# fcogidi/X3D-tf

Measured on NVIDIA B200. Metric: X3D-M clips/sec, higher is better.
Workload: dtype bf16

## Files before the change

### include/x3d_b200.h

```cpp
#ifndef X3D_B200_H_
#define X3D_B200_H_

#include <stddef.h>
#include <stdint.h>

#ifdef __cplusplus
extern "C" {
#endif

#define X3D_B200_VERSION 100

enum x3d_dtype { X3D_F32 = 0, X3D_BF16 = 1 };

enum x3d_status {
  X3D_OK = 0,
  X3D_ERR_INVALID_ARG = -1,
  X3D_ERR_UNSUPPORTED = -2,
  X3D_ERR_LAUNCH = -3,
  X3D_ERR_NO_DEVICE = -4
};

int x3d_version(void);
const char* x3d_last_error(void);

uint32_t x3d_crc32c(const void* data, size_t len, uint32_t crc);

int x3d_stem_fwd(const void* in, int in_dtype, const float* ws, const float* wt,
                 const float* bias, void* out, int out_dtype,
                 int N, int T, int H, int W, int C, int kt, void* stream);

int x3d_stem_tc_fwd(const void* in, int in_dtype, const void* wc, const float* bias, void* out,
                    int N, int T, int H, int W, int C, int kt, void* stream);

typedef struct x3d_pw_args {
  const void* A; const float* Wt; const float* bias; const void* R; const float* se; void* D;
  int64_t M; int32_t K, Nc, lda, ldw, ldr, ldd;
  int64_t rows_per_clip;
  int32_t a_dtype, d_dtype, swish, relu;
  int32_t gather, T, Ho, Wo, Hi, Wi, stride;
} x3d_pw_args;
int x3d_pw_fwd(const x3d_pw_args* args, void* stream);

int x3d_tf32_split(const float* W, float* out, int rows, int cols, int ld, int transpose, void* stream);
int x3d_pw_tf32_fwd(const float* A, const float* Bsplit, const float* bias, float* D, int64_t M, int K,
                    int Nc, int lda, int ldd, int relu, double* stats, void* stream);

int x3d_dw_partial_blocks(int T, int H, int W, int C, int stride, int dtype);
int x3d_dw3x3x3_fwd(const void* in, const float* w, const float* bias, void* out,
                    float* se_partial, int N, int T, int H, int W, int C, int stride,
                    int pad_h, int pad_w, int dtype, void* stream);
int x3d_dw3x3x3_act_fwd(const void* in, const float* w, const float* bias, void* out,
                        float* se_partial, int N, int T, int H, int W, int C, int stride,
                        int pad_h, int pad_w, int dtype, int act, void* stream);

int x3d_dw_planar_partial_blocks(int T, int H, int W, int C, int stride);
int x3d_dw_planar_lane_permille(int T, int H, int W, int C, int stride);
int x3d_dw3x3x3_planar_fwd(const void* in, const float* taps, void* out, float* se_partial, int N, int T,
                           int H, int W, int C, int stride, int pad_h, int pad_w, int act, void* stream);

int x3d_se_mlp_fwd(const float* partial, int nblk, float inv_count, const float* w1,
                   const float* b1, const float* w2, const float* b2, float* scale,
                   int N, int C, int Cw, void* stream);

int x3d_avgpool_fwd(const void* in, float* out, int N, int64_t P, int C, int dtype, void* stream);

int x3d_softmax_viewmean_fwd(const float* logits, float* probs, int N, int ncls, int num_preds,
                             void* stream);

int x3d_gather_rows_fwd(const void* in, void* out, int NT, int Hi, int Wi, int stride, int C,
                        int dtype, void* stream);

int x3d_head_fc_fwd(const float* A, const float* Wt, const float* bias, float* D, int M, int K,
                    int Nc, int lda, int ldw, int ldd, int relu, void* stream);

typedef struct x3d_pw_tc_args {
  const void* A; const void* Wp; const float* bias; const void* R; const float* se; void* D;
  int64_t M; int32_t K, Nc, lda, ldr, ldd, Kpad, Npad;
  int64_t rows_per_clip;
  int32_t swish, relu;
  const void* A2; int64_t a2_nt; int32_t K2, a2_stride, a2_hi, a2_wi;
  float* colmean; int32_t store_d, reserved;
} x3d_pw_tc_args;
int x3d_pw_tc_fwd(const x3d_pw_tc_args* args, void* stream);
int x3d_pw_tc_sampler_supported(int Hi, int Wi, int stride);

int x3d_expand_dw_partial_blocks(int T, int H, int W, int Cin, int C, int stride);
int x3d_expand_dw_fwd(const void* x, const void* wa, const float* bias_a, const float* wb,
                      const float* bias_b, void* out, float* se_partial, int N, int T, int H,
                      int W, int Cin, int C, int Kpad, int Npad, int stride, int pad_h, int pad_w,
                      void* stream);

int x3d_expand_dw2_partial_blocks(int T, int H, int W, int Cin, int C, int stride);
int x3d_expand_dw2_fwd(const void* x, const void* wa, const float* bias_a, const float* wb,
                       const float* bias_b, void* out, float* se_partial, int N, int T, int H,
                       int W, int Cin, int C, int Kpad, int Npad, int stride, int pad_h, int pad_w,
                       int act, void* stream);

int x3d_normalize_u8(const uint8_t* in, void* out, int64_t pixels, const float* mean,
                     const float* std, float norm_value, int dtype, void* stream);
int x3d_eval_views_u8(const uint8_t* video, uint8_t* out, int F, int H, int W, int T, int views,
                      int crops, int S, void* stream);
int x3d_stem_tc_u8_fwd(const uint8_t* in, const float* mean, const float* std, float norm_value,
                       const void* wc, const float* bias, void* out, int N, int T, int H, int W,
                       int C, int kt, void* stream);
int x3d_eval_metrics(const float* probs, const int32_t* labels, double* acc, int V, int ncls,
                     int k, void* stream);


int x3d_colreduce(const float* a, const float* x, const float* mean, const float* rstd,
                  const float* relu_out, int64_t M, int C, int64_t seg_rows, double* out, int mode,
                  void* stream);
int x3d_bn_finalize(const double* sums, int64_t M, int C, float eps, float momentum, float* mean,
                    float* var, float* rstd, float* mov_mean, float* mov_var, void* stream);
int x3d_bn_apply_fwd(const float* x, const float* mean, const float* rstd, const float* gamma,
                     const float* beta, float* y, int64_t M, int C, int relu, void* stream);
int x3d_bn_bwd_apply(const float* dy, const float* x, const float* relu_out, const float* mean,
                     const float* rstd, const float* gamma, const double* sums, float* dx, int64_t M,
                     int C, void* stream);
int x3d_d2f(const double* in, float* out, int64_t n, float scale, void* stream);
int x3d_pw_wgrad(const float* A, const float* dD, double* dW, int64_t M, int K, int N, int lda,
                 int ldd, int gather, int Ho, int Wo, int Hi, int Wi, int stride, void* stream);
int x3d_dw_dgrad(const float* dy, const float* w, float* dx, int N, int T, int H, int W, int C,
                 int stride, int pad_h, int pad_w, void* stream);
int x3d_dw_wgrad(const float* x, const float* dy, double* dwt, int N, int T, int H, int W, int C,
                 int stride, int pad_h, int pad_w, void* stream);
int x3d_stem_convs_fwd(const float* in, const float* ws, float* out, int N, int T, int H, int W,
                       int C, void* stream);
int x3d_stem_convs_wgrad(const float* in, const float* ds, double* dws, int N, int T, int H, int W,
                         int C, void* stream);
int x3d_tconv_fwd(const float* in, const float* wt, float* out, int N, int T, int64_t P, int C,
                  int kt, int flip, void* stream);
int x3d_tconv_wgrad(const float* s, const float* dy, double* dwt, int N, int T, int64_t P, int C,
                    int kt, void* stream);
int x3d_scale_swish_fwd(const float* y, const float* s, float* out, int64_t M, int C,
                        int64_t rows_per_clip, void* stream);
int x3d_scale_swish_bwd(const float* dout, const float* y, const float* s, float* dy, double* ds,
                        int64_t M, int C, int64_t rows_per_clip, void* stream);
int x3d_ew(const float* a, const float* b, float* out, int64_t n, int op, void* stream);
int x3d_pool_bwd(const float* dm, float* dy, int64_t M, int C, int64_t rows_per_clip, float scale,
                 int accumulate, void* stream);
int x3d_strided_add(const float* src, float* dst, int NT, int Ho, int Wo, int Hi, int Wi,
                    int stride, int C, void* stream);
int x3d_dropout_mask(float* mask, int64_t n, float rate, uint64_t seed, void* stream);
int x3d_softmax_xent(const float* logits, const int32_t* labels, float* loss, float* dlogits, int N,
                     int ncls, float gscale, void* stream);
int x3d_sgd_nesterov_step(float* w, const float* grad, float* v, const float* wd, int64_t n,
                          float lr, float momentum, void* stream);
int x3d_adam_step(float* w, const float* grad, float* m, float* v, const float* wd, int64_t n,
                  float lr_t, float beta1, float beta2, float eps, void* stream);

#ifdef __cplusplus
}
#endif
#endif
```

### x3d_tf_b200/_lib.py

```python
from __future__ import annotations

import ctypes as C
import os
import threading

LIB_PATH = os.path.join(os.path.dirname(os.path.abspath(__file__)), "lib", "libx3d_b200.so")

X3D_F32, X3D_BF16 = 0, 1


class X3DLibError(RuntimeError):
    pass


class PwArgs(C.Structure):
    _fields_ = [("A", C.c_void_p), ("Wt", C.c_void_p), ("bias", C.c_void_p), ("R", C.c_void_p),
                ("se", C.c_void_p), ("D", C.c_void_p),
                ("M", C.c_int64), ("K", C.c_int32), ("Nc", C.c_int32), ("lda", C.c_int32),
                ("ldw", C.c_int32), ("ldr", C.c_int32), ("ldd", C.c_int32),
                ("rows_per_clip", C.c_int64),
                ("a_dtype", C.c_int32), ("d_dtype", C.c_int32), ("swish", C.c_int32),
                ("relu", C.c_int32),
                ("gather", C.c_int32), ("T", C.c_int32), ("Ho", C.c_int32), ("Wo", C.c_int32),
                ("Hi", C.c_int32), ("Wi", C.c_int32), ("stride", C.c_int32)]


class PwTcArgs(C.Structure):
    _fields_ = [("A", C.c_void_p), ("Wp", C.c_void_p), ("bias", C.c_void_p), ("R", C.c_void_p),
                ("se", C.c_void_p), ("D", C.c_void_p),
                ("M", C.c_int64), ("K", C.c_int32), ("Nc", C.c_int32), ("lda", C.c_int32),
                ("ldr", C.c_int32), ("ldd", C.c_int32), ("Kpad", C.c_int32), ("Npad", C.c_int32),
                ("rows_per_clip", C.c_int64), ("swish", C.c_int32), ("relu", C.c_int32),
                ("A2", C.c_void_p), ("a2_nt", C.c_int64), ("K2", C.c_int32), ("a2_stride", C.c_int32),
                ("a2_hi", C.c_int32), ("a2_wi", C.c_int32),
                ("colmean", C.c_void_p), ("store_d", C.c_int32), ("reserved", C.c_int32)]


SIGNATURES = {
    "x3d_version": (C.c_int, []),
    "x3d_last_error": (C.c_char_p, []),
    "x3d_crc32c": (C.c_uint32, [C.c_void_p, C.c_size_t, C.c_uint32]),
    "x3d_stem_fwd": (C.c_int, [C.c_void_p, C.c_int, C.c_void_p, C.c_void_p, C.c_void_p,
                               C.c_void_p, C.c_int, C.c_int, C.c_int, C.c_int, C.c_int, C.c_int,
                               C.c_int, C.c_void_p]),
    "x3d_stem_tc_fwd": (C.c_int, [C.c_void_p, C.c_int, C.c_void_p, C.c_void_p, C.c_void_p, C.c_int,
                                  C.c_int, C.c_int, C.c_int, C.c_int, C.c_int, C.c_void_p]),
    "x3d_pw_fwd": (C.c_int, [C.POINTER(PwArgs), C.c_void_p]),
    "x3d_tf32_split": (C.c_int, [C.c_void_p, C.c_void_p, C.c_int, C.c_int, C.c_int, C.c_int, C.c_void_p]),
    "x3d_pw_tf32_fwd": (C.c_int, [C.c_void_p] * 4 + [C.c_int64] + [C.c_int] * 5 + [C.c_void_p, C.c_void_p]),
    "x3d_dw_partial_blocks": (C.c_int, [C.c_int, C.c_int, C.c_int, C.c_int, C.c_int, C.c_int]),
    "x3d_dw3x3x3_fwd": (C.c_int, [C.c_void_p, C.c_void_p, C.c_void_p, C.c_void_p, C.c_void_p,
                                  C.c_int, C.c_int, C.c_int, C.c_int, C.c_int, C.c_int, C.c_int,
                                  C.c_int, C.c_int, C.c_void_p]),
    "x3d_dw3x3x3_act_fwd": (C.c_int, [C.c_void_p, C.c_void_p, C.c_void_p, C.c_void_p, C.c_void_p,
                                      C.c_int, C.c_int, C.c_int, C.c_int, C.c_int, C.c_int, C.c_int,
                                      C.c_int, C.c_int, C.c_int, C.c_void_p]),
    "x3d_dw_planar_partial_blocks": (C.c_int, [C.c_int] * 5),
    "x3d_dw_planar_lane_permille": (C.c_int, [C.c_int] * 5),
    "x3d_dw3x3x3_planar_fwd": (C.c_int, [C.c_void_p] * 4 + [C.c_int] * 9 + [C.c_void_p]),
    "x3d_se_mlp_fwd": (C.c_int, [C.c_void_p, C.c_int, C.c_float, C.c_void_p, C.c_void_p,
                                 C.c_void_p, C.c_void_p, C.c_void_p, C.c_int, C.c_int, C.c_int,
                                 C.c_void_p]),
    "x3d_avgpool_fwd": (C.c_int, [C.c_void_p, C.c_void_p, C.c_int, C.c_int64, C.c_int, C.c_int,
                                  C.c_void_p]),
    "x3d_softmax_viewmean_fwd": (C.c_int, [C.c_void_p, C.c_void_p, C.c_int, C.c_int, C.c_int,
                                           C.c_void_p]),
    "x3d_pw_tc_fwd": (C.c_int, [C.POINTER(PwTcArgs), C.c_void_p]),
    "x3d_pw_tc_sampler_supported": (C.c_int, [C.c_int] * 3),
    "x3d_gather_rows_fwd": (C.c_int, [C.c_void_p, C.c_void_p, C.c_int, C.c_int, C.c_int, C.c_int,
                                      C.c_int, C.c_int, C.c_void_p]),
    "x3d_expand_dw_partial_blocks": (C.c_int, [C.c_int] * 6),
    "x3d_expand_dw_fwd": (C.c_int, [C.c_void_p] * 7 + [C.c_int] * 11 + [C.c_void_p]),
    "x3d_expand_dw2_partial_blocks": (C.c_int, [C.c_int] * 6),
    "x3d_expand_dw2_fwd": (C.c_int, [C.c_void_p] * 7 + [C.c_int] * 12 + [C.c_void_p]),
    "x3d_colreduce": (C.c_int, [C.c_void_p] * 5 + [C.c_int64, C.c_int, C.c_int64, C.c_void_p, C.c_int, C.c_void_p]),
    "x3d_bn_finalize": (C.c_int, [C.c_void_p, C.c_int64, C.c_int, C.c_float, C.c_float] + [C.c_void_p] * 6),
    "x3d_bn_apply_fwd": (C.c_int, [C.c_void_p] * 6 + [C.c_int64, C.c_int, C.c_int, C.c_void_p]),
    "x3d_bn_bwd_apply": (C.c_int, [C.c_void_p] * 8 + [C.c_int64, C.c_int, C.c_void_p]),
    "x3d_d2f": (C.c_int, [C.c_void_p, C.c_void_p, C.c_int64, C.c_float, C.c_void_p]),
    "x3d_pw_wgrad": (C.c_int, [C.c_void_p] * 3 + [C.c_int64] + [C.c_int] * 10 + [C.c_void_p]),
    "x3d_dw_dgrad": (C.c_int, [C.c_void_p] * 3 + [C.c_int] * 8 + [C.c_void_p]),
    "x3d_dw_wgrad": (C.c_int, [C.c_void_p] * 3 + [C.c_int] * 8 + [C.c_void_p]),
    "x3d_stem_convs_fwd": (C.c_int, [C.c_void_p] * 3 + [C.c_int] * 5 + [C.c_void_p]),
    "x3d_stem_convs_wgrad": (C.c_int, [C.c_void_p] * 3 + [C.c_int] * 5 + [C.c_void_p]),
    "x3d_tconv_fwd": (C.c_int, [C.c_void_p] * 3 + [C.c_int, C.c_int, C.c_int64, C.c_int, C.c_int, C.c_int, C.c_void_p]),
    "x3d_tconv_wgrad": (C.c_int, [C.c_void_p] * 3 + [C.c_int, C.c_int, C.c_int64, C.c_int, C.c_int, C.c_void_p]),
    "x3d_scale_swish_fwd": (C.c_int, [C.c_void_p] * 3 + [C.c_int64, C.c_int, C.c_int64, C.c_void_p]),
    "x3d_scale_swish_bwd": (C.c_int, [C.c_void_p] * 5 + [C.c_int64, C.c_int, C.c_int64, C.c_void_p]),
    "x3d_ew": (C.c_int, [C.c_void_p] * 3 + [C.c_int64, C.c_int, C.c_void_p]),
    "x3d_pool_bwd": (C.c_int, [C.c_void_p] * 2 + [C.c_int64, C.c_int, C.c_int64, C.c_float, C.c_int, C.c_void_p]),
    "x3d_strided_add": (C.c_int, [C.c_void_p] * 2 + [C.c_int] * 7 + [C.c_void_p]),
    "x3d_dropout_mask": (C.c_int, [C.c_void_p, C.c_int64, C.c_float, C.c_uint64, C.c_void_p]),
    "x3d_softmax_xent": (C.c_int, [C.c_void_p] * 4 + [C.c_int, C.c_int, C.c_float, C.c_void_p]),
    "x3d_adam_step": (C.c_int, [C.c_void_p] * 5 + [C.c_int64, C.c_float, C.c_float, C.c_float, C.c_float, C.c_void_p]),
    "x3d_sgd_nesterov_step": (C.c_int, [C.c_void_p] * 4 + [C.c_int64, C.c_float, C.c_float, C.c_void_p]),
    "x3d_normalize_u8": (C.c_int, [C.c_void_p, C.c_void_p, C.c_int64, C.POINTER(C.c_float),
                                   C.POINTER(C.c_float), C.c_float, C.c_int, C.c_void_p]),
    "x3d_eval_views_u8": (C.c_int, [C.c_void_p, C.c_void_p] + [C.c_int] * 7 + [C.c_void_p]),
    "x3d_stem_tc_u8_fwd": (C.c_int, [C.c_void_p, C.POINTER(C.c_float), C.POINTER(C.c_float), C.c_float,
                                     C.c_void_p, C.c_void_p, C.c_void_p] + [C.c_int] * 6 + [C.c_void_p]),
    "x3d_eval_metrics": (C.c_int, [C.c_void_p, C.c_void_p, C.c_void_p, C.c_int, C.c_int, C.c_int,
                                   C.c_void_p]),
    "x3d_head_fc_fwd": (C.c_int, [C.c_void_p, C.c_void_p, C.c_void_p, C.c_void_p, C.c_int, C.c_int,
                                  C.c_int, C.c_int, C.c_int, C.c_int, C.c_int, C.c_void_p]),
}

_lock = threading.Lock()
_lib = None


def lib() -> C.CDLL:
    global _lib
    if _lib is None:
        with _lock:
            if _lib is None:
                if not os.path.exists(LIB_PATH):
                    raise X3DLibError(
                        f"{LIB_PATH} is missing: build it with `python -m x3d_tf_b200.build` "
                        "(nvcc, sm_100a).  There is no CPU or PyTorch fallback.")
                h = C.CDLL(LIB_PATH)
                for name, (res, args) in SIGNATURES.items():
                    fn = getattr(h, name)
                    fn.restype, fn.argtypes = res, args
                if h.x3d_version() != 100:
                    raise X3DLibError(f"ABI version mismatch: library reports {h.x3d_version()}")
                _lib = h
                try:
                    from . import tf_bundle
                    tf_bundle.set_native_crc32c(
                        lambda data, crc=0: h.x3d_crc32c(C.c_char_p(data), len(data), crc))
                except Exception:
                    pass
    return _lib


calls = 0


def check(status: int, what: str = "") -> None:
    global calls
    calls += 1
    if status != 0:
        msg = lib().x3d_last_error().decode("utf-8", "replace")
        raise X3DLibError(f"{what or 'x3d call'} failed with status {status}: {msg}")
```

### x3d_tf_b200/csrc/x3d_pw_tc.cu

```cuda
#include <stdlib.h>

#include "tma_common.cuh"

namespace x3d {
namespace tc {

constexpr int kBlockM = 128, kBlockK = 64, kStageBytes = kBlockM * kBlockK * 2;
using namespace ptx;

#ifdef X3D_PW_TRACE
__device__ long long g_pw_trace[8 * 256];
#define X3D_TRACE(slot)                                                                  \
  do {                                                                                   \
    if (trace_on && trace_n < 256) g_pw_trace[trace_n * 8 + (slot)] = clock64();         \
  } while (0)
#else
#define X3D_TRACE(slot) do {} while (0)
#endif

__device__ __forceinline__ void tcgen05_before_sync() {
  asm volatile("tcgen05.fence::before_thread_sync;" ::: "memory");
}
__device__ __forceinline__ void tcgen05_after_sync() {
  asm volatile("tcgen05.fence::after_thread_sync;" ::: "memory");
}
__device__ __forceinline__ void umma_bf16(uint32_t tmem_d, uint64_t desc_a, uint64_t desc_b,
                                          uint32_t idesc, uint32_t accumulate) {
  asm volatile(
      "{\n\t.reg .pred p;\n\t"
      "setp.ne.b32 p, %4, 0;\n\t"
      "tcgen05.mma.cta_group::1.kind::f16 [%0], %1, %2, %3, p;\n\t}" ::"r"(tmem_d),
      "l"(desc_a), "l"(desc_b), "r"(idesc), "r"(accumulate)
      : "memory");
}
__device__ __forceinline__ void umma_commit(uint64_t* bar) {
  asm volatile("tcgen05.commit.cta_group::1.mbarrier::arrive::one.shared::cluster.b64 [%0];" ::"r"(
                   smem_u32(bar))
               : "memory");
}
__device__ __forceinline__ void tmem_ld16(uint32_t taddr, uint32_t (&v)[16]) {
  asm volatile(
      "tcgen05.ld.sync.aligned.32x32b.x16.b32 "
      "{%0, %1, %2, %3, %4, %5, %6, %7, %8, %9, %10, %11, %12, %13, %14, %15}, [%16];"
      : "=r"(v[0]), "=r"(v[1]), "=r"(v[2]), "=r"(v[3]), "=r"(v[4]), "=r"(v[5]), "=r"(v[6]),
        "=r"(v[7]), "=r"(v[8]), "=r"(v[9]), "=r"(v[10]), "=r"(v[11]), "=r"(v[12]), "=r"(v[13]),
        "=r"(v[14]), "=r"(v[15])
      : "r"(taddr));
}
__device__ __forceinline__ void tmem_ld_wait() {
  asm volatile("tcgen05.wait::ld.sync.aligned;" ::: "memory");
}

__device__ __forceinline__ uint64_t make_desc_sw128(uint32_t smem_addr) {
  uint64_t d = 0;
  d |= static_cast<uint64_t>((smem_addr & 0x3FFFF) >> 4);
  d |= static_cast<uint64_t>(0) << 16;
  d |= static_cast<uint64_t>(1024 >> 4) << 32;
  d |= static_cast<uint64_t>(1) << 46;
  d |= static_cast<uint64_t>(2) << 61;
  return d;
}
__device__ __forceinline__ uint32_t make_idesc_bf16(int n) {
  return (1u << 4) | (1u << 7) | (1u << 10) | (static_cast<uint32_t>(n >> 3) << 17) |
         (static_cast<uint32_t>(kBlockM >> 4) << 24);
}

struct Params {
  const float* bias; const bf16* R; const float* se; bf16* D;
  long M; long rows_per_clip;
  int Kc;
  int Nc;
  int ldr, ldd;
  int NT;
  int KC;
  int k16_last;
  int KC1;
  int k16_last1;
  int a2_ppf;
  int a2_wo;
  float* colmean;
  int ldc;
  int store_d;
  int stages;
  int tmem_cols;
  int relu, swish;
  int contiguous;
};

constexpr int kEpiWarps = 8, kProWarps = 8, kOutBufs = 4;
constexpr int kProGroups = 2;
constexpr int kProRows = 8 * kProWarps / kProGroups / 2;
constexpr int kThreadsPlain = 64 + 32 * kEpiWarps, kThreadsPro = kThreadsPlain + 32 * kProWarps;

template <bool kPro>
__global__ void __launch_bounds__(kPro ? kThreadsPro : kThreadsPlain, 1)
pw_tc_kernel(const __grid_constant__ CUtensorMap tmA, const __grid_constant__ CUtensorMap tmW,
             const __grid_constant__ CUtensorMap tmD, const __grid_constant__ CUtensorMap tmA2,
             const Params p) {
  extern __shared__ __align__(1024) uint8_t smem_raw[];
  uint8_t* smem = reinterpret_cast<uint8_t*>((reinterpret_cast<uintptr_t>(smem_raw) + 1023) &
                                             ~static_cast<uintptr_t>(1023));
  const int warp = threadIdx.x >> 5, lane = threadIdx.x & 31;
  const int n0 = blockIdx.y * p.NT;
  const int w_chunk_bytes = p.NT * 128;

  uint8_t* sW = smem;
  uint8_t* sA = sW + p.KC * w_chunk_bytes;
  uint8_t* sD = sA + p.stages * kStageBytes;
  float* sBias = reinterpret_cast<float*>(sD + kOutBufs * kStageBytes);
  uint64_t* bars = reinterpret_cast<uint64_t*>(sBias + 256);
  uint64_t* full = bars;
  uint64_t* empty = full + p.stages;
  uint64_t* xform = empty + p.stages;
  uint64_t* w_full = xform + p.stages;
  uint64_t* t_full = w_full + 1;
  uint64_t* t_empty = t_full + 2;
  uint32_t* tmem_slot = reinterpret_cast<uint32_t*>(t_empty + 2);

  for (int i = threadIdx.x; i < p.NT; i += blockDim.x) {
    const int col = n0 + i;
    sBias[i] = (p.bias != nullptr && col < p.Nc) ? p.bias[col] : 0.f;
  }
  if (warp == 0 && elect_one()) {
    prefetch_tmap(&tmA);
    prefetch_tmap(&tmW);
    prefetch_tmap(&tmD);
    if (p.KC > p.KC1) prefetch_tmap(&tmA2);
    for (int s = 0; s < p.stages; ++s) {
      mbar_init(&full[s], 1);
      mbar_init(&empty[s], 1);
      mbar_init(&xform[s], 32 * kProWarps / kProGroups);
    }
    mbar_init(w_full, 1);
    for (int i = 0; i < 2; ++i) {
      mbar_init(&t_full[i], 1);
      mbar_init(&t_empty[i], 16 * kEpiWarps);
    }
    fence_barrier_init();
  }
  if (warp == 1) {
    asm volatile("tcgen05.alloc.cta_group::1.sync.aligned.shared::cta.b32 [%0], %1;" ::"r"(
                     smem_u32(tmem_slot)),
                 "r"(static_cast<uint32_t>(p.tmem_cols))
                 : "memory");
    asm volatile("tcgen05.relinquish_alloc_permit.cta_group::1.sync.aligned;" ::: "memory");
  }
  tcgen05_before_sync();
  __syncthreads();
  tcgen05_after_sync();
  const uint32_t tmem_base = *tmem_slot;

  const long num_tiles = (p.M + kBlockM - 1) / kBlockM;
  long tile_lo = blockIdx.x, tile_hi = num_tiles, t_stride = gridDim.x;
  if (p.contiguous) {
    const long t_per = num_tiles / gridDim.x, t_rem = num_tiles % gridDim.x;
    tile_lo = blockIdx.x * t_per + (blockIdx.x < t_rem ? blockIdx.x : t_rem);
    tile_hi = tile_lo + t_per + (blockIdx.x < t_rem ? 1 : 0);
    t_stride = 1;
  }

  if (warp == 0) {
    if (elect_one()) {
      mbar_expect_tx(w_full, static_cast<uint32_t>(p.KC * w_chunk_bytes));
      for (int kc = 0; kc < p.KC; ++kc)
        tma_load_2d(sW + kc * w_chunk_bytes, &tmW, kc * kBlockK, n0, w_full);
      pdl_wait();
      pdl_trigger();
      int s = 0;
      uint32_t ph = 0;
      for (long tile = tile_lo; tile < tile_hi; tile += t_stride) {
        const int row0 = static_cast<int>(tile * kBlockM);
        int nt0 = 0, ho0 = 0;
        if (p.a2_ppf) {
          nt0 = row0 / p.a2_ppf;
          ho0 = (row0 - nt0 * p.a2_ppf) / p.a2_wo;
        }
        for (int kc = 0; kc < p.KC; ++kc) {
          mbar_wait(&empty[s], ph ^ 1);
          mbar_expect_tx(&full[s], kStageBytes);
          if (kc < p.KC1) tma_load_2d(sA + s * kStageBytes, &tmA, kc * kBlockK, row0, &full[s]);
          else if (p.a2_ppf) tma_load_4d(smem_u32(sA + s * kStageBytes), &tmA2, (kc - p.KC1) * kBlockK, 0, ho0, nt0, &full[s]);
          else tma_load_2d(sA + s * kStageBytes, &tmA2, (kc - p.KC1) * kBlockK, row0, &full[s]);
          if (++s == p.stages) { s = 0; ph ^= 1; }
        }
      }
    }
  } else if (warp == 1) {
    pdl_trigger();
    const uint32_t idesc = make_idesc_bf16(p.NT);
    mbar_wait(w_full, 0);
    int s = 0;
    uint32_t ph = 0;
    long it = 0;
    for (long tile = tile_lo; tile < tile_hi; tile += t_stride, ++it) {
      const int as = static_cast<int>(it & 1);
      const uint32_t aph = static_cast<uint32_t>((it >> 1) & 1);
      mbar_wait(&t_empty[as], aph ^ 1);
      tcgen05_after_sync();
      const uint32_t d_tmem = tmem_base + static_cast<uint32_t>(as * p.NT);
      for (int kc = 0; kc < p.KC; ++kc) {
        mbar_wait(kPro ? &xform[s] : &full[s], ph);
        tcgen05_after_sync();
        if (elect_one()) {
          const uint32_t a_addr = smem_u32(sA + s * kStageBytes);
          const uint32_t b_addr = smem_u32(sW + kc * w_chunk_bytes);
          const int nk = (kc == p.KC - 1) ? p.k16_last : (kc == p.KC1 - 1 ? p.k16_last1 : 4);
          for (int k = 0; k < nk; ++k)
            umma_bf16(d_tmem, make_desc_sw128(a_addr + k * 32), make_desc_sw128(b_addr + k * 32),
                      idesc, (kc | k) != 0 ? 1u : 0u);
          umma_commit(&empty[s]);
          if (kc == p.KC - 1) umma_commit(&t_full[as]);
        }
        __syncwarp();
        if (++s == p.stages) { s = 0; ph ^= 1; }
      }
    }
  } else if (warp < 2 + kEpiWarps) {
    pdl_wait();
    pdl_trigger();
    const int q = warp & 3;
    const int grp = (warp - 2) >> 2;
    const bool leader = q == 2 && lane == 0;
    const __nv_bfloat162 zero2 = __floats2bfloat162_rn(0.f, 0.f);
    const int r_loc = q * 32 + lane;
    const uint32_t sw_row = static_cast<uint32_t>(r_loc) * 128, sw_x = static_cast<uint32_t>(r_loc & 7);
    const int n_sub = (p.NT + 63) >> 6;
    const uint32_t stage0 = smem_u32(sD + grp * 2 * kStageBytes);
    const uint32_t bias_s = smem_u32(sBias);
    const uint32_t taddr = tmem_base + (static_cast<uint32_t>(q * 32) << 16) +
                           static_cast<uint32_t>(grp * p.NT);
    uint32_t sub_ctr = 0, aph = 0;
#ifdef X3D_PW_TRACE
    const bool trace_on = blockIdx.x == 7 && blockIdx.y == 0 && grp == 0 && leader;
    int trace_n = 0;
#endif
    for (long tile = tile_lo + grp * t_stride; tile < tile_hi; tile += 2 * t_stride, aph ^= 1) {
      X3D_TRACE(0);
      const long row = tile * kBlockM + r_loc;
      const bool row_ok = row < p.M;
      const bf16* rrow = (p.R && row_ok) ? p.R + row * p.ldr + n0 : nullptr;
      uint4 rr[8];
#pragma unroll
      for (int c = 0; c < 8; ++c)
        rr[c] = (rrow && c * 8 < p.NT && n0 + c * 8 < p.Nc) ? __ldg(reinterpret_cast<const uint4*>(rrow + c * 8))
                                                           : make_uint4(0, 0, 0, 0);
      if (p.R) {
        const long nrow = row + 2L * t_stride * kBlockM;
        if (nrow < p.M && tile + 2 * t_stride < tile_hi) {
          const char* np_ = reinterpret_cast<const char*>(p.R + nrow * p.ldr + n0);
          for (int off = 0; off < p.NT * 2; off += 128)
            asm volatile("prefetch.global.L2 [%0];" ::"l"(np_ + off));
        }
      }
      mbar_wait(&t_full[grp], aph);
      X3D_TRACE(1);
      tcgen05_after_sync();
      for (int sb = 0; sb < n_sub; ++sb, ++sub_ctr) {
        if (n0 + sb * 64 >= p.Nc) break;
        const uint32_t buf = stage0 + (sub_ctr & 1) * kStageBytes + sw_row;
        if (sb > 0) {
#pragma unroll
          for (int c = 0; c < 8; ++c) {
            const int cc = sb * 64 + c * 8;
            rr[c] = (rrow && cc < p.NT && n0 + cc < p.Nc) ? __ldg(reinterpret_cast<const uint4*>(rrow + cc))
                                                         : make_uint4(0, 0, 0, 0);
          }
        }
#pragma unroll
        for (int g = 0; g < 4; ++g) {
          const int c0 = sb * 64 + g * 16;
          if (c0 >= p.NT || n0 + c0 >= p.Nc) continue;
          uint32_t v[16];
          tmem_ld16(taddr + c0, v);
          tmem_ld_wait();
#ifdef X3D_PW_TRACE
          if (g == 0 && sb == 0 && trace_on && trace_n < 256) g_pw_trace[trace_n * 8 + 7] = clock64();
#endif
#pragma unroll
          for (int h = 0; h < 2; ++h) {
            const int cc = c0 + h * 8;
            float4 b0, b1;
            asm volatile("ld.shared.v4.f32 {%0, %1, %2, %3}, [%4];" : "=f"(b0.x), "=f"(b0.y), "=f"(b0.z), "=f"(b0.w) : "r"(bias_s + cc * 4));
            asm volatile("ld.shared.v4.f32 {%0, %1, %2, %3}, [%4];" : "=f"(b1.x), "=f"(b1.y), "=f"(b1.z), "=f"(b1.w) : "r"(bias_s + cc * 4 + 16));
            float2 y[4];
            y[0] = __fadd2_rn(make_float2(__uint_as_float(v[h * 8 + 0]), __uint_as_float(v[h * 8 + 1])), make_float2(b0.x, b0.y));
            y[1] = __fadd2_rn(make_float2(__uint_as_float(v[h * 8 + 2]), __uint_as_float(v[h * 8 + 3])), make_float2(b0.z, b0.w));
            y[2] = __fadd2_rn(make_float2(__uint_as_float(v[h * 8 + 4]), __uint_as_float(v[h * 8 + 5])), make_float2(b1.x, b1.y));
            y[3] = __fadd2_rn(make_float2(__uint_as_float(v[h * 8 + 6]), __uint_as_float(v[h * 8 + 7])), make_float2(b1.z, b1.w));
            if (p.R) {
              const uint4 ru = rr[g * 2 + h];
              const uint32_t rw[4] = {ru.x, ru.y, ru.z, ru.w};
#pragma unroll
              for (int j = 0; j < 4; ++j)
                y[j] = __fadd2_rn(y[j], make_float2(__uint_as_float(rw[j] << 16),
                                                    __uint_as_float(rw[j] & 0xffff0000u)));
            }
            uint32_t o[4];
#pragma unroll
            for (int j = 0; j < 4; ++j) {
              __nv_bfloat162 t = __float22bfloat162_rn(y[j]);
              if (p.relu) t = __hmax2(t, zero2);
              o[j] = *reinterpret_cast<uint32_t*>(&t);
            }
            const uint32_t chunk = static_cast<uint32_t>(g * 2 + h);
            asm volatile("st.shared.v4.b32 [%0], {%1, %2, %3, %4};" ::"r"(buf + ((chunk ^ sw_x) << 4)),
                         "r"(o[0]), "r"(o[1]), "r"(o[2]), "r"(o[3]) : "memory");
          }
        }
        X3D_TRACE(2);
        if (sb == n_sub - 1 || n0 + (sb + 1) * 64 >= p.Nc) {
          tcgen05_before_sync();
          mbar_arrive(&t_empty[grp]);
        }
        fence_proxy_async();
        X3D_TRACE(3);
        if (leader) tma_store_wait_read<0>();
        X3D_TRACE(4);
        if (grp == 0) asm volatile("bar.sync 1, 128;" ::: "memory");
        else asm volatile("bar.sync 2, 128;" ::: "memory");
        X3D_TRACE(5);
        if (leader && p.store_d) {
          tma_store_2d(&tmD, stage0 + (sub_ctr & 1) * kStageBytes, n0 + sb * 64,
                       static_cast<int>(tile * kBlockM));
          tma_store_commit();
        }
        if (p.colmean != nullptr) {
          const int ccol = r_loc & 63, half = r_loc >> 6;
          const int col_g = n0 + sb * 64 + ccol;
          const long row_base = tile * kBlockM + half * 64;
          int nrows = p.M - row_base < 64 ? static_cast<int>(p.M - row_base) : 64;
          if (ccol < p.NT - sb * 64 && col_g < p.Nc && nrows > 0) {
            const uint32_t sbuf = stage0 + (sub_ctr & 1) * kStageBytes;
            float sum = 0.f;
            for (int r = 0; r < nrows; ++r) {
              const int row = half * 64 + r;
              unsigned short h;
              asm volatile("ld.shared.u16 %0, [%1];" : "=h"(h)
                           : "r"(sbuf + row * 128 + ((((ccol >> 3) ^ (row & 7)) << 4) | ((ccol & 7) << 1))));
              sum += __uint_as_float(static_cast<uint32_t>(h) << 16);
            }
            p.colmean[(tile * 2 + half) * p.ldc + col_g] = sum * (1.f / 64.f);
          }
        }
        X3D_TRACE(6);
#ifdef X3D_PW_TRACE
        if (trace_on) ++trace_n;
#endif
      }
    }
    if (leader) tma_store_wait_read<0>();
  } else if (kPro) {
    pdl_wait();
    pdl_trigger();
    const int tt = threadIdx.x - kThreadsPlain;
    constexpr int kGT = 32 * kProWarps / kProGroups;
    const int grp = tt / kGT;
    const int pchunk = tt & 7;
    const int rbase = (tt % kGT) >> 3;
    const int kin = (pchunk ^ (rbase & 7)) << 3;
    const uint32_t rpc = static_cast<uint32_t>(p.rows_per_clip > 0 ? p.rows_per_clip : 0x7fffffff);
    const uint32_t step = static_cast<uint32_t>(t_stride) * kBlockM;
    struct Pos { long tile; int kc; uint32_t clip, rem; };
    auto advance = [&](Pos& q) {
      if (++q.kc == p.KC) {
        q.kc = 0;
        q.tile += t_stride;
        q.rem += step;
        while (q.rem >= rpc) { q.rem -= rpc; ++q.clip; }
      }
    };
    auto se_request = [&](const Pos& q, float4& s0, float4& s1) {
      s0 = make_float4(1.f, 1.f, 1.f, 1.f);
      s1 = s0;
      const int k = q.kc * kBlockK + kin;
      if (p.se != nullptr && q.tile < tile_hi && k < p.Kc && q.kc < p.KC1 && q.rem + kBlockM <= rpc) {
        const float4* sp = reinterpret_cast<const float4*>(p.se + static_cast<long>(q.clip) * p.Kc + k);
        s0 = __ldg(sp);
        s1 = __ldg(sp + 1);
      }
    };
    Pos cur;
    cur.tile = tile_lo; cur.kc = 0;
    cur.clip = static_cast<uint32_t>(tile_lo * static_cast<long>(kBlockM) / rpc);
    cur.rem = static_cast<uint32_t>(tile_lo * static_cast<long>(kBlockM) - static_cast<long>(cur.clip) * rpc);
    int s = 0;
    uint32_t ph = 0;
    for (int g = 0; g < grp; ++g) {
      advance(cur);
      if (++s == p.stages) { s = 0; ph ^= 1; }
    }
    float4 nx0, nx1;
    se_request(cur, nx0, nx1);
    while (cur.tile < tile_hi) {
      const uint32_t clip0 = cur.clip, rem0 = cur.rem;
      const bool one_clip = rem0 + kBlockM <= rpc;
      const int k = cur.kc * kBlockK + kin;
      const bool k_ok = k < p.Kc && cur.kc < p.KC1;
      float2 sc[4];
      sc[0] = make_float2(nx0.x, nx0.y); sc[1] = make_float2(nx0.z, nx0.w);
      sc[2] = make_float2(nx1.x, nx1.y); sc[3] = make_float2(nx1.z, nx1.w);
#pragma unroll
      for (int g = 0; g < kProGroups; ++g) advance(cur);
      se_request(cur, nx0, nx1);
      mbar_wait(&full[s], ph);
      if (k_ok) {
        const uint32_t addr0 = smem_u32(sA + s * kStageBytes) + rbase * 128 + pchunk * 16;
        float2 hs[4];
#pragma unroll
        for (int j = 0; j < 4; ++j) hs[j] = __fmul2_rn(sc[j], make_float2(0.5f, 0.5f));
#pragma unroll
        for (int half = 0; half < kBlockM / (kGT / 8) / 4; ++half) {
          uint32_t w[4][4];
#pragma unroll
          for (int i = 0; i < 4; ++i)
            asm volatile("ld.shared.v4.b32 {%0, %1, %2, %3}, [%4];"
                         : "=r"(w[i][0]), "=r"(w[i][1]), "=r"(w[i][2]), "=r"(w[i][3])
                         : "r"(addr0 + (half * 4 + i) * (kGT / 8 * 128)));
#pragma unroll
          for (int i = 0; i < 4; ++i) {
            if (p.se && !one_clip) {
              uint32_t x = rem0 + rbase + (kGT / 8) * (half * 4 + i), clip = clip0;
              while (x >= rpc) { x -= rpc; ++clip; }
              if (static_cast<long>(clip) * rpc + x < p.M) {
                const float4* sp = reinterpret_cast<const float4*>(p.se + static_cast<long>(clip) * p.Kc + k);
                const float4 s0 = __ldg(sp), s1 = __ldg(sp + 1);
                sc[0] = make_float2(s0.x, s0.y); sc[1] = make_float2(s0.z, s0.w);
                sc[2] = make_float2(s1.x, s1.y); sc[3] = make_float2(s1.z, s1.w);
#pragma unroll
                for (int j = 0; j < 4; ++j) hs[j] = __fmul2_rn(sc[j], make_float2(0.5f, 0.5f));
              }
            }
            if (p.swish) {
#pragma unroll
              for (int j = 0; j < 4; ++j) {
                const float2 h = __fmul2_rn(make_float2(__uint_as_float(w[i][j] << 16), __uint_as_float(w[i][j] & 0xffff0000u)), hs[j]);
                float2 t;
                asm("tanh.approx.f32 %0, %1;" : "=f"(t.x) : "f"(h.x));
                asm("tanh.approx.f32 %0, %1;" : "=f"(t.y) : "f"(h.y));
                __nv_bfloat162 t2 = __float22bfloat162_rn(__ffma2_rn(h, t, h));
                w[i][j] = *reinterpret_cast<uint32_t*>(&t2);
              }
            } else {
#pragma unroll
              for (int j = 0; j < 4; ++j) {
                const float2 scj = make_float2(2.f * hs[j].x, 2.f * hs[j].y);
                __nv_bfloat162 t2 = __float22bfloat162_rn(__fmul2_rn(
                    make_float2(__uint_as_float(w[i][j] << 16), __uint_as_float(w[i][j] & 0xffff0000u)), scj));
                w[i][j] = *reinterpret_cast<uint32_t*>(&t2);
              }
            }
            asm volatile("st.shared.v4.b32 [%0], {%1, %2, %3, %4};" ::"r"(addr0 + (half * 4 + i) * (kGT / 8 * 128)), "r"(w[i][0]), "r"(w[i][1]), "r"(w[i][2]), "r"(w[i][3]) : "memory");
          }
        }
      }
      fence_proxy_async();
      mbar_arrive(&xform[s]);
      s += kProGroups;
      while (s >= p.stages) { s -= p.stages; ph ^= 1; }
    }
  }

  tcgen05_before_sync();
  __syncthreads();
  if (warp == 1) {
    asm volatile("tcgen05.dealloc.cta_group::1.sync.aligned.b32 %0, %1;" ::"r"(tmem_base),
                 "r"(static_cast<uint32_t>(p.tmem_cols))
                 : "memory");
  }
}

static bool make_map_2d(CUtensorMap* m, const void* base, uint64_t inner, uint64_t outer,
                        uint64_t row_stride_bytes, uint32_t box_inner, uint32_t box_outer) {
  EncodeTiledFn enc = tensor_map_encoder();
  if (!enc) return false;
  cuuint64_t dims[2] = {inner, outer};
  cuuint64_t strides[1] = {row_stride_bytes};
  cuuint32_t box[2] = {box_inner, box_outer};
  cuuint32_t estr[2] = {1, 1};
  return enc(m, CU_TENSOR_MAP_DATA_TYPE_BFLOAT16, 2, const_cast<void*>(base), dims, strides, box,
             estr, CU_TENSOR_MAP_INTERLEAVE_NONE, CU_TENSOR_MAP_SWIZZLE_128B,
             CU_TENSOR_MAP_L2_PROMOTION_L2_256B, CU_TENSOR_MAP_FLOAT_OOB_FILL_NONE) == CUDA_SUCCESS;
}

static bool make_map_sampler(CUtensorMap* m, const void* base, int C, int Hi, int Wi, long NT, int s,
                             int bw, int bh, int bf) {
  EncodeTiledFn enc = tensor_map_encoder();
  if (!enc) return false;
  const int Ho = (Hi - 1) / s + 1, Wo = (Wi - 1) / s + 1;
  cuuint64_t dims[4] = {(cuuint64_t)C, (cuuint64_t)Wo, (cuuint64_t)Ho, (cuuint64_t)NT};
  cuuint64_t strides[3] = {(cuuint64_t)s * C * 2, (cuuint64_t)s * Wi * C * 2, (cuuint64_t)Hi * Wi * C * 2};
  cuuint32_t box[4] = {64, (cuuint32_t)bw, (cuuint32_t)bh, (cuuint32_t)bf};
  cuuint32_t estr[4] = {1, 1, 1, 1};
  return enc(m, CU_TENSOR_MAP_DATA_TYPE_BFLOAT16, 4, const_cast<void*>(base), dims, strides, box,
             estr, CU_TENSOR_MAP_INTERLEAVE_NONE, CU_TENSOR_MAP_SWIZZLE_128B,
             CU_TENSOR_MAP_L2_PROMOTION_L2_256B, CU_TENSOR_MAP_FLOAT_OOB_FILL_NONE) == CUDA_SUCCESS;
}

static bool sampler_box(int Ho, int Wo, int* bh, int* bf) {
  if (Wo <= 0 || Wo > kBlockM || kBlockM % Wo) return false;
  const int rh = kBlockM / Wo;
  if (rh <= Ho) { if (Ho % rh) return false; *bh = rh; *bf = 1; return true; }
  if (rh % Ho) return false;
  *bh = Ho; *bf = rh / Ho;
  return true;
}

}
}

using namespace x3d;

extern "C" int x3d_pw_tc_sampler_supported(int Hi, int Wi, int stride) {
  if (Hi <= 0 || Wi <= 0 || stride < 1) return 0;
  int bh, bf;
  return tc::sampler_box((Hi - 1) / stride + 1, (Wi - 1) / stride + 1, &bh, &bf) ? 1 : 0;
}

extern "C" int x3d_pw_tc_fwd(const x3d_pw_tc_args* a, void* stream) {
  X3D_REQUIRE(a && a->A && a->Wp && a->D, X3D_ERR_INVALID_ARG, "x3d_pw_tc_fwd: null pointer");
  X3D_REQUIRE(a->M > 0 && a->M < (1L << 31), X3D_ERR_INVALID_ARG, "x3d_pw_tc_fwd: M out of range");
  X3D_REQUIRE(a->K > 0 && a->K % 8 == 0 && a->lda % 8 == 0 && a->lda >= a->K, X3D_ERR_INVALID_ARG,
              "x3d_pw_tc_fwd: K=%d / lda=%d must be multiples of 8", a->K, a->lda);
  X3D_REQUIRE(a->Nc > 0 && a->Nc % 8 == 0 && a->ldd % 8 == 0 && (!a->R || a->ldr % 8 == 0),
              X3D_ERR_INVALID_ARG, "x3d_pw_tc_fwd: Nc/ldd/ldr must be multiples of 8");
  X3D_REQUIRE(a->Kpad % 64 == 0 && a->Kpad >= a->K && a->Npad % 16 == 0 && a->Npad >= a->Nc,
              X3D_ERR_INVALID_ARG, "x3d_pw_tc_fwd: bad packed weight extents Kpad=%d Npad=%d", a->Kpad, a->Npad);
  X3D_REQUIRE(!a->se || a->rows_per_clip > 0, X3D_ERR_INVALID_ARG, "x3d_pw_tc_fwd: rows_per_clip missing");
  X3D_REQUIRE(!a->colmean || (reinterpret_cast<uintptr_t>(a->colmean) & 3) == 0, X3D_ERR_INVALID_ARG, "x3d_pw_tc_fwd: colmean alignment");
  X3D_REQUIRE((reinterpret_cast<uintptr_t>(a->A) & 15) == 0 && (reinterpret_cast<uintptr_t>(a->Wp) & 15) == 0 &&
              (reinterpret_cast<uintptr_t>(a->D) & 15) == 0, X3D_ERR_INVALID_ARG, "x3d_pw_tc_fwd: pointers must be 16-byte aligned");
  X3D_REQUIRE(device_sm_count() > 0 && device_is_sm100(), X3D_ERR_NO_DEVICE, "x3d_pw_tc_fwd: needs an sm_100 device");
  const int k16_total = (a->K + 15) / 16;
  const int KC1 = (k16_total + 3) / 4;
  const int k16_last1 = k16_total - (KC1 - 1) * 4;
  int KC = KC1, k16_last = k16_last1, a2_bh = 0, a2_bf = 0, a2_ho = 0, a2_wo = 0;
  if (a->A2) {
    X3D_REQUIRE(!a->R, X3D_ERR_INVALID_ARG, "x3d_pw_tc_fwd: A2 (shortcut as extra K) and R (residual) exclude each other");
    X3D_REQUIRE(a->K2 > 0 && a->K2 % 8 == 0 && a->a2_stride >= 0, X3D_ERR_INVALID_ARG, "x3d_pw_tc_fwd: bad second source K2=%d stride=%d", a->K2, a->a2_stride);
    X3D_REQUIRE((reinterpret_cast<uintptr_t>(a->A2) & 15) == 0, X3D_ERR_INVALID_ARG, "x3d_pw_tc_fwd: A2 must be 16-byte aligned");
    if (a->a2_stride > 0) {
      X3D_REQUIRE(a->a2_hi > 0 && a->a2_wi > 0 && a->a2_nt > 0, X3D_ERR_INVALID_ARG, "x3d_pw_tc_fwd: bad second source %dx%d", a->a2_hi, a->a2_wi);
      a2_ho = (a->a2_hi - 1) / a->a2_stride + 1; a2_wo = (a->a2_wi - 1) / a->a2_stride + 1;
      X3D_REQUIRE(a->M == a->a2_nt * a2_ho * a2_wo, X3D_ERR_INVALID_ARG, "x3d_pw_tc_fwd: M=%ld is not nt*Ho*Wo = %ld*%d*%d",
                  (long)a->M, (long)a->a2_nt, a2_ho, a2_wo);
      X3D_REQUIRE(tc::sampler_box(a2_ho, a2_wo, &a2_bh, &a2_bf), X3D_ERR_UNSUPPORTED,
                  "x3d_pw_tc_fwd: 128-pixel tiles do not align with %dx%d frames (x3d_pw_tc_sampler_supported)", a2_ho, a2_wo);
    }
    const int k16_2 = (a->K2 + 15) / 16, KC2 = (k16_2 + 3) / 4;
    KC = KC1 + KC2; k16_last = k16_2 - (KC2 - 1) * 4;
    X3D_REQUIRE(a->Kpad >= KC * 64, X3D_ERR_INVALID_ARG, "x3d_pw_tc_fwd: Kpad=%d < %d (both sources, 64-wide chunks)", a->Kpad, KC * 64);
  }
  const int budget = device_max_smem() - 1024  - 1024  - 512  -
                     tc::kOutBufs * tc::kStageBytes ;
  int n_tiles = (a->Npad + 255) / 256;
  int NT = 0, stages = 0;
  for (;; ++n_tiles) {
    const int per = (a->Npad + n_tiles - 1) / n_tiles;
    NT = n_tiles == 1 ? (per + 15) / 16 * 16 : (per + 63) / 64 * 64;
    const int wbytes = KC * NT * 128;
    stages = (budget - wbytes) / tc::kStageBytes;
    if (stages >= 3 || NT <= 64) break;
  }
  X3D_REQUIRE(stages >= 2 && stages >= tc::kProGroups, X3D_ERR_UNSUPPORTED, "x3d_pw_tc_fwd: K=%d too large for shared memory", a->K);
  if (stages > 8) stages = 8;
  n_tiles = (a->Nc + NT - 1) / NT;
  int tmem_cols = 32;
  while (tmem_cols < 2 * NT) tmem_cols *= 2;
  X3D_REQUIRE(tmem_cols <= 512, X3D_ERR_UNSUPPORTED, "x3d_pw_tc_fwd: NT=%d needs too much TMEM", NT);

  CUtensorMap tmA, tmW;
  X3D_REQUIRE(tensor_map_encoder() != nullptr, X3D_ERR_NO_DEVICE, "x3d_pw_tc_fwd: cuTensorMapEncodeTiled unavailable");
  X3D_REQUIRE(tc::make_map_2d(&tmA, a->A, (uint64_t)a->K, (uint64_t)a->M, (uint64_t)a->lda * 2, 64, 128),
              X3D_ERR_LAUNCH, "x3d_pw_tc_fwd: tensor map for A failed (K=%d M=%ld lda=%d)", a->K, (long)a->M, a->lda);
  X3D_REQUIRE(tc::make_map_2d(&tmW, a->Wp, (uint64_t)a->Kpad, (uint64_t)a->Npad, (uint64_t)a->Kpad * 2, 64, (uint32_t)NT),
              X3D_ERR_LAUNCH, "x3d_pw_tc_fwd: tensor map for W failed (Kpad=%d Npad=%d NT=%d)", a->Kpad, a->Npad, NT);

  CUtensorMap tmD;
  X3D_REQUIRE(tc::make_map_2d(&tmD, a->D, (uint64_t)a->Nc, (uint64_t)a->M, (uint64_t)a->ldd * 2, 64, 128),
              X3D_ERR_LAUNCH, "x3d_pw_tc_fwd: tensor map for D failed (Nc=%d M=%ld ldd=%d)", a->Nc, (long)a->M, a->ldd);
  CUtensorMap tmA2 = tmA;
  if (a->A2 && a->a2_stride > 0)
    X3D_REQUIRE(tc::make_map_sampler(&tmA2, a->A2, a->K2, a->a2_hi, a->a2_wi, (long)a->a2_nt, a->a2_stride, a2_wo, a2_bh, a2_bf),
                X3D_ERR_LAUNCH, "x3d_pw_tc_fwd: tensor map for A2 failed (K2=%d %dx%d stride %d)", a->K2, a->a2_hi, a->a2_wi, a->a2_stride);
  else if (a->A2)
    X3D_REQUIRE(tc::make_map_2d(&tmA2, a->A2, (uint64_t)a->K2, (uint64_t)a->M, (uint64_t)a->K2 * 2, 64, 128),
                X3D_ERR_LAUNCH, "x3d_pw_tc_fwd: tensor map for dense A2 failed (K2=%d M=%ld)", a->K2, (long)a->M);
  tc::Params p;
  p.bias = a->bias; p.R = static_cast<const bf16*>(a->R); p.se = a->se; p.D = static_cast<bf16*>(a->D);
  p.M = a->M; p.rows_per_clip = a->rows_per_clip; p.Kc = a->K; p.Nc = a->Nc; p.ldr = a->ldr; p.ldd = a->ldd;
  p.colmean = a->colmean; p.ldc = a->Nc; p.store_d = a->colmean == nullptr || a->store_d;
  p.KC1 = KC1; p.k16_last1 = k16_last1; p.a2_ppf = (a->A2 && a->a2_stride > 0) ? a2_ho * a2_wo : 0; p.a2_wo = a2_wo;
  p.NT = NT; p.KC = KC; p.k16_last = k16_last; p.stages = stages; p.tmem_cols = tmem_cols;
  p.relu = a->relu; p.swish = a->swish;
  p.contiguous = a->se != nullptr ? 1 : 0;

  const size_t smem = 1024 + (size_t)KC * NT * 128 + (size_t)(stages + tc::kOutBufs) * tc::kStageBytes + 1024 + 512;
  const long num_tiles = (a->M + tc::kBlockM - 1) / tc::kBlockM;
  int gx = device_sm_count() / n_tiles;
  if (gx < 1) gx = 1;
  if (gx > num_tiles) gx = (int)num_tiles;
  dim3 grid(gx, n_tiles);
  cudaStream_t st = static_cast<cudaStream_t>(stream);
  const bool pro = (a->se != nullptr) || a->swish;
  cudaError_t e;
  static SmemOptIn optin_pro, optin_plain;
  if (pro) {
    e = ensure_dynamic_smem(tc::pw_tc_kernel<true>, optin_pro, smem, false);
    X3D_REQUIRE(e == cudaSuccess, X3D_ERR_LAUNCH, "x3d_pw_tc_fwd: smem attribute: %s", cudaGetErrorString(e));
    e = launch_pdl(tc::pw_tc_kernel<true>, grid, dim3(tc::kThreadsPro), smem, st, tmA, tmW, tmD, tmA2, p);
    X3D_REQUIRE(e == cudaSuccess, X3D_ERR_LAUNCH, "x3d_pw_tc_fwd: launch: %s", cudaGetErrorString(e));
  } else {
    e = ensure_dynamic_smem(tc::pw_tc_kernel<false>, optin_plain, smem, false);
    X3D_REQUIRE(e == cudaSuccess, X3D_ERR_LAUNCH, "x3d_pw_tc_fwd: smem attribute: %s", cudaGetErrorString(e));
    e = launch_pdl(tc::pw_tc_kernel<false>, grid, dim3(tc::kThreadsPlain), smem, st, tmA, tmW, tmD, tmA2, p);
    X3D_REQUIRE(e == cudaSuccess, X3D_ERR_LAUNCH, "x3d_pw_tc_fwd: launch: %s", cudaGetErrorString(e));
  }
  return check_launch("x3d_pw_tc_fwd");
}

#ifdef X3D_PW_TRACE
extern "C" int x3d_pw_trace_dump(long long* host_out) {
  return cudaMemcpyFromSymbol(host_out, x3d::tc::g_pw_trace, sizeof(long long) * 8 * 256) == cudaSuccess ? 0 : -3;
}
#endif
```

### x3d_tf_b200/model.py

```python
from __future__ import annotations

import os

import math
from collections import OrderedDict
from typing import Dict, Iterable, List, Optional, Tuple

import numpy as np
import torch

from . import arch as A
from . import ops
from . import tf_bundle

_BN_LEAVES = ("gamma", "beta", "moving_mean", "moving_variance")


def _pad8(c: int) -> int:
    return (c + 7) // 8 * 8


def _glorot(rng, shape, fan_in, fan_out):
    lim = math.sqrt(6.0 / (fan_in + fan_out))
    return rng.uniform(-lim, lim, size=shape).astype(np.float32)


class _LoadStatus:

    def __init__(self, missing, unused):
        self.missing, self.unused = list(missing), list(unused)

    def expect_partial(self):
        return self

    def assert_consumed(self):
        if self.missing or self.unused:
            raise AssertionError(f"unresolved: missing={self.missing[:3]} unused={self.unused[:3]}")
        return self

    def assert_existing_objects_matched(self):
        if self.missing:
            raise AssertionError(f"variables without a checkpoint value: {self.missing[:3]}")
        return self


class Layer:

    _init_seed = 0

    def __init__(self, name: Optional[str] = None):
        self.name = name or type(self).__name__.lower()
        self._vars: "OrderedDict[str, np.ndarray]" = OrderedDict()
        self._children: "OrderedDict[str, Layer]" = OrderedDict()
        self._dev: Dict[tuple, dict] = {}

    def _rng(self):
        Layer._init_seed += 1
        return np.random.default_rng(Layer._init_seed)

    def _add_conv(self, key: str, shape: Tuple[int, ...], groups: int = 1):
        rf = int(np.prod(shape[:-2]))
        fan_in, fan_out = rf * shape[-2], rf * shape[-1]
        self._vars[key] = _glorot(self._rng(), shape, fan_in, fan_out)

    def _add_bn(self, key: str, c: int):
        self._vars[f"{key}/gamma"] = np.ones(c, np.float32)
        self._vars[f"{key}/beta"] = np.zeros(c, np.float32)
        self._vars[f"{key}/moving_mean"] = np.zeros(c, np.float32)
        self._vars[f"{key}/moving_variance"] = np.ones(c, np.float32)

    def _child(self, key: str, layer: "Layer") -> "Layer":
        self._children[key] = layer
        return layer

    def named_variables(self, prefix: str = "") -> "OrderedDict[str, np.ndarray]":
        out: "OrderedDict[str, np.ndarray]" = OrderedDict()
        for k, v in self._vars.items():
            out[prefix + k] = v
        for ck, ch in self._children.items():
            out.update(ch.named_variables(f"{prefix}{ck}/"))
        return out

    def set_weights_dict(self, weights: Dict[str, np.ndarray], prefix: str = "",
                         strict: bool = True) -> List[str]:
        missing = []
        for k in list(self._vars):
            full = prefix + k
            if full in weights:
                w = np.asarray(weights[full], dtype=np.float32)
                if w.shape != self._vars[k].shape:
                    raise ValueError(f"{full}: shape {w.shape} != expected {self._vars[k].shape}")
                self._vars[k] = np.ascontiguousarray(w)
            else:
                missing.append(full)
        for ck, ch in self._children.items():
            missing += ch.set_weights_dict(weights, f"{prefix}{ck}/", strict=False)
        self._invalidate()
        if strict and missing:
            raise KeyError(f"no value for {len(missing)} variables, e.g. {missing[:3]}")
        return missing

    def count_params(self) -> int:
        return sum(int(v.size) for v in self.named_variables().values())

    def _invalidate(self):
        self._dev.clear()
        for ch in self._children.values():
            ch._invalidate()

    def __call__(self, x, training: bool = False):
        return self.call(x, training=training)

    def call(self, x, training: bool = False):
        raise NotImplementedError

    @staticmethod
    def _no_training(training: bool):
        if training:
            raise NotImplementedError(
                "training=True on a stand-alone block: the training kernels (batch-statistics BatchNorm, "
                "dropout, backward) run on the whole model's flat parameter arena -- use "
                "X3D.call(x, training=True) / X3D.fit(...) (training.X3DTrainer), see INTEGRATION.md")

    def _fold_bn(self, key: str, eps: float) -> Tuple[np.ndarray, np.ndarray]:
        g = self._vars[f"{key}/gamma"].astype(np.float64)
        b = self._vars[f"{key}/beta"].astype(np.float64)
        m = self._vars[f"{key}/moving_mean"].astype(np.float64)
        v = self._vars[f"{key}/moving_variance"].astype(np.float64)
        s = g / np.sqrt(v + eps)
        return s, b - m * s


def _dev_f32(a: np.ndarray, device) -> torch.Tensor:
    return torch.from_numpy(np.ascontiguousarray(a, dtype=np.float32)).to(device)


def _pad_to(a: np.ndarray, axis: int, size: int) -> np.ndarray:
    if a.shape[axis] == size:
        return a
    pad = [(0, 0)] * a.ndim
    pad[axis] = (0, size - a.shape[axis])
    return np.pad(a, pad)


def _as_device_clip(x, device) -> torch.Tensor:
    if isinstance(x, np.ndarray):
        x = torch.from_numpy(np.ascontiguousarray(x))
    if not isinstance(x, torch.Tensor):
        raise TypeError("input must be a torch.Tensor or numpy array in NDHWC layout")
    if x.dim() != 5:
        raise ValueError(f"expected a 5-D NDHWC tensor, got shape {tuple(x.shape)}")
    if x.dtype == torch.float16:
        x = x.to(torch.bfloat16)
    elif x.dtype == torch.float64:
        x = x.to(torch.float32)
    if x.dtype not in (torch.float32, torch.bfloat16, torch.uint8):
        raise TypeError(f"unsupported input dtype {x.dtype}")
    if not x.is_cuda:
        if device is None:
            if not torch.cuda.is_available():
                raise RuntimeError("no CUDA device: the X3D path has no CPU implementation")
            device = torch.device("cuda", torch.cuda.current_device())
        x = x.to(device, non_blocking=True)
    return x.contiguous()


def _pad_channels(x: torch.Tensor, cs: int) -> torch.Tensor:
    c = x.shape[-1]
    if c == cs:
        return x
    out = torch.zeros(x.shape[:-1] + (cs,), dtype=x.dtype, device=x.device)
    out[..., :c] = x
    return out


class PointwiseConv:

    def __init__(self, kernel: np.ndarray, scale, shift, device, bias=None):
        k2 = kernel.reshape(kernel.shape[-2], kernel.shape[-1]).astype(np.float64)
        K, N = k2.shape
        self.K, self.N, self.Ks, self.Ns = K, N, _pad8(K), _pad8(N)
        if scale is not None:
            k2 = k2 * scale[None, :]
        b = np.zeros(N, np.float64) if shift is None else np.asarray(shift, np.float64)
        if bias is not None:
            b = b + np.asarray(bias, np.float64)
        wt = _pad_to(_pad_to(k2, 0, self.Ks), 1, self.Ns)
        self.wt = _dev_f32(wt, device)
        self.bias = _dev_f32(_pad_to(b, 0, self.Ns), device)
        npad, kpad = (self.Ns + 15) // 16 * 16, (self.Ks + 63) // 64 * 64
        wp = _pad_to(_pad_to(k2.T, 0, npad), 1, kpad)
        self.wp = torch.from_numpy(np.ascontiguousarray(wp, dtype=np.float32)).to(device).to(
            torch.bfloat16).contiguous()
        self._k2t = _pad_to(_pad_to(k2.T, 0, self.Ns), 1, self.Ks)
        self._paired: Dict[int, Tuple[torch.Tensor, torch.Tensor]] = {}
        self._stacked: Dict[int, tuple] = {}

    def _pair_factor(self, M: int, rows_per_clip: int = 0) -> int:
        for P in (4, 2):
            if P > Options.pair_pixels or M % P or (rows_per_clip and rows_per_clip % P):
                continue
            if P * self.Ks > Options.pair_max_k or P * self.Ns > Options.pair_max_n:
                continue
            if not Options.pair_aligned and self.Ks % 16 == 0 and self.Ns % 16 == 0:
                continue
            return P
        return 1

    def _paired_weights(self, P: int, device) -> Tuple[torch.Tensor, torch.Tensor]:
        if P not in self._paired:
            w = np.zeros((P * self.Ns, P * self.Ks), np.float64)
            for i in range(P):
                w[i * self.Ns:(i + 1) * self.Ns, i * self.Ks:(i + 1) * self.Ks] = self._k2t
            npad, kpad = (P * self.Ns + 15) // 16 * 16, (P * self.Ks + 63) // 64 * 64
            w = _pad_to(_pad_to(w, 0, npad), 1, kpad)
            wp = torch.from_numpy(np.ascontiguousarray(w, dtype=np.float32)).to(device).to(
                torch.bfloat16).contiguous()
            self._paired[P] = (wp, self.bias.repeat(P).contiguous())
        return self._paired[P]

    def _stacked_weights(self, other: "PointwiseConv", device) -> Tuple[torch.Tensor, torch.Tensor]:
        key = id(other)
        if key not in self._stacked:
            if other.Ns != self.Ns:
                raise ValueError("stacked pointwise convs need the same output width")
            k1, k2 = (self.Ks + 63) // 64 * 64, (other.Ks + 63) // 64 * 64
            w = np.zeros(((self.Ns + 15) // 16 * 16, k1 + k2), np.float64)
            w[:self.Ns, :self.Ks] = self._k2t
            w[:self.Ns, k1:k1 + other.Ks] = other._k2t
            wp = torch.from_numpy(np.ascontiguousarray(w, dtype=np.float32)).to(device).to(
                torch.bfloat16).contiguous()
            self._stacked[key] = (wp, (self.bias + other.bias).contiguous(), other)
        return self._stacked[key][:2]

    def run_with_shortcut(self, a: torch.Tensor, M: int, shortcut: "PointwiseConv", x: torch.Tensor,
                          stride: int, *, se=None, rows_per_clip=0, swish=False, relu=False) -> torch.Tensor:
        wp, bias = self._stacked_weights(shortcut, a.device)
        return ops.pw_tc_fwd(a, wp, bias, M=M, K=self.Ks, Nc=self.Ns, se=se, rows_per_clip=rows_per_clip,
                             swish=swish, relu=relu, a2=x, a2_stride=stride)

    def run(self, a: torch.Tensor, M: int, *, use_tc: bool, out_dtype=None, residual=None,
            se=None, rows_per_clip=0, swish=False, relu=False, gather=None, pair_rows=0) -> torch.Tensor:
        if use_tc and a.dtype == torch.bfloat16 and gather is None and \
                (out_dtype is None or out_dtype == torch.bfloat16):
            P = self._pair_factor(M, pair_rows or rows_per_clip) if se is None else 1
            if P > 1 and a.is_contiguous() and (residual is None or residual.is_contiguous()):
                wp, bias = self._paired_weights(P, a.device)
                return ops.pw_tc_fwd(a, wp, bias, M=M // P, K=P * self.Ks, Nc=P * self.Ns, residual=residual,
                                     swish=swish, relu=relu).view(M, self.Ns)
            return ops.pw_tc_fwd(a, self.wp, self.bias, M=M, K=self.Ks, Nc=self.Ns,
                                 residual=residual, se=se, rows_per_clip=rows_per_clip,
                                 swish=swish, relu=relu)
        return ops.pw_fwd(a, self.wt, self.bias, M=M, K=self.Ks, Nc=self.Ns, out_dtype=out_dtype,
                          residual=residual, se=se, rows_per_clip=rows_per_clip, swish=swish,
                          relu=relu, gather=gather)


class Options:
    pointwise = "tc"
    stem = "tc"
    fuse_expand = os.environ.get("X3D_FUSE_EXPAND", "off")
    stem_u8 = os.environ.get("X3D_STEM_U8", "normalize")
    swish_in_dw = os.environ.get("X3D_SWISH_IN_DW", "1") == "1"
    fold_shortcut = os.environ.get("X3D_FOLD_SHORTCUT", "1") == "1"
    pool_in_conv5 = os.environ.get("X3D_POOL_IN_CONV5", "1") == "1"
    channelwise = os.environ.get("X3D_CHANNELWISE", "auto")
    pair_pixels = int(os.environ.get("X3D_PAIR_PIXELS", "2"))
    pair_max_k = int(os.environ.get("X3D_PAIR_MAX_K", "256"))
    pair_max_n = int(os.environ.get("X3D_PAIR_MAX_N", "256"))
    pair_aligned = os.environ.get("X3D_PAIR_ALIGNED", "0") == "1"


def _use_tc() -> bool:
    return Options.pointwise == "tc"


class X3D_Stem(Layer):

    def __init__(self, bn_cfg, regularizer=None, out_channels: int = 24,
                 temp_filter_size: int = 5, in_channels: int = 3):
        super().__init__(name="conv_1")
        self.bn_momentum, self.bn_eps = bn_cfg.MOMENTUM, bn_cfg.EPS
        self.out_channels, self.temp_filter_size = out_channels, temp_filter_size
        self._add_conv("conv_s/kernel", (1, 3, 3, in_channels, out_channels))
        self._add_conv("conv_t/kernel", (temp_filter_size, 1, 1, 1, out_channels),
                       groups=out_channels)
        self._add_bn("bn", out_channels)
        self.input_norm: Optional[Tuple[tuple, tuple]] = None

    def _prep(self, device):
        key = (str(device),)
        if key not in self._dev:
            C, cs = self.out_channels, _pad8(self.out_channels)
            s, t = self._fold_bn("bn", self.bn_eps)
            ws = self._vars["conv_s/kernel"].reshape(27, C).astype(np.float64)
            wt = self._vars["conv_t/kernel"].reshape(self.temp_filter_size, C).astype(np.float64) * s
            d = {"ws": _dev_f32(_pad_to(ws, 1, cs), device),
                 "wt": _dev_f32(_pad_to(wt, 1, cs), device),
                 "bias": _dev_f32(_pad_to(t, 0, cs), device)}
            if cs <= 32 and self.temp_filter_size == 5:
                wc = np.zeros((self.temp_filter_size, 4, 32, 8), np.float64)
                full = ws[None, :, :] * wt[:, None, :]
                for k in range(27):
                    wc[:, k // 8, :C, k % 8] = full[:, k, :]
                d["wc"] = torch.from_numpy(wc.astype(np.float32)).to(device).to(
                    torch.bfloat16).contiguous()
            self._dev[key] = d
        return self._dev[key]

    def _forward(self, x: torch.Tensor, out_dtype) -> torch.Tensor:
        d = self._prep(x.device)
        ops.Profiler.tag = "stem"
        tc = out_dtype == torch.bfloat16 and "wc" in d and Options.stem == "tc"
        if x.dtype == torch.uint8:
            if self.input_norm is None:
                raise ValueError("uint8 clips need input_norm = (mean, std) (cfg.DATA.MEAN / cfg.DATA.STD)")
            mean, std = self.input_norm
            if tc and Options.stem_u8 == "fused":
                return ops.stem_tc_u8_fwd(x, mean, std, d["wc"], d["bias"])
            x = ops.normalize_u8(x, mean, std, out_dtype)
        if tc:
            return ops.stem_tc_fwd(x, d["wc"], d["bias"])
        return ops.stem_fwd(x, d["ws"], d["wt"], d["bias"], out_dtype)

    def call(self, input, training: bool = False):
        self._no_training(training)
        x = _as_device_clip(input, None)
        out_dtype = torch.float32 if x.dtype == torch.uint8 else x.dtype
        return self._forward(x, out_dtype)[..., :self.out_channels]


class AdaptiveAvgPool3D(Layer):

    def __init__(self, spatial_out_shape=(1, 1, 1), data_format="channels_last", **kwargs):
        super().__init__(name=kwargs.get("name"))
        assert len(spatial_out_shape) == 3, "Please specify 3D shape"
        assert data_format in ("channels_last", "channels_first")
        self.data_format, self.out_shape = data_format, tuple(spatial_out_shape)

    def call(self, input, training: bool = False):
        x = _as_device_clip(input, None)
        if self.data_format == "channels_first":
            x = x.permute(0, 2, 3, 4, 1).contiguous()
        m = ops.avgpool_fwd(x)
        n, c = m.shape
        o = self.out_shape
        if self.data_format == "channels_last":
            return m.reshape(-1, o[0], o[1], o[2], c)
        return m.reshape(-1, c, o[0], o[1], o[2])


class Bottleneck(Layer):

    def __init__(self, channels: tuple, bn_cfg, regularizer=None, stride: int = 1,
                 block_index: int = 0, se_ratio: float = 0.0625, temp_kernel_size: int = 3,
                 in_channels: Optional[int] = None):
        super().__init__()
        if temp_kernel_size != 3:
            raise NotImplementedError("only the 3x3x3 channelwise kernel is built")
        self.block_index, self._bn_cfg = block_index, bn_cfg
        self.inner, self.out_channels, self.stride = channels[0], channels[1], stride
        self.in_channels = in_channels
        self.has_se = A.se_enabled(block_index)
        self.se_width = A.round_width(self.inner, se_ratio) if self.has_se else 0
        if in_channels is not None:
            self._build(in_channels)

    def _build(self, cin: int):
        self.in_channels = cin
        inner, cout = self.inner, self.out_channels
        v = OrderedDict()
        old, self._vars = self._vars, v
        self._add_conv("a/kernel", (1, 1, 1, cin, inner))
        self._add_bn("bn_a", inner)
        self._add_conv("b/kernel", (3, 3, 3, 1, inner), groups=inner)
        self._add_bn("bn_b", inner)
        if self.has_se:
            self._add_conv("se_fc1/kernel", (1, 1, 1, inner, self.se_width))
            self._vars["se_fc1/bias"] = np.zeros(self.se_width, np.float32)
            self._add_conv("se_fc2/kernel", (1, 1, 1, self.se_width, inner))
            self._vars["se_fc2/bias"] = np.zeros(inner, np.float32)
        self._add_conv("c/kernel", (1, 1, 1, inner, cout))
        self._add_bn("bn_c", cout)
        self._vars.update(old)

    def _prep(self, device):
        key = (str(device),)
        if key not in self._dev:
            eps = self._bn_cfg.EPS
            ci = _pad8(self.inner)
            sa, ta = self._fold_bn("bn_a", eps)
            sb, tb = self._fold_bn("bn_b", eps)
            sc, tc = self._fold_bn("bn_c", eps)
            d = {"a": PointwiseConv(self._vars["a/kernel"], sa, ta, device),
                 "c": PointwiseConv(self._vars["c/kernel"], sc, tc, device)}
            wb = self._vars["b/kernel"].reshape(27, self.inner).astype(np.float64) * sb
            d["wb"] = _dev_f32(_pad_to(wb, 1, ci), device)
            d["bb"] = _dev_f32(_pad_to(tb, 0, ci), device)
            d["wbp"] = ops.dw_planar_taps(d["wb"], d["bb"])
            if self.has_se:
                w1 = self._vars["se_fc1/kernel"].reshape(self.inner, self.se_width)
                w2 = self._vars["se_fc2/kernel"].reshape(self.se_width, self.inner)
                d["w1"] = _dev_f32(_pad_to(w1, 0, ci), device)
                d["b1"] = _dev_f32(self._vars["se_fc1/bias"], device)
                d["w2"] = _dev_f32(_pad_to(w2, 1, ci), device)
                d["b2"] = _dev_f32(_pad_to(self._vars["se_fc2/bias"], 0, ci), device)
            self._dev[key] = d
        return self._dev[key]

    def _forward(self, x: torch.Tensor, residual: Optional[torch.Tensor] = None,
                 relu: bool = False, shortcut: Optional[PointwiseConv] = None,
                 shortcut_rows: Optional[torch.Tensor] = None) -> torch.Tensor:
        if self.in_channels is None:
            raise RuntimeError("Bottleneck used before its input width is known")
        d = self._prep(x.device)
        N, T, H, W, _ = x.shape
        ci = _pad8(self.inner)
        tc = _use_tc()
        _, ph, _ = A.same_pad(H, 3, self.stride)
        _, pw, _ = A.same_pad(W, 3, self.stride)
        mode = Options.fuse_expand
        fuse2 = tc and x.dtype == torch.bfloat16 and (mode == "all" or (mode == "auto" and ci <= 72)) and \
            ops.expand_dw2_supported(T, H, W, x.shape[-1], ci, self.stride) > 0
        if fuse2:
            ops.Profiler.tag = "ab"
            swish_in_b = Options.swish_in_dw and not self.has_se
            b, partial = ops.expand_dw2_fwd(x, d["a"].wp, d["a"].bias, d["wb"], d["bb"],
                                            self.stride, ph, pw, self.has_se, swish=swish_in_b)
        elif tc and mode == "v1" and x.dtype == torch.bfloat16 and \
                ops.expand_dw_supported(T, H, W, x.shape[-1], ci, self.stride) > 0:
            ops.Profiler.tag = "ab"
            b, partial = ops.expand_dw_fwd(x, d["a"].wp, d["a"].bias, d["wb"], d["bb"],
                                           self.stride, ph, pw, self.has_se)
            swish_in_b = False
        else:
            ops.Profiler.tag = "a"
            a = d["a"].run(x, N * T * H * W, use_tc=tc, relu=True, pair_rows=T * H * W).view(N, T, H, W, ci)
            ops.Profiler.tag = "b"
            swish_in_b = Options.swish_in_dw and not self.has_se
            cw = Options.channelwise
            planar = a.dtype == torch.bfloat16 and cw != "tma" and \
                ops.dw_planar_supported(T, H, W, ci, self.stride) > 0 and \
                (cw == "planar" or (self.stride == 1 and
                                    ops.dw_planar_lane_use(T, H, W, ci, self.stride) >= 0.85))
            if planar:
                b, partial = ops.dw_planar_fwd(a, d["wbp"], self.stride, ph, pw, self.has_se, swish=swish_in_b)
            else:
                b, partial = ops.dw_fwd(a, d["wb"], d["bb"], self.stride, ph, pw, self.has_se, swish=swish_in_b)
            del a
        _, _, Ho, Wo, _ = b.shape
        se = None
        if self.has_se:
            ops.Profiler.tag = "se"
            se = ops.se_mlp_fwd(partial, T * Ho * Wo, d["w1"], d["b1"], d["w2"], d["b2"])
        ops.Profiler.tag = "c"
        if shortcut is not None:
            out = d["c"].run_with_shortcut(b, N * T * Ho * Wo, shortcut, x if shortcut_rows is None else shortcut_rows,
                                           self.stride, se=se,
                                           rows_per_clip=T * Ho * Wo, swish=not swish_in_b, relu=relu)
        else:
            out = d["c"].run(b, N * T * Ho * Wo, use_tc=tc, se=se, rows_per_clip=T * Ho * Wo,
                             swish=not swish_in_b, residual=residual, relu=relu)
        return out.view(N, T, Ho, Wo, _pad8(self.out_channels))

    def call(self, input, training: bool = False):
        self._no_training(training)
        x = _as_device_clip(input, None)
        if self.in_channels is None:
            self._build(x.shape[-1])
        if x.shape[-1] != self.in_channels:
            raise ValueError(f"expected {self.in_channels} input channels, got {x.shape[-1]}")
        y = self._forward(_pad_channels(x, _pad8(self.in_channels)))
        return y[..., :self.out_channels]


class ResBlock(Layer):

    _block_index = 0

    def __init__(self, channels: tuple, bn_cfg, regularizer=None, stride: int = 1,
                 se_ratio: float = 0.0625, temp_kernel_size: int = 3):
        super().__init__(name="ResBlock_%u" % ResBlock._block_index)
        ResBlock._block_index += 1
        self.in_channels, self.inner_channels, self.out_channels = channels
        self._bn_cfg, self.stride = bn_cfg, stride
        self.has_shortcut = self.in_channels != self.out_channels or stride != 1
        if self.has_shortcut:
            self._add_conv("residual/kernel", (1, 1, 1, self.in_channels, self.out_channels))
            self._add_bn("bn_r", self.out_channels)
        self.bottleneck = self._child("bottleneck", Bottleneck(
            channels=channels[1:], stride=stride, bn_cfg=bn_cfg, regularizer=regularizer,
            block_index=ResBlock._block_index, se_ratio=se_ratio,
            temp_kernel_size=temp_kernel_size, in_channels=self.in_channels))

    def _prep(self, device):
        key = (str(device),)
        if key not in self._dev:
            d = {}
            if self.has_shortcut:
                s, t = self._fold_bn("bn_r", self._bn_cfg.EPS)
                d["r"] = PointwiseConv(self._vars["residual/kernel"], s, t, device)
            self._dev[key] = d
        return self._dev[key]

    def _forward(self, x: torch.Tensor) -> torch.Tensor:
        d = self._prep(x.device)
        N, T, H, W, _ = x.shape
        if self.has_shortcut:
            s = self.stride
            Ho, Wo = (H - 1) // s + 1, (W - 1) // s + 1
            ops.Profiler.tag = "shortcut"
            if _use_tc() and x.dtype == torch.bfloat16 and Options.fold_shortcut:
                rows = None if ops.pw_tc_sampler_supported(H, W, s) else \
                    (x.view(-1, x.shape[-1]) if s == 1 else ops.gather_rows_fwd(x, s))
                return self.bottleneck._forward(x, relu=True, shortcut=d["r"], shortcut_rows=rows)
            if _use_tc() and x.dtype == torch.bfloat16:
                rows = x.view(-1, x.shape[-1]) if s == 1 else ops.gather_rows_fwd(x, s)
                res = d["r"].run(rows, N * T * Ho * Wo, use_tc=True, pair_rows=T * Ho * Wo)
            else:
                res = d["r"].run(x, N * T * Ho * Wo, use_tc=False, gather=(T, Ho, Wo, H, W, s))
        else:
            res = x
        return self.bottleneck._forward(x, residual=res, relu=True)

    def call(self, input, training: bool = False):
        self._no_training(training)
        x = _as_device_clip(input, None)
        if x.shape[-1] != self.in_channels:
            raise ValueError(f"expected {self.in_channels} input channels, got {x.shape[-1]}")
        y = self._forward(_pad_channels(x, _pad8(self.in_channels)))
        return y[..., :self.out_channels]


class ResStage(Layer):

    _stage_index = 2

    def __init__(self, in_channels: int, inner_channels: int, out_channels: int, depth: int,
                 bn_cfg, regularizer=None, se_ratio: float = 0.0625, temp_kernel_size: int = 3):
        super().__init__(name="res_stage_%u" % ResStage._stage_index)
        ResStage._stage_index += 1
        self._bn_cfg, self._inner_channels = bn_cfg, inner_channels
        self.in_channels, self.out_channels = in_channels, out_channels
        self.blocks: List[ResBlock] = []
        for i in range(depth):
            blk = ResBlock(bn_cfg=bn_cfg, se_ratio=se_ratio, regularizer=regularizer,
                           temp_kernel_size=temp_kernel_size, stride=2 if i == 0 else 1,
                           channels=(in_channels if i == 0 else out_channels, inner_channels,
                                     out_channels))
            self.blocks.append(self._child(f"stage/layer_with_weights-{i}", blk))

    def _forward(self, x):
        for b in self.blocks:
            x = b._forward(x)
        return x

    def call(self, input, training: bool = False):
        self._no_training(training)
        x = _as_device_clip(input, None)
        y = self._forward(_pad_channels(x, _pad8(self.in_channels)))
        return y[..., :self.out_channels]


def finalize_metrics(acc: torch.Tensor, group=None, k: int = 5, return_dict: bool = True):
    import torch.distributed as dist
    if dist.is_available() and dist.is_initialized():
        backend = dist.get_backend(group)
        buf = acc if (backend == "nccl") == acc.is_cuda else (acc.cuda() if backend == "nccl" else acc.cpu())
        dist.all_reduce(buf, op=dist.ReduceOp.SUM, group=group)
        acc = buf
    a = [float(v) for v in acc.detach().cpu().tolist()]
    count = max(a[3], 1.0)
    res = {"loss": a[0] / count, "acc": a[1] / count, f"top_{k}_acc": a[2] / count, "videos": int(a[3])}
    return res if return_dict else [res["loss"], res["acc"], res[f"top_{k}_acc"]]


def keras_default_weights(cfg, seed: int = 0) -> "OrderedDict[str, np.ndarray]":
    saved = (ResBlock._block_index, ResStage._stage_index, Layer._init_seed)
    reset_block_counters()
    Layer._init_seed = int(seed) * 100003
    try:
        return X3D(cfg).named_variables()
    finally:
        ResBlock._block_index, ResStage._stage_index, Layer._init_seed = saved


def reset_block_counters() -> None:
    ResBlock._block_index = 0
    ResStage._stage_index = 2


class _Conv5(Layer):

    def __init__(self, cin: int, cout: int, bn_cfg):
        super().__init__(name="conv_5")
        self.cin, self.cout, self._bn_cfg = cin, cout, bn_cfg
        self._add_conv("layer_with_weights-0/kernel", (1, 1, 1, cin, cout))
        self._add_bn("layer_with_weights-1", cout)

    def _prep(self, device):
        key = (str(device),)
        if key not in self._dev:
            s, t = self._fold_bn("layer_with_weights-1", self._bn_cfg.EPS)
            self._dev[key] = PointwiseConv(self._vars["layer_with_weights-0/kernel"], s, t, device)
        return self._dev[key]

    def _forward(self, x):
        N, T, H, W, _ = x.shape
        ops.Profiler.tag = "conv5"
        y = self._prep(x.device).run(x, N * T * H * W, use_tc=_use_tc(), relu=True)
        return y.view(N, T, H, W, _pad8(self.cout))

    def _forward_pooled(self, x) -> Optional[torch.Tensor]:
        N, T, H, W, _ = x.shape
        P = T * H * W
        if not (_use_tc() and x.dtype == torch.bfloat16 and Options.pool_in_conv5 and P % 64 == 0):
            return None
        ops.Profiler.tag = "conv5"
        pc = self._prep(x.device)
        means = ops.pw_tc_fwd(x, pc.wp, pc.bias, M=N * P, K=pc.Ks, Nc=pc.Ns, relu=True, colmean=True, store=False)
        ops.Profiler.tag = "head_pool"
        return ops.avgpool_fwd(means[:N * P // 64].view(N, P // 64, pc.Ns))


class _Dense(Layer):
    def __init__(self, name, key_shape, bias: bool):
        super().__init__(name=name)
        if len(key_shape) == 5:
            self._add_conv("kernel", key_shape)
        else:
            self._vars["kernel"] = _glorot(self._rng(), key_shape, key_shape[0], key_shape[1])
        if bias:
            self._vars["bias"] = np.zeros(key_shape[-1], np.float32)

    def _prep(self, device):
        key = (str(device),)
        if key not in self._dev:
            self._dev[key] = PointwiseConv(self._vars["kernel"], None, None, device,
                                           bias=self._vars.get("bias"))
        return self._dev[key]


class X3D(Layer):

    def __init__(self, cfg, dtype: Optional[str] = None, device=None, use_cuda_graph: bool = True):
        super().__init__(name="X3D")
        self.cfg = cfg
        self.num_classes = cfg.NETWORK.NUM_CLASSES
        self._bn_cfg = cfg.NETWORK.BN
        self._num_preds = cfg.TEST.NUM_TEMPORAL_VIEWS * cfg.TEST.NUM_SPATIAL_CROPS
        self._arch = A.build_arch(cfg, first_block_index=ResBlock._block_index + 1)
        self._conv1_dim = self._arch.stem_channels
        self._dtype = {None: None, "float32": torch.float32, "bfloat16": torch.bfloat16,
                       "bf16": torch.bfloat16, "fp32": torch.float32}[dtype]
        self._device = torch.device(device) if device is not None else None
        self._use_graph = use_cuda_graph
        self._graphs: Dict[tuple, tuple] = {}
        self.last_logits: Optional[torch.Tensor] = None

        self.conv1 = self._child("conv1", X3D_Stem(
            regularizer=None, bn_cfg=cfg.NETWORK.BN, out_channels=self._conv1_dim,
            temp_filter_size=cfg.NETWORK.C1_TEMP_FILTER,
            in_channels=cfg.DATA.NUM_INPUT_CHANNELS))
        if cfg.DATA.NUM_INPUT_CHANNELS == 3:
            self.conv1.input_norm = (tuple(cfg.DATA.MEAN), tuple(cfg.DATA.STD))
        self.stages: List[ResStage] = []
        for s, (depth, cin, inner, cout) in enumerate(self._arch.stage_dims):
            st = ResStage(in_channels=cin, inner_channels=inner, out_channels=cout, depth=depth,
                          bn_cfg=self._bn_cfg, regularizer=None)
            self.stages.append(self._child(f"stages/{s}", st))
        last_out = self._arch.stage_dims[-1][3]
        c5 = self.stages[-1]._inner_channels
        self.conv5 = self._child("conv5", _Conv5(last_out, c5, self._bn_cfg))
        self.pool5 = AdaptiveAvgPool3D(name="pool_5")
        self.fc1 = self._child("fc1", _Dense("fc_1", (1, 1, 1, c5, 2048), bias=False))
        self.dropout_rate = cfg.NETWORK.DROPOUT_RATE
        self.fc2 = self._child("fc2", _Dense("fc_2", (2048, self.num_classes), bias=True))

    def load_weights(self, filepath: str, verify: bool = True) -> _LoadStatus:
        names = set(self.named_variables())
        got = tf_bundle.load_model_variables(filepath, verify=verify)
        missing = self.set_weights_dict(got, strict=False)
        return _LoadStatus(missing, sorted(set(got) - names))

    def save_weights(self, filepath: str) -> None:
        tf_bundle.write_bundle(filepath, dict(self.named_variables()))

    def _forward(self, x: torch.Tensor, training: bool) -> Tuple[torch.Tensor, torch.Tensor]:
        act_dtype = self._dtype or (torch.float32 if x.dtype == torch.uint8 else x.dtype)
        out = self.conv1._forward(x, act_dtype)
        for st in self.stages:
            out = st._forward(out)
        pooled = self.conv5._forward_pooled(out)
        if pooled is None:
            out = self.conv5._forward(out)
            ops.Profiler.tag = "head_pool"
            pooled = ops.avgpool_fwd(out)
        N = pooled.shape[0]
        ops.Profiler.tag = "head_fc"
        f1 = self.fc1._prep(x.device)
        h = ops.head_fc_fwd(pooled, f1.wt, None, K=f1.Ks, Nc=f1.Ns, relu=True)
        f2 = self.fc2._prep(x.device)
        logits_p = ops.head_fc_fwd(h, f2.wt, f2.bias, K=f2.Ks, Nc=f2.Ns)
        logits = logits_p if f2.Ns == self.num_classes else \
            logits_p[:, :self.num_classes].contiguous()
        ops.Profiler.tag = "head_softmax"
        probs = ops.softmax_viewmean_fwd(logits, 1 if training else self._num_preds)
        return probs, logits

    def _check_input(self, shape):
        if len(shape) != 5 or shape[-1] != self.cfg.DATA.NUM_INPUT_CHANNELS:
            raise ValueError(f"expected NDHWC clips with {self.cfg.DATA.NUM_INPUT_CHANNELS} channels, "
                             f"got shape {tuple(shape)}")
        if shape[0] % self._num_preds != 0:
            raise ValueError(f"batch {shape[0]} must be a multiple of "
                             f"NUM_TEMPORAL_VIEWS*NUM_SPATIAL_CROPS = {self._num_preds}")

    def _graph(self, shape, dtype, device, slot: int = 0, training: bool = False):
        key = (tuple(shape), dtype, str(device), Options.pointwise, Options.stem, Options.stem_u8, Options.swish_in_dw,
               Options.fuse_expand, Options.channelwise, Options.fold_shortcut, Options.pool_in_conv5, slot)
        if key not in self._graphs:
            static_in = torch.zeros(tuple(shape), dtype=dtype, device=device)
            self._forward(static_in, training)
            torch.cuda.current_stream().synchronize()
            g = torch.cuda.CUDAGraph()
            pool = None
            if slot:
                pool = self._graph(shape, dtype, device, 0, training)[0].pool()
            with torch.cuda.graph(g, pool=pool):
                s_probs, s_logits = self._forward(static_in, training)
            self._graphs[key] = (g, static_in, s_probs, s_logits)
        return self._graphs[key]

    def __call__(self, x, training: bool = False, copy: bool = True):
        return self.call(x, training=training, copy=copy)

    def _trainer(self):
        if getattr(self, "_tr", None) is None:
            import torch.distributed as dist
            from .training import X3DTrainer
            world = dist.get_world_size() if dist.is_available() and dist.is_initialized() else 1
            rank = dist.get_rank() if world > 1 else 0
            dev = self._device or torch.device("cuda", torch.cuda.current_device())
            self._tr = X3DTrainer(self.cfg, device=dev, world=world, rank=rank).load(dict(self.named_variables()))
        return self._tr

    def _sync_from_trainer(self):
        if getattr(self, "_tr", None) is not None:
            self.set_weights_dict(self._tr.weights(), strict=False)

    def set_weights_dict(self, weights, prefix: str = "", strict: bool = True):
        self._graphs.clear()
        missing = super().set_weights_dict(weights, prefix, strict)
        if getattr(self, "_tr", None) is not None and not getattr(self, "_syncing", False):
            self._tr = None
        return missing

    def fit(self, dataset, epochs: int = 1, initial_epoch: int = 0, steps_per_epoch: Optional[int] = None,
            lr_schedule=None, verbose: int = 0, **_):
        from . import ops
        from .training import lr_schedule as default_schedule
        tr = self._trainer()
        sched = lr_schedule or (lambda e: default_schedule(self.cfg, e))
        dev = tr.device
        mean, std = tuple(self.cfg.DATA.MEAN), tuple(self.cfg.DATA.STD)
        hist = {"loss": [], "lr": []}
        for epoch in range(initial_epoch, epochs):
            lr = float(sched(epoch))
            tot, n = torch.zeros((), dtype=torch.float64, device=dev), 0
            for i, (clips, labels) in enumerate(dataset):
                if steps_per_epoch is not None and i >= steps_per_epoch:
                    break
                x = _as_device_clip(clips, dev)
                if x.dtype == torch.uint8:
                    x = ops.normalize_u8(x, mean, std, torch.float32)
                lab = torch.as_tensor(np.asarray(labels.cpu() if isinstance(labels, torch.Tensor) else labels)
                                      .reshape(-1), dtype=torch.int32).to(dev)
                loss = tr.step(x.float(), lab, lr)
                tot += loss.double().mean()
                n += 1
            hist["loss"].append(float(tot / max(n, 1)))
            hist["lr"].append(lr)
            if verbose:
                print(f"Epoch {epoch + 1}/{epochs} - loss: {hist['loss'][-1]:.4f} - lr: {lr:.5f}")
        self._syncing = True
        try:
            self._sync_from_trainer()
        finally:
            self._syncing = False
        return hist

    def call(self, input, training: bool = False, copy: bool = True):
        if training:
            x = _as_device_clip(input, self._device)
            if x.dtype == torch.uint8:
                x = ops.normalize_u8(x, tuple(self.cfg.DATA.MEAN), tuple(self.cfg.DATA.STD), torch.float32)
            tr = self._trainer()
            logits = tr.forward_training(x.float())
            tr.iteration += 1
            self.last_logits = logits
            self._syncing = True
            try:
                self._sync_from_trainer()
            finally:
                self._syncing = False
            return ops.softmax_viewmean_fwd(logits.contiguous(), 1)
        x = _as_device_clip(input, self._device)
        self._check_input(x.shape)
        if not self._use_graph:
            probs, self.last_logits = self._forward(x, training)
            return probs
        g, static_in, s_probs, s_logits = self._graph(x.shape, x.dtype, x.device, 0, training)
        if x.data_ptr() != static_in.data_ptr():
            static_in.copy_(x, non_blocking=True)
        g.replay()
        if not copy:
            self.last_logits = s_logits
            return s_probs
        self.last_logits = s_logits.clone()
        return s_probs.clone()

    def static_input(self, shape, dtype=torch.bfloat16):
        for key, (_, static_in, _, _) in self._graphs.items():
            if tuple(key[0]) == tuple(shape) and key[1] == dtype and key[-1] == 0:
                return static_in
        return None

    def predict(self, batches, training: bool = False, on_device=None):
        self._no_training(training)
        if not torch.cuda.is_available():
            raise RuntimeError("no CUDA device: the X3D path has no CPU implementation")
        device = self._device or torch.device("cuda", torch.cuda.current_device())
        main = torch.cuda.current_stream(device)
        if getattr(self, "_copy_stream", None) is None:
            self._copy_stream = torch.cuda.Stream(device)
        cs = self._copy_stream
        slots: Dict[tuple, dict] = {}

        def stage(hb, slot):
            if isinstance(hb, np.ndarray):
                hb = torch.from_numpy(np.ascontiguousarray(hb))
            if hb.dtype in (torch.float16, torch.float64):
                hb = hb.to(torch.float32)
            self._check_input(hb.shape)
            g, static_in, s_probs, s_logits = self._graph(hb.shape, hb.dtype, device, slot, training)
            st = slots.setdefault((tuple(hb.shape), hb.dtype, slot), {
                "host_out": torch.empty(tuple(s_probs.shape), dtype=torch.float32).pin_memory(),
                "done": torch.cuda.Event(), "copied": torch.cuda.Event()})
            st.update(g=g, s_probs=s_probs, s_logits=s_logits)
            cs.wait_event(st["done"])
            cs.wait_stream(main) if not st.get("used") else None
            st["used"] = True
            with torch.cuda.stream(cs):
                static_in.copy_(hb, non_blocking=True)
                st["copied"].record(cs)
            return st

        it = iter(batches)
        first = next(it, None)
        if first is None:
            return
        nxt, pending, i = stage(first, 0), None, 0
        while nxt is not None:
            cur = nxt
            hb = next(it, None)
            nxt = stage(hb, (i + 1) & 1) if hb is not None else None
            main.wait_event(cur["copied"])
            cur["g"].replay()
            if on_device is not None:
                on_device(cur["s_probs"], i)
            cur["host_out"].copy_(cur["s_probs"], non_blocking=True)
            cur["done"].record(main)
            self.last_logits = cur["s_logits"]
            if pending is not None:
                pending["done"].synchronize()
                yield pending["host_out"].clone()
            pending, i = cur, i + 1
        pending["done"].synchronize()
        yield pending["host_out"].clone()

    def compile(self, optimizer=None, loss=None, metrics=None, top_k: int = 5, **_):
        self._top_k = int(top_k)
        return self

    def evaluate(self, dataset, group=None, return_dict: bool = True, verbose: int = 0):
        device = self._device or torch.device("cuda", torch.cuda.current_device())
        acc = torch.zeros(4, dtype=torch.float64, device=device)
        labels_dev: List[torch.Tensor] = []
        k = getattr(self, "_top_k", 5)

        def clips_only():
            for clips, labels in dataset:
                lab = torch.as_tensor(np.asarray(labels).reshape(-1), dtype=torch.int32)
                if lab.numel() * self._num_preds != clips.shape[0]:
                    raise ValueError(f"{clips.shape[0]} clips need {clips.shape[0] // self._num_preds} "
                                     f"labels, got {lab.numel()}")
                labels_dev.append(lab.to(device))
                yield clips

        def on_device(probs, i):
            ops.eval_metrics(probs, labels_dev[i], acc, k)
            labels_dev[i] = None

        n = 0
        for _ in self.predict(clips_only(), on_device=on_device):
            n += 1
            if verbose:
                print(f"\r{n} batches", end="", flush=True)
        return finalize_metrics(acc, group, k, return_dict)

    def summary(self, input_shape) -> str:
        T, H, W, _ = input_shape
        plan = A.plan_shapes(self._arch, T, H, W)
        rows = [("input_1 (InputLayer)", f"[(None, {T}, {H}, {W}, {input_shape[3]})]", 0),
                ("conv_1 (X3D_Stem)", f"(None, {T}, {plan.stem.H}, {plan.stem.W}, {self._conv1_dim})",
                 self.conv1.count_params())]
        for s, st in enumerate(self.stages):
            lv = plan.stages[s]
            rows.append((f"res_stage_{s + 2} (ResStage)",
                         f"(None, {T}, {lv.H}, {lv.W}, {st.out_channels})", st.count_params()))
        lv = plan.stages[-1]
        rows += [("conv_5 (Sequential)", f"(None, {T}, {lv.H}, {lv.W}, {self.conv5.cout})",
                  self.conv5.count_params()),
                 ("pool_5 (AdaptiveAvgPool3D)", f"(None, 1, 1, 1, {self.conv5.cout})", 0),
                 ("fc_1 (Conv3D)", "(None, 1, 1, 1, 2048)", self.fc1.count_params()),
                 ("dropout (Dropout)", "(None, 1, 1, 1, 2048)", 0),
                 ("fc_2 (Dense)", f"(None, 1, 1, 1, {self.num_classes})", self.fc2.count_params())]
        total = self.count_params()
        nontrain = sum(int(v.size) for k, v in self.named_variables().items()
                       if not A.is_trainable(k))
        lines = ['Model: "X3D"', "_" * 65, f"{'Layer (type)':<29}{'Output Shape':<26}Param #",
                 "=" * 65]
        for name, shape, n in rows:
            lines += [f"{name:<29}{shape:<26}{n}", "_" * 65]
        lines[-1] = "=" * 65
        lines += [f"Total params: {total:,}", f"Trainable params: {total - nontrain:,}",
                  f"Non-trainable params: {nontrain:,}", "_" * 65]
        text = "\n".join(lines)
        print(text)
        return text
```

### x3d_tf_b200/ops.py

```python
from __future__ import annotations

from typing import Optional, Tuple

import torch

from . import _lib
from ._lib import X3D_BF16, X3D_F32, PwArgs, PwTcArgs, check, lib


class Profiler:
    enabled = False
    tag = ""
    records: list = []
    launches = 0

    @classmethod
    def start(cls):
        cls.enabled, cls.records, cls.launches = True, [], 0

    @classmethod
    def stop(cls):
        cls.enabled = False
        torch.cuda.synchronize()
        out = [(tag, name, e0.elapsed_time(e1)) for tag, name, e0, e1 in cls.records]
        cls.records = []
        return out


def _launch(name: str, fn) -> None:
    Profiler.launches += 1
    if Profiler.enabled:
        e0 = torch.cuda.Event(enable_timing=True)
        e1 = torch.cuda.Event(enable_timing=True)
        e0.record()
        status = fn()
        e1.record()
        Profiler.records.append((Profiler.tag, name, e0, e1))
    else:
        status = fn()
    check(status, name)


def _dt(t: torch.Tensor) -> int:
    if t.dtype == torch.float32:
        return X3D_F32
    if t.dtype == torch.bfloat16:
        return X3D_BF16
    raise TypeError(f"unsupported activation dtype {t.dtype} (float32 or bfloat16)")


def _torch_dt(code: int):
    return torch.float32 if code == X3D_F32 else torch.bfloat16


def _stream() -> int:
    return torch.cuda.current_stream().cuda_stream


def _req(t: torch.Tensor, name: str) -> torch.Tensor:
    if not t.is_cuda:
        raise ValueError(f"{name} must be a CUDA tensor (there is no CPU path)")
    if not t.is_contiguous():
        raise ValueError(f"{name} must be contiguous")
    return t


def _ptr(t: Optional[torch.Tensor]) -> Optional[int]:
    return None if t is None else t.data_ptr()


def stem_fwd(x: torch.Tensor, ws: torch.Tensor, wt: torch.Tensor, bias: torch.Tensor,
             out_dtype: torch.dtype) -> torch.Tensor:
    _req(x, "x")
    N, T, H, W, ci = x.shape
    if ci != 3:
        raise ValueError("stem input must have 3 channels")
    C = bias.numel()
    Ho, Wo = (H - 1) // 2 + 1, (W - 1) // 2 + 1
    out = torch.empty((N, T, Ho, Wo, C), dtype=out_dtype, device=x.device)
    _launch("x3d_stem_fwd", lambda: lib().x3d_stem_fwd(x.data_ptr(), _dt(x), ws.data_ptr(), wt.data_ptr(), bias.data_ptr(),
                             out.data_ptr(), _dt(out), N, T, H, W, C, wt.shape[0], _stream()))
    return out


def stem_tc_fwd(x: torch.Tensor, wc: torch.Tensor, bias: torch.Tensor) -> torch.Tensor:
    _req(x, "x")
    N, T, H, W, ci = x.shape
    if ci != 3:
        raise ValueError("stem input must have 3 channels")
    C = bias.numel()
    Ho, Wo = (H - 1) // 2 + 1, (W - 1) // 2 + 1
    out = torch.empty((N, T, Ho, Wo, C), dtype=torch.bfloat16, device=x.device)
    _launch("x3d_stem_tc_fwd", lambda: lib().x3d_stem_tc_fwd(
        x.data_ptr(), _dt(x), wc.data_ptr(), bias.data_ptr(), out.data_ptr(), N, T, H, W, C,
        wc.shape[0], _stream()))
    return out


def _f3(vals) -> "_lib.C.Array":
    v = [float(x) for x in vals]
    if len(v) != 3:
        raise ValueError("mean / std must have 3 entries (RGB)")
    return (_lib.C.c_float * 3)(*v)


def normalize_u8(x: torch.Tensor, mean, std, out_dtype: torch.dtype, norm_value: float = 255.0) -> torch.Tensor:
    _req(x, "x")
    if x.dtype != torch.uint8 or x.shape[-1] != 3:
        raise TypeError("normalize_u8 needs uint8 clips with 3 channels")
    out = torch.empty(x.shape, dtype=out_dtype, device=x.device)
    _launch("x3d_normalize_u8", lambda: lib().x3d_normalize_u8(
        x.data_ptr(), out.data_ptr(), x.numel() // 3, _f3(mean), _f3(std), float(norm_value), _dt(out), _stream()))
    return out


def eval_views_u8(video: torch.Tensor, T: int, views: int, crops: int, size: int) -> torch.Tensor:
    _req(video, "video")
    if video.dtype != torch.uint8 or video.dim() != 4 or video.shape[-1] != 3:
        raise TypeError("eval_views_u8 needs a [F,H,W,3] uint8 video")
    F, H, W, _ = video.shape
    out = torch.empty((crops * views, T, size, size, 3), dtype=torch.uint8, device=video.device)
    _launch("x3d_eval_views_u8", lambda: lib().x3d_eval_views_u8(video.data_ptr(), out.data_ptr(), F, H, W, T, views,
                                                               crops, size, _stream()))
    return out


def stem_tc_u8_fwd(x: torch.Tensor, mean, std, wc: torch.Tensor, bias: torch.Tensor,
                   norm_value: float = 255.0) -> torch.Tensor:
    _req(x, "x")
    if x.dtype != torch.uint8 or x.shape[-1] != 3:
        raise TypeError("stem_tc_u8_fwd needs uint8 clips with 3 channels")
    N, T, H, W, _ = x.shape
    C = bias.numel()
    Ho, Wo = (H - 1) // 2 + 1, (W - 1) // 2 + 1
    out = torch.empty((N, T, Ho, Wo, C), dtype=torch.bfloat16, device=x.device)
    _launch("x3d_stem_tc_u8_fwd", lambda: lib().x3d_stem_tc_u8_fwd(
        x.data_ptr(), _f3(mean), _f3(std), float(norm_value), wc.data_ptr(), bias.data_ptr(), out.data_ptr(),
        N, T, H, W, C, wc.shape[0], _stream()))
    return out


def eval_metrics(probs: torch.Tensor, labels: torch.Tensor, acc: torch.Tensor, k: int = 5) -> None:
    _req(probs, "probs"); _req(labels, "labels"); _req(acc, "acc")
    if probs.dtype != torch.float32 or labels.dtype != torch.int32 or acc.dtype != torch.float64:
        raise TypeError("eval_metrics: probs fp32, labels int32, acc fp64")
    V, ncls = probs.shape
    if labels.numel() != V or acc.numel() < 4:
        raise ValueError(f"eval_metrics: {V} videos but {labels.numel()} labels / acc of {acc.numel()}")
    _launch("x3d_eval_metrics", lambda: lib().x3d_eval_metrics(
        probs.data_ptr(), labels.data_ptr(), acc.data_ptr(), V, ncls, int(k), _stream()))


def pw_fwd(a: torch.Tensor, wt: torch.Tensor, bias: Optional[torch.Tensor], *, M: int, K: int,
           Nc: int, out: Optional[torch.Tensor] = None, out_dtype: Optional[torch.dtype] = None,
           residual: Optional[torch.Tensor] = None, se: Optional[torch.Tensor] = None,
           rows_per_clip: int = 0, swish: bool = False, relu: bool = False,
           gather: Optional[Tuple[int, int, int, int, int, int]] = None) -> torch.Tensor:
    _req(a, "a")
    if out is None:
        out = torch.empty((M, Nc), dtype=out_dtype or a.dtype, device=a.device)
    args = PwArgs()
    args.A, args.Wt, args.bias = a.data_ptr(), wt.data_ptr(), _ptr(bias)
    args.R, args.se, args.D = _ptr(residual), _ptr(se), out.data_ptr()
    args.M, args.K, args.Nc = M, K, Nc
    args.lda, args.ldw, args.ldr, args.ldd = K, wt.shape[1], Nc, Nc
    args.rows_per_clip = rows_per_clip
    args.a_dtype, args.d_dtype = _dt(a), _dt(out)
    args.swish, args.relu = int(swish), int(relu)
    if gather is not None:
        args.gather = 1
        args.T, args.Ho, args.Wo, args.Hi, args.Wi, args.stride = gather
    _launch("x3d_pw_fwd", lambda: lib().x3d_pw_fwd(args, _stream()))
    return out


def pw_tc_fwd(a: torch.Tensor, wp: torch.Tensor, bias: Optional[torch.Tensor], *, M: int, K: int,
              Nc: int, out: Optional[torch.Tensor] = None, residual: Optional[torch.Tensor] = None,
              se: Optional[torch.Tensor] = None, rows_per_clip: int = 0, swish: bool = False,
              relu: bool = False, a2: Optional[torch.Tensor] = None, a2_stride: int = 1,
              colmean: bool = False, store: bool = True):
    _req(a, "a")
    if a.dtype != torch.bfloat16:
        raise TypeError("pw_tc_fwd needs bf16 activations")
    if not store and not colmean:
        raise ValueError("pw_tc_fwd: store=False only together with colmean=True")
    if out is None:
        out = torch.empty((M if store else 128, Nc), dtype=torch.bfloat16, device=a.device)
    means = torch.empty((2 * -(-M // 128), Nc), dtype=torch.float32, device=a.device) if colmean else None
    args = PwTcArgs()
    args.A, args.Wp, args.bias = a.data_ptr(), wp.data_ptr(), _ptr(bias)
    args.R, args.se, args.D = _ptr(residual), _ptr(se), out.data_ptr()
    args.colmean, args.store_d = _ptr(means), int(store)
    args.M, args.K, args.Nc = M, K, Nc
    args.lda, args.ldr, args.ldd = K, Nc, Nc
    args.Npad, args.Kpad = wp.shape
    args.rows_per_clip = rows_per_clip
    args.swish, args.relu = int(swish), int(relu)
    if a2 is not None:
        _req(a2, "a2")
        if a2.dtype != torch.bfloat16 or a2.dim() not in (2, 5):
            raise TypeError("pw_tc_fwd: a2 must be a bf16 [N,T,H,W,C] tensor or a dense [M,C] matrix")
        if a2.dim() == 5:
            args.A2, args.a2_nt, args.K2 = a2.data_ptr(), a2.shape[0] * a2.shape[1], a2.shape[4]
            args.a2_stride, args.a2_hi, args.a2_wi = a2_stride, a2.shape[2], a2.shape[3]
        else:
            if a2.shape[0] != M:
                raise ValueError("pw_tc_fwd: dense a2 needs M rows")
            args.A2, args.K2, args.a2_stride = a2.data_ptr(), a2.shape[1], 0
    _launch("x3d_pw_tc_fwd", lambda: lib().x3d_pw_tc_fwd(args, _stream()))
    if colmean:
        return (out, means) if store else means
    return out


def pw_tc_sampler_supported(Hi: int, Wi: int, stride: int) -> bool:
    return bool(lib().x3d_pw_tc_sampler_supported(Hi, Wi, stride))


def gather_rows_fwd(x: torch.Tensor, stride: int) -> torch.Tensor:
    _req(x, "x")
    N, T, H, W, C = x.shape
    Ho, Wo = (H - 1) // stride + 1, (W - 1) // stride + 1
    out = torch.empty((N * T * Ho * Wo, C), dtype=x.dtype, device=x.device)
    _launch("x3d_gather_rows_fwd", lambda: lib().x3d_gather_rows_fwd(
        x.data_ptr(), out.data_ptr(), N * T, H, W, stride, C, _dt(x), _stream()))
    return out


def head_fc_fwd(a: torch.Tensor, wt: torch.Tensor, bias: Optional[torch.Tensor], *, K: int, Nc: int,
                relu: bool = False) -> torch.Tensor:
    _req(a, "a")
    if a.dtype != torch.float32:
        raise TypeError("head_fc_fwd needs float32 input")
    M = a.shape[0]
    out = torch.empty((M, Nc), dtype=torch.float32, device=a.device)
    _launch("x3d_head_fc_fwd", lambda: lib().x3d_head_fc_fwd(
        a.data_ptr(), wt.data_ptr(), _ptr(bias), out.data_ptr(), M, K, Nc, a.shape[1], wt.shape[1],
        Nc, int(relu), _stream()))
    return out


def dw_fwd(x: torch.Tensor, w: torch.Tensor, bias: torch.Tensor, stride: int, pad_h: int,
           pad_w: int, want_se: bool, swish: bool = False) -> Tuple[torch.Tensor, Optional[torch.Tensor]]:
    _req(x, "x")
    if swish and want_se:
        raise ValueError("swish can only be fused when no SE sums are requested")
    N, T, H, W, C = x.shape
    Ho, Wo = -(-H // stride), -(-W // stride)
    out = torch.empty((N, T, Ho, Wo, C), dtype=x.dtype, device=x.device)
    partial = None
    if want_se:
        nblk = lib().x3d_dw_partial_blocks(T, H, W, C, stride, _dt(x))
        if nblk <= 0:
            raise _lib.X3DLibError("x3d_dw_partial_blocks rejected the shape")
        partial = torch.empty((N, nblk, C), dtype=torch.float32, device=x.device)
    _launch("x3d_dw3x3x3_fwd", lambda: lib().x3d_dw3x3x3_act_fwd(x.data_ptr(), w.data_ptr(), bias.data_ptr(), out.data_ptr(),
                                _ptr(partial), N, T, H, W, C, stride, pad_h, pad_w, _dt(x), int(swish),
                                _stream()))
    return out, partial


def dw_planar_taps(w: torch.Tensor, bias: torch.Tensor) -> torch.Tensor:
    C = w.shape[1]
    t = torch.cat([w, bias.view(1, C)], 0)
    return t.view(28, C // 2, 2).permute(1, 0, 2).contiguous()


def dw_planar_supported(T: int, H: int, W: int, c: int, stride: int) -> int:
    if c % 8 or c // 2 > 288:
        return 0
    return int(lib().x3d_dw_planar_partial_blocks(T, H, W, c, stride))


def dw_planar_lane_use(T: int, H: int, W: int, c: int, stride: int) -> float:
    if c % 8 or c // 2 > 288:
        return 0.0
    return int(lib().x3d_dw_planar_lane_permille(T, H, W, c, stride)) / 1000.0


def dw_planar_fwd(x: torch.Tensor, taps: torch.Tensor, stride: int, pad_h: int, pad_w: int, want_se: bool,
                  swish: bool = False) -> Tuple[torch.Tensor, Optional[torch.Tensor]]:
    _req(x, "x")
    if x.dtype != torch.bfloat16:
        raise TypeError("dw_planar_fwd needs bf16 activations")
    if swish and want_se:
        raise ValueError("swish in the epilogue only without SE (the SE scale comes before the swish)")
    N, T, H, W, C = x.shape
    Ho, Wo = -(-H // stride), -(-W // stride)
    out = torch.empty((N, T, Ho, Wo, C), dtype=x.dtype, device=x.device)
    partial = None
    if want_se:
        nblk = dw_planar_supported(T, H, W, C, stride)
        if nblk <= 0:
            raise _lib.X3DLibError("x3d_dw_planar_partial_blocks rejected the shape")
        partial = torch.empty((N, nblk, C), dtype=torch.float32, device=x.device)
    _launch("x3d_dw3x3x3_planar_fwd", lambda: lib().x3d_dw3x3x3_planar_fwd(
        x.data_ptr(), taps.data_ptr(), out.data_ptr(), _ptr(partial), N, T, H, W, C, stride, pad_h, pad_w,
        1 if swish else 0, _stream()))
    return out, partial


def expand_dw_supported(T: int, H: int, W: int, cin: int, c: int, stride: int) -> int:
    return int(lib().x3d_expand_dw_partial_blocks(T, H, W, cin, c, stride))


def expand_dw_fwd(x: torch.Tensor, wa: torch.Tensor, bias_a: torch.Tensor, wb: torch.Tensor,
                  bias_b: torch.Tensor, stride: int, pad_h: int, pad_w: int,
                  want_se: bool) -> Tuple[torch.Tensor, Optional[torch.Tensor]]:
    _req(x, "x")
    if x.dtype != torch.bfloat16:
        raise TypeError("expand_dw_fwd needs bf16 activations")
    N, T, H, W, cin = x.shape
    C = wb.shape[1]
    Ho, Wo = -(-H // stride), -(-W // stride)
    out = torch.empty((N, T, Ho, Wo, C), dtype=x.dtype, device=x.device)
    partial = None
    if want_se:
        nblk = expand_dw_supported(T, H, W, cin, C, stride)
        if nblk <= 0:
            raise _lib.X3DLibError("x3d_expand_dw_partial_blocks rejected the shape")
        partial = torch.empty((N, nblk, C), dtype=torch.float32, device=x.device)
    npad, kpad = wa.shape
    _launch("x3d_expand_dw_fwd", lambda: lib().x3d_expand_dw_fwd(
        x.data_ptr(), wa.data_ptr(), bias_a.data_ptr(), wb.data_ptr(), bias_b.data_ptr(),
        out.data_ptr(), _ptr(partial), N, T, H, W, cin, C, kpad, npad, stride, pad_h, pad_w,
        _stream()))
    return out, partial


def pw_tf32(a: torch.Tensor, w: torch.Tensor, bias: Optional[torch.Tensor] = None, *, relu: bool = False,
            transpose_w: bool = True, M: Optional[int] = None, stats: Optional[torch.Tensor] = None) -> torch.Tensor:
    _req(a, "a")
    _req(w, "w")
    if a.dtype != torch.float32 or w.dtype != torch.float32:
        raise TypeError("pw_tf32 needs fp32 operands")
    K, N = w.shape
    red, nout = (K, N) if transpose_w else (N, K)
    M = a.shape[0] if M is None else M
    lda = a.shape[-1]
    if lda < red:
        raise ValueError(f"a has {lda} columns, the reduction needs {red}")
    bs = torch.empty((2, nout, red), dtype=torch.float32, device=a.device)
    _launch("x3d_tf32_split", lambda: lib().x3d_tf32_split(w.data_ptr(), bs.data_ptr(), nout, red, N,
                                                         1 if transpose_w else 0, _stream()))
    out = torch.empty((M, nout), dtype=torch.float32, device=a.device)
    _launch("x3d_pw_tf32_fwd", lambda: lib().x3d_pw_tf32_fwd(a.data_ptr(), bs.data_ptr(), _ptr(bias), out.data_ptr(),
                                                           M, red, nout, lda, nout, 1 if relu else 0, _ptr(stats),
                                                           _stream()))
    return out


def expand_dw2_supported(T: int, H: int, W: int, cin: int, c: int, stride: int) -> int:
    return int(lib().x3d_expand_dw2_partial_blocks(T, H, W, cin, c, stride))


def expand_dw2_fwd(x: torch.Tensor, wa: torch.Tensor, bias_a: torch.Tensor, wb: torch.Tensor,
                   bias_b: torch.Tensor, stride: int, pad_h: int, pad_w: int, want_se: bool,
                   swish: bool = False) -> Tuple[torch.Tensor, Optional[torch.Tensor]]:
    _req(x, "x")
    if x.dtype != torch.bfloat16:
        raise TypeError("expand_dw2_fwd needs bf16 activations")
    if swish and want_se:
        raise ValueError("swish in the epilogue only without SE (the SE scale comes before the swish)")
    N, T, H, W, cin = x.shape
    C = wb.shape[1]
    Ho, Wo = -(-H // stride), -(-W // stride)
    out = torch.empty((N, T, Ho, Wo, C), dtype=x.dtype, device=x.device)
    partial = None
    if want_se:
        nblk = expand_dw2_supported(T, H, W, cin, C, stride)
        if nblk <= 0:
            raise _lib.X3DLibError("x3d_expand_dw2_partial_blocks rejected the shape")
        partial = torch.empty((N, nblk, C), dtype=torch.float32, device=x.device)
    npad, kpad = wa.shape
    _launch("x3d_expand_dw2_fwd", lambda: lib().x3d_expand_dw2_fwd(
        x.data_ptr(), wa.data_ptr(), bias_a.data_ptr(), wb.data_ptr(), bias_b.data_ptr(),
        out.data_ptr(), _ptr(partial), N, T, H, W, cin, C, kpad, npad, stride, pad_h, pad_w,
        1 if swish else 0, _stream()))
    return out, partial


def se_mlp_fwd(partial: torch.Tensor, count: int, w1: torch.Tensor, b1: torch.Tensor,
               w2: torch.Tensor, b2: torch.Tensor) -> torch.Tensor:
    N, nblk, C = partial.shape
    scale = torch.empty((N, C), dtype=torch.float32, device=partial.device)
    _launch("x3d_se_mlp_fwd", lambda: lib().x3d_se_mlp_fwd(partial.data_ptr(), nblk, 1.0 / float(count), w1.data_ptr(),
                               b1.data_ptr(), w2.data_ptr(), b2.data_ptr(), scale.data_ptr(),
                               N, C, w1.shape[1], _stream()))
    return scale


def avgpool_fwd(x: torch.Tensor) -> torch.Tensor:
    _req(x, "x")
    N, C = x.shape[0], x.shape[-1]
    P = x.numel() // (N * C)
    out = torch.empty((N, C), dtype=torch.float32, device=x.device)
    _launch("x3d_avgpool_fwd", lambda: lib().x3d_avgpool_fwd(x.data_ptr(), out.data_ptr(), N, P, C, _dt(x), _stream()))
    return out


def softmax_viewmean_fwd(logits: torch.Tensor, num_preds: int) -> torch.Tensor:
    _req(logits, "logits")
    N, ncls = logits.shape
    if N % num_preds:
        raise ValueError(f"batch {N} is not a multiple of num_preds {num_preds}")
    probs = torch.empty((N // num_preds, ncls), dtype=torch.float32, device=logits.device)
    _launch("x3d_softmax_viewmean_fwd", lambda: lib().x3d_softmax_viewmean_fwd(logits.data_ptr(), probs.data_ptr(), N, ncls, num_preds,
                                         _stream()))
    return probs
```

Before: 8323.

## Chain block projection GEMM with next block's expand GEMM in one kernel

New measurement: 8440, median of 6. +1.4%, better.

```diff
diff --git a/include/x3d_b200.h b/include/x3d_b200.h
--- a/include/x3d_b200.h
+++ b/include/x3d_b200.h
@@ -84,6 +84,18 @@
 int x3d_pw_tc_fwd(const x3d_pw_tc_args* args, void* stream);
 int x3d_pw_tc_sampler_supported(int Hi, int Wi, int stride);
 
+typedef struct x3d_pw_tc_chain_args {
+  const void* A; const void* Wp; const float* bias; const void* R; const float* se; void* D;
+  int64_t M; int32_t K, Nc, lda, ldr, ldd, Kpad, Npad;
+  int64_t rows_per_clip;
+  int32_t swish, relu;
+  const void* A2; int64_t a2_nt; int32_t K2, a2_stride, a2_hi, a2_wi;
+  const void* Wp2; const float* bias2; void* D2;
+  int32_t Nc2, ldd2, Kpad2, Npad2, pair2, relu2;
+} x3d_pw_tc_chain_args;
+int x3d_pw_tc_chain_fwd(const x3d_pw_tc_chain_args* args, void* stream);
+int x3d_pw_tc_chain_supported(int K, int K2, int Nc, int Nc2, int pair2);
+
 int x3d_expand_dw_partial_blocks(int T, int H, int W, int Cin, int C, int stride);
 int x3d_expand_dw_fwd(const void* x, const void* wa, const float* bias_a, const float* wb,
                       const float* bias_b, void* out, float* se_partial, int N, int T, int H,
diff --git a/x3d_tf_b200/_lib.py b/x3d_tf_b200/_lib.py
--- a/x3d_tf_b200/_lib.py
+++ b/x3d_tf_b200/_lib.py
@@ -36,6 +36,19 @@
                 ("colmean", C.c_void_p), ("store_d", C.c_int32), ("reserved", C.c_int32)]
 
 
+class PwTcChainArgs(C.Structure):
+    _fields_ = [("A", C.c_void_p), ("Wp", C.c_void_p), ("bias", C.c_void_p), ("R", C.c_void_p),
+                ("se", C.c_void_p), ("D", C.c_void_p),
+                ("M", C.c_int64), ("K", C.c_int32), ("Nc", C.c_int32), ("lda", C.c_int32),
+                ("ldr", C.c_int32), ("ldd", C.c_int32), ("Kpad", C.c_int32), ("Npad", C.c_int32),
+                ("rows_per_clip", C.c_int64), ("swish", C.c_int32), ("relu", C.c_int32),
+                ("A2", C.c_void_p), ("a2_nt", C.c_int64), ("K2", C.c_int32), ("a2_stride", C.c_int32),
+                ("a2_hi", C.c_int32), ("a2_wi", C.c_int32),
+                ("Wp2", C.c_void_p), ("bias2", C.c_void_p), ("D2", C.c_void_p),
+                ("Nc2", C.c_int32), ("ldd2", C.c_int32), ("Kpad2", C.c_int32), ("Npad2", C.c_int32),
+                ("pair2", C.c_int32), ("relu2", C.c_int32)]
+
+
 SIGNATURES = {
     "x3d_version": (C.c_int, []),
     "x3d_last_error": (C.c_char_p, []),
@@ -67,6 +80,8 @@
                                            C.c_void_p]),
     "x3d_pw_tc_fwd": (C.c_int, [C.POINTER(PwTcArgs), C.c_void_p]),
     "x3d_pw_tc_sampler_supported": (C.c_int, [C.c_int] * 3),
+    "x3d_pw_tc_chain_fwd": (C.c_int, [C.POINTER(PwTcChainArgs), C.c_void_p]),
+    "x3d_pw_tc_chain_supported": (C.c_int, [C.c_int] * 5),
     "x3d_gather_rows_fwd": (C.c_int, [C.c_void_p, C.c_void_p, C.c_int, C.c_int, C.c_int, C.c_int,
                                       C.c_int, C.c_int, C.c_void_p]),
     "x3d_expand_dw_partial_blocks": (C.c_int, [C.c_int] * 6),
diff --git a/x3d_tf_b200/csrc/x3d_pw_tc.cu b/x3d_tf_b200/csrc/x3d_pw_tc.cu
--- a/x3d_tf_b200/csrc/x3d_pw_tc.cu
+++ b/x3d_tf_b200/csrc/x3d_pw_tc.cu
@@ -89,8 +89,203 @@
 
 constexpr int kEpiWarps = 8, kProWarps = 8, kOutBufs = 4;
 constexpr int kProGroups = 2;
-constexpr int kProRows = 8 * kProWarps / kProGroups / 2;
 constexpr int kThreadsPlain = 64 + 32 * kEpiWarps, kThreadsPro = kThreadsPlain + 32 * kProWarps;
+
+struct TileRange { long lo, hi, stride; };
+__device__ __forceinline__ TileRange cta_tiles(const Params& p) {
+  const long num_tiles = (p.M + kBlockM - 1) / kBlockM;
+  TileRange r{blockIdx.x, num_tiles, gridDim.x};
+  if (p.contiguous) {
+    const long t_per = num_tiles / gridDim.x, t_rem = num_tiles % gridDim.x;
+    r.lo = blockIdx.x * t_per + (blockIdx.x < t_rem ? blockIdx.x : t_rem);
+    r.hi = r.lo + t_per + (blockIdx.x < t_rem ? 1 : 0);
+    r.stride = 1;
+  }
+  return r;
+}
+
+__device__ __forceinline__ void produce_a(const Params& p, const TileRange& tr, const CUtensorMap* tmA,
+                                          const CUtensorMap* tmA2, uint8_t* sA, uint64_t* full, uint64_t* empty) {
+  int s = 0;
+  uint32_t ph = 0;
+  for (long tile = tr.lo; tile < tr.hi; tile += tr.stride) {
+    const int row0 = static_cast<int>(tile * kBlockM);
+    int nt0 = 0, ho0 = 0;
+    if (p.a2_ppf) {
+      nt0 = row0 / p.a2_ppf;
+      ho0 = (row0 - nt0 * p.a2_ppf) / p.a2_wo;
+    }
+    for (int kc = 0; kc < p.KC; ++kc) {
+      mbar_wait(&empty[s], ph ^ 1);
+      mbar_expect_tx(&full[s], kStageBytes);
+      if (kc < p.KC1) tma_load_2d(sA + s * kStageBytes, tmA, kc * kBlockK, row0, &full[s]);
+      else if (p.a2_ppf) tma_load_4d(smem_u32(sA + s * kStageBytes), tmA2, (kc - p.KC1) * kBlockK, 0, ho0, nt0, &full[s]);
+      else tma_load_2d(sA + s * kStageBytes, tmA2, (kc - p.KC1) * kBlockK, row0, &full[s]);
+      if (++s == p.stages) { s = 0; ph ^= 1; }
+    }
+  }
+}
+
+__device__ __forceinline__ void mma_tile(const Params& p, uint8_t* sA, uint8_t* sW, uint64_t* ready, uint64_t* empty,
+                                         uint64_t* acc_full, uint32_t d_tmem, uint32_t idesc, int& s, uint32_t& ph) {
+  for (int kc = 0; kc < p.KC; ++kc) {
+    mbar_wait(&ready[s], ph);
+    tcgen05_after_sync();
+    if (elect_one()) {
+      const uint32_t a_addr = smem_u32(sA + s * kStageBytes);
+      const uint32_t b_addr = smem_u32(sW + kc * p.NT * 128);
+      const int nk = (kc == p.KC - 1) ? p.k16_last : (kc == p.KC1 - 1 ? p.k16_last1 : 4);
+      for (int k = 0; k < nk; ++k)
+        umma_bf16(d_tmem, make_desc_sw128(a_addr + k * 32), make_desc_sw128(b_addr + k * 32),
+                  idesc, (kc | k) != 0 ? 1u : 0u);
+      umma_commit(&empty[s]);
+      if (kc == p.KC - 1) umma_commit(acc_full);
+    }
+    __syncwarp();
+    if (++s == p.stages) { s = 0; ph ^= 1; }
+  }
+}
+
+__device__ __forceinline__ uint4 epi_pack8(const uint32_t* v, uint32_t bias_addr, bool has_r, uint4 ru, bool relu) {
+  const __nv_bfloat162 zero2 = __floats2bfloat162_rn(0.f, 0.f);
+  float4 b0, b1;
+  asm volatile("ld.shared.v4.f32 {%0, %1, %2, %3}, [%4];" : "=f"(b0.x), "=f"(b0.y), "=f"(b0.z), "=f"(b0.w) : "r"(bias_addr));
+  asm volatile("ld.shared.v4.f32 {%0, %1, %2, %3}, [%4];" : "=f"(b1.x), "=f"(b1.y), "=f"(b1.z), "=f"(b1.w) : "r"(bias_addr + 16));
+  float2 y[4];
+  y[0] = __fadd2_rn(make_float2(__uint_as_float(v[0]), __uint_as_float(v[1])), make_float2(b0.x, b0.y));
+  y[1] = __fadd2_rn(make_float2(__uint_as_float(v[2]), __uint_as_float(v[3])), make_float2(b0.z, b0.w));
+  y[2] = __fadd2_rn(make_float2(__uint_as_float(v[4]), __uint_as_float(v[5])), make_float2(b1.x, b1.y));
+  y[3] = __fadd2_rn(make_float2(__uint_as_float(v[6]), __uint_as_float(v[7])), make_float2(b1.z, b1.w));
+  if (has_r) {
+    const uint32_t rw[4] = {ru.x, ru.y, ru.z, ru.w};
+#pragma unroll
+    for (int j = 0; j < 4; ++j)
+      y[j] = __fadd2_rn(y[j], make_float2(__uint_as_float(rw[j] << 16), __uint_as_float(rw[j] & 0xffff0000u)));
+  }
+  uint32_t o[4];
+#pragma unroll
+  for (int j = 0; j < 4; ++j) {
+    __nv_bfloat162 t = __float22bfloat162_rn(y[j]);
+    if (relu) t = __hmax2(t, zero2);
+    o[j] = *reinterpret_cast<uint32_t*>(&t);
+  }
+  return make_uint4(o[0], o[1], o[2], o[3]);
+}
+__device__ __forceinline__ void st_shared16(uint32_t addr, uint4 o) {
+  asm volatile("st.shared.v4.b32 [%0], {%1, %2, %3, %4};" ::"r"(addr), "r"(o.x), "r"(o.y), "r"(o.z), "r"(o.w) : "memory");
+}
+
+__device__ __forceinline__ void prologue_transform(const Params& p, const TileRange& tr, int tt, uint8_t* sA,
+                                                   uint64_t* full, uint64_t* xform) {
+  pdl_wait();
+  pdl_trigger();
+  const long tile_hi = tr.hi, t_stride = tr.stride;
+  constexpr int kGT = 32 * kProWarps / kProGroups;
+  const int grp = tt / kGT;
+  const int pchunk = tt & 7;
+  const int rbase = (tt % kGT) >> 3;
+  const int kin = (pchunk ^ (rbase & 7)) << 3;
+  const uint32_t rpc = static_cast<uint32_t>(p.rows_per_clip > 0 ? p.rows_per_clip : 0x7fffffff);
+  const uint32_t step = static_cast<uint32_t>(t_stride) * kBlockM;
+  struct Pos { long tile; int kc; uint32_t clip, rem; };
+  auto advance = [&](Pos& q) {
+    if (++q.kc == p.KC) {
+      q.kc = 0;
+      q.tile += t_stride;
+      q.rem += step;
+      while (q.rem >= rpc) { q.rem -= rpc; ++q.clip; }
+    }
+  };
+  auto se_request = [&](const Pos& q, float4& s0, float4& s1) {
+    s0 = make_float4(1.f, 1.f, 1.f, 1.f);
+    s1 = s0;
+    const int k = q.kc * kBlockK + kin;
+    if (p.se != nullptr && q.tile < tile_hi && k < p.Kc && q.kc < p.KC1 && q.rem + kBlockM <= rpc) {
+      const float4* sp = reinterpret_cast<const float4*>(p.se + static_cast<long>(q.clip) * p.Kc + k);
+      s0 = __ldg(sp);
+      s1 = __ldg(sp + 1);
+    }
+  };
+  Pos cur;
+  cur.tile = tr.lo; cur.kc = 0;
+  cur.clip = static_cast<uint32_t>(tr.lo * static_cast<long>(kBlockM) / rpc);
+  cur.rem = static_cast<uint32_t>(tr.lo * static_cast<long>(kBlockM) - static_cast<long>(cur.clip) * rpc);
+  int s = 0;
+  uint32_t ph = 0;
+  for (int g = 0; g < grp; ++g) {
+    advance(cur);
+    if (++s == p.stages) { s = 0; ph ^= 1; }
+  }
+  float4 nx0, nx1;
+  se_request(cur, nx0, nx1);
+  while (cur.tile < tile_hi) {
+    const uint32_t clip0 = cur.clip, rem0 = cur.rem;
+    const bool one_clip = rem0 + kBlockM <= rpc;
+    const int k = cur.kc * kBlockK + kin;
+    const bool k_ok = k < p.Kc && cur.kc < p.KC1;
+    float2 sc[4];
+    sc[0] = make_float2(nx0.x, nx0.y); sc[1] = make_float2(nx0.z, nx0.w);
+    sc[2] = make_float2(nx1.x, nx1.y); sc[3] = make_float2(nx1.z, nx1.w);
+#pragma unroll
+    for (int g = 0; g < kProGroups; ++g) advance(cur);
+    se_request(cur, nx0, nx1);
+    mbar_wait(&full[s], ph);
+    if (k_ok) {
+      const uint32_t addr0 = smem_u32(sA + s * kStageBytes) + rbase * 128 + pchunk * 16;
+      float2 hs[4];
+#pragma unroll
+      for (int j = 0; j < 4; ++j) hs[j] = __fmul2_rn(sc[j], make_float2(0.5f, 0.5f));
+#pragma unroll
+      for (int half = 0; half < kBlockM / (kGT / 8) / 4; ++half) {
+        uint32_t w[4][4];
+#pragma unroll
+        for (int i = 0; i < 4; ++i)
+          asm volatile("ld.shared.v4.b32 {%0, %1, %2, %3}, [%4];"
+                       : "=r"(w[i][0]), "=r"(w[i][1]), "=r"(w[i][2]), "=r"(w[i][3])
+                       : "r"(addr0 + (half * 4 + i) * (kGT / 8 * 128)));
+#pragma unroll
+        for (int i = 0; i < 4; ++i) {
+          if (p.se && !one_clip) {
+            uint32_t x = rem0 + rbase + (kGT / 8) * (half * 4 + i), clip = clip0;
+            while (x >= rpc) { x -= rpc; ++clip; }
+            if (static_cast<long>(clip) * rpc + x < p.M) {
+              const float4* sp = reinterpret_cast<const float4*>(p.se + static_cast<long>(clip) * p.Kc + k);
+              const float4 s0 = __ldg(sp), s1 = __ldg(sp + 1);
+              sc[0] = make_float2(s0.x, s0.y); sc[1] = make_float2(s0.z, s0.w);
+              sc[2] = make_float2(s1.x, s1.y); sc[3] = make_float2(s1.z, s1.w);
+#pragma unroll
+              for (int j = 0; j < 4; ++j) hs[j] = __fmul2_rn(sc[j], make_float2(0.5f, 0.5f));
+            }
+          }
+          if (p.swish) {
+#pragma unroll
+            for (int j = 0; j < 4; ++j) {
+              const float2 h = __fmul2_rn(make_float2(__uint_as_float(w[i][j] << 16), __uint_as_float(w[i][j] & 0xffff0000u)), hs[j]);
+              float2 t;
+              asm("tanh.approx.f32 %0, %1;" : "=f"(t.x) : "f"(h.x));
+              asm("tanh.approx.f32 %0, %1;" : "=f"(t.y) : "f"(h.y));
+              __nv_bfloat162 t2 = __float22bfloat162_rn(__ffma2_rn(h, t, h));
+              w[i][j] = *reinterpret_cast<uint32_t*>(&t2);
+            }
+          } else {
+#pragma unroll
+            for (int j = 0; j < 4; ++j) {
+              const float2 scj = make_float2(2.f * hs[j].x, 2.f * hs[j].y);
+              __nv_bfloat162 t2 = __float22bfloat162_rn(__fmul2_rn(
+                  make_float2(__uint_as_float(w[i][j] << 16), __uint_as_float(w[i][j] & 0xffff0000u)), scj));
+              w[i][j] = *reinterpret_cast<uint32_t*>(&t2);
+            }
+          }
+          asm volatile("st.shared.v4.b32 [%0], {%1, %2, %3, %4};" ::"r"(addr0 + (half * 4 + i) * (kGT / 8 * 128)), "r"(w[i][0]), "r"(w[i][1]), "r"(w[i][2]), "r"(w[i][3]) : "memory");
+        }
+      }
+    }
+    fence_proxy_async();
+    mbar_arrive(&xform[s]);
+    s += kProGroups;
+    while (s >= p.stages) { s -= p.stages; ph ^= 1; }
+  }
+}
 
 template <bool kPro>
 __global__ void __launch_bounds__(kPro ? kThreadsPro : kThreadsPlain, 1)
@@ -150,14 +345,8 @@
   tcgen05_after_sync();
   const uint32_t tmem_base = *tmem_slot;
 
-  const long num_tiles = (p.M + kBlockM - 1) / kBlockM;
-  long tile_lo = blockIdx.x, tile_hi = num_tiles, t_stride = gridDim.x;
-  if (p.contiguous) {
-    const long t_per = num_tiles / gridDim.x, t_rem = num_tiles % gridDim.x;
-    tile_lo = blockIdx.x * t_per + (blockIdx.x < t_rem ? blockIdx.x : t_rem);
-    tile_hi = tile_lo + t_per + (blockIdx.x < t_rem ? 1 : 0);
-    t_stride = 1;
-  }
+  const TileRange tr = cta_tiles(p);
+  const long tile_lo = tr.lo, tile_hi = tr.hi, t_stride = tr.stride;
 
   if (warp == 0) {
     if (elect_one()) {
@@ -166,24 +355,7 @@
         tma_load_2d(sW + kc * w_chunk_bytes, &tmW, kc * kBlockK, n0, w_full);
       pdl_wait();
       pdl_trigger();
-      int s = 0;
-      uint32_t ph = 0;
-      for (long tile = tile_lo; tile < tile_hi; tile += t_stride) {
-        const int row0 = static_cast<int>(tile * kBlockM);
-        int nt0 = 0, ho0 = 0;
-        if (p.a2_ppf) {
-          nt0 = row0 / p.a2_ppf;
-          ho0 = (row0 - nt0 * p.a2_ppf) / p.a2_wo;
-        }
-        for (int kc = 0; kc < p.KC; ++kc) {
-          mbar_wait(&empty[s], ph ^ 1);
-          mbar_expect_tx(&full[s], kStageBytes);
-          if (kc < p.KC1) tma_load_2d(sA + s * kStageBytes, &tmA, kc * kBlockK, row0, &full[s]);
-          else if (p.a2_ppf) tma_load_4d(smem_u32(sA + s * kStageBytes), &tmA2, (kc - p.KC1) * kBlockK, 0, ho0, nt0, &full[s]);
-          else tma_load_2d(sA + s * kStageBytes, &tmA2, (kc - p.KC1) * kBlockK, row0, &full[s]);
-          if (++s == p.stages) { s = 0; ph ^= 1; }
-        }
-      }
+      produce_a(p, tr, &tmA, &tmA2, sA, full, empty);
     }
   } else if (warp == 1) {
     pdl_trigger();
@@ -197,23 +369,8 @@
       const uint32_t aph = static_cast<uint32_t>((it >> 1) & 1);
       mbar_wait(&t_empty[as], aph ^ 1);
       tcgen05_after_sync();
-      const uint32_t d_tmem = tmem_base + static_cast<uint32_t>(as * p.NT);
-      for (int kc = 0; kc < p.KC; ++kc) {
-        mbar_wait(kPro ? &xform[s] : &full[s], ph);
-        tcgen05_after_sync();
-        if (elect_one()) {
-          const uint32_t a_addr = smem_u32(sA + s * kStageBytes);
-          const uint32_t b_addr = smem_u32(sW + kc * w_chunk_bytes);
-          const int nk = (kc == p.KC - 1) ? p.k16_last : (kc == p.KC1 - 1 ? p.k16_last1 : 4);
-          for (int k = 0; k < nk; ++k)
-            umma_bf16(d_tmem, make_desc_sw128(a_addr + k * 32), make_desc_sw128(b_addr + k * 32),
-                      idesc, (kc | k) != 0 ? 1u : 0u);
-          umma_commit(&empty[s]);
-          if (kc == p.KC - 1) umma_commit(&t_full[as]);
-        }
-        __syncwarp();
-        if (++s == p.stages) { s = 0; ph ^= 1; }
-      }
+      mma_tile(p, sA, sW, kPro ? xform : full, empty, &t_full[as], tmem_base + static_cast<uint32_t>(as * p.NT),
+               idesc, s, ph);
     }
   } else if (warp < 2 + kEpiWarps) {
     pdl_wait();
@@ -221,7 +378,6 @@
     const int q = warp & 3;
     const int grp = (warp - 2) >> 2;
     const bool leader = q == 2 && lane == 0;
-    const __nv_bfloat162 zero2 = __floats2bfloat162_rn(0.f, 0.f);
     const int r_loc = q * 32 + lane;
     const uint32_t sw_row = static_cast<uint32_t>(r_loc) * 128, sw_x = static_cast<uint32_t>(r_loc & 7);
     const int n_sub = (p.NT + 63) >> 6;
@@ -279,32 +435,9 @@
 #pragma unroll
           for (int h = 0; h < 2; ++h) {
             const int cc = c0 + h * 8;
-            float4 b0, b1;
-            asm volatile("ld.shared.v4.f32 {%0, %1, %2, %3}, [%4];" : "=f"(b0.x), "=f"(b0.y), "=f"(b0.z), "=f"(b0.w) : "r"(bias_s + cc * 4));
-            asm volatile("ld.shared.v4.f32 {%0, %1, %2, %3}, [%4];" : "=f"(b1.x), "=f"(b1.y), "=f"(b1.z), "=f"(b1.w) : "r"(bias_s + cc * 4 + 16));
-            float2 y[4];
-            y[0] = __fadd2_rn(make_float2(__uint_as_float(v[h * 8 + 0]), __uint_as_float(v[h * 8 + 1])), make_float2(b0.x, b0.y));
-            y[1] = __fadd2_rn(make_float2(__uint_as_float(v[h * 8 + 2]), __uint_as_float(v[h * 8 + 3])), make_float2(b0.z, b0.w));
-            y[2] = __fadd2_rn(make_float2(__uint_as_float(v[h * 8 + 4]), __uint_as_float(v[h * 8 + 5])), make_float2(b1.x, b1.y));
-            y[3] = __fadd2_rn(make_float2(__uint_as_float(v[h * 8 + 6]), __uint_as_float(v[h * 8 + 7])), make_float2(b1.z, b1.w));
-            if (p.R) {
-              const uint4 ru = rr[g * 2 + h];
-              const uint32_t rw[4] = {ru.x, ru.y, ru.z, ru.w};
-#pragma unroll
-              for (int j = 0; j < 4; ++j)
-                y[j] = __fadd2_rn(y[j], make_float2(__uint_as_float(rw[j] << 16),
-                                                    __uint_as_float(rw[j] & 0xffff0000u)));
-            }
-            uint32_t o[4];
-#pragma unroll
-            for (int j = 0; j < 4; ++j) {
-              __nv_bfloat162 t = __float22bfloat162_rn(y[j]);
-              if (p.relu) t = __hmax2(t, zero2);
-              o[j] = *reinterpret_cast<uint32_t*>(&t);
-            }
+            const uint4 o = epi_pack8(v + h * 8, bias_s + cc * 4, p.R != nullptr, rr[g * 2 + h], p.relu);
             const uint32_t chunk = static_cast<uint32_t>(g * 2 + h);
-            asm volatile("st.shared.v4.b32 [%0], {%1, %2, %3, %4};" ::"r"(buf + ((chunk ^ sw_x) << 4)),
-                         "r"(o[0]), "r"(o[1]), "r"(o[2]), "r"(o[3]) : "memory");
+            st_shared16(buf + ((chunk ^ sw_x) << 4), o);
           }
         }
         X3D_TRACE(2);
@@ -350,114 +483,289 @@
     }
     if (leader) tma_store_wait_read<0>();
   } else if (kPro) {
+    prologue_transform(p, tr, threadIdx.x - kThreadsPlain, sA, full, xform);
+  }
+
+  tcgen05_before_sync();
+  __syncthreads();
+  if (warp == 1) {
+    asm volatile("tcgen05.dealloc.cta_group::1.sync.aligned.b32 %0, %1;" ::"r"(tmem_base),
+                 "r"(static_cast<uint32_t>(p.tmem_cols))
+                 : "memory");
+  }
+}
+
+struct ChainParams {
+  Params c;
+  const float* bias2;
+  int Nc2, NT2;
+  int KCy, k16_y;
+  int pair;
+  int ny;
+  int nd2;
+  int relu2;
+};
+constexpr int kChainEpi2Warps = 4;
+constexpr int kChainThreadsPlain = 64 + 32 * (kEpiWarps + kChainEpi2Warps);
+constexpr int kChainThreadsPro = kChainThreadsPlain + 32 * kProWarps;
+
+template <bool kPro>
+__global__ void __launch_bounds__(kPro ? kChainThreadsPro : kChainThreadsPlain, 1)
+pw_tc_chain_kernel(const __grid_constant__ CUtensorMap tmA, const __grid_constant__ CUtensorMap tmW,
+                   const __grid_constant__ CUtensorMap tmD, const __grid_constant__ CUtensorMap tmA2,
+                   const __grid_constant__ CUtensorMap tmW2, const __grid_constant__ CUtensorMap tmZ,
+                   const ChainParams cp) {
+  extern __shared__ __align__(1024) uint8_t smem_raw[];
+  uint8_t* smem = reinterpret_cast<uint8_t*>((reinterpret_cast<uintptr_t>(smem_raw) + 1023) &
+                                             ~static_cast<uintptr_t>(1023));
+  const Params& p = cp.c;
+  const int warp = threadIdx.x >> 5, lane = threadIdx.x & 31;
+  const int y_slot_bytes = cp.KCy * kStageBytes;
+
+  uint8_t* sW = smem;
+  uint8_t* sW2 = sW + p.KC * p.NT * 128;
+  uint8_t* sA = sW2 + cp.KCy * cp.NT2 * 128;
+  uint8_t* sY = sA + p.stages * kStageBytes;
+  uint8_t* sS = sY + cp.ny * y_slot_bytes;
+  uint8_t* sO = sS + (cp.pair ? cp.ny * kStageBytes : 0);
+  float* sBias = reinterpret_cast<float*>(sO + 2 * kStageBytes);
+  float* sBias2 = sBias + 256;
+  uint64_t* bars = reinterpret_cast<uint64_t*>(sBias2 + 256);
+  uint64_t* full = bars;
+  uint64_t* empty = full + p.stages;
+  uint64_t* xform = empty + p.stages;
+  uint64_t* w_full = xform + p.stages;
+  uint64_t* t_full = w_full + 1;
+  uint64_t* t_empty = t_full + 2;
+  uint64_t* y_full = t_empty + 2;
+  uint64_t* y_free = y_full + 2;
+  uint64_t* z_full = y_free + 2;
+  uint64_t* z_empty = z_full + 2;
+  uint32_t* tmem_slot = reinterpret_cast<uint32_t*>(z_empty + 2);
+
+  for (int i = threadIdx.x; i < 256; i += blockDim.x) {
+    sBias[i] = (p.bias != nullptr && i < p.Nc) ? p.bias[i] : 0.f;
+    sBias2[i] = (cp.bias2 != nullptr && i < cp.Nc2) ? cp.bias2[i] : 0.f;
+  }
+  if (warp == 0 && elect_one()) {
+    prefetch_tmap(&tmA);
+    prefetch_tmap(&tmW);
+    prefetch_tmap(&tmD);
+    prefetch_tmap(&tmW2);
+    prefetch_tmap(&tmZ);
+    if (p.KC > p.KC1) prefetch_tmap(&tmA2);
+    for (int s = 0; s < p.stages; ++s) {
+      mbar_init(&full[s], 1);
+      mbar_init(&empty[s], 1);
+      mbar_init(&xform[s], 32 * kProWarps / kProGroups);
+    }
+    mbar_init(w_full, 1);
+    for (int i = 0; i < 2; ++i) {
+      mbar_init(&t_full[i], 1);
+      mbar_init(&t_empty[i], 16 * kEpiWarps);
+      mbar_init(&y_full[i], 16 * kEpiWarps);
+      mbar_init(&y_free[i], 2);
+      mbar_init(&z_full[i], 1);
+      mbar_init(&z_empty[i], 32 * kChainEpi2Warps);
+    }
+    fence_barrier_init();
+  }
+  if (warp == 1) {
+    asm volatile("tcgen05.alloc.cta_group::1.sync.aligned.shared::cta.b32 [%0], %1;" ::"r"(
+                     smem_u32(tmem_slot)),
+                 "r"(static_cast<uint32_t>(p.tmem_cols))
+                 : "memory");
+    asm volatile("tcgen05.relinquish_alloc_permit.cta_group::1.sync.aligned;" ::: "memory");
+  }
+  tcgen05_before_sync();
+  __syncthreads();
+  tcgen05_after_sync();
+  const uint32_t tmem_base = *tmem_slot;
+  const uint32_t z_col = static_cast<uint32_t>(2 * p.NT);
+
+  const TileRange tr = cta_tiles(p);
+  if (warp == 0) {
+    if (elect_one()) {
+      mbar_expect_tx(w_full, static_cast<uint32_t>((p.KC * p.NT + cp.KCy * cp.NT2) * 128));
+      for (int kc = 0; kc < p.KC; ++kc) tma_load_2d(sW + kc * p.NT * 128, &tmW, kc * kBlockK, 0, w_full);
+      for (int kc = 0; kc < cp.KCy; ++kc) tma_load_2d(sW2 + kc * cp.NT2 * 128, &tmW2, kc * kBlockK, 0, w_full);
+      pdl_wait();
+      pdl_trigger();
+      produce_a(p, tr, &tmA, &tmA2, sA, full, empty);
+    }
+  } else if (warp == 1) {
+    pdl_trigger();
+    const uint32_t idesc = make_idesc_bf16(p.NT), idesc2 = make_idesc_bf16(cp.NT2);
+    mbar_wait(w_full, 0);
+    auto expand_mma = [&](long j) {
+      const int ys = cp.ny == 2 ? static_cast<int>(j & 1) : 0;
+      const long yu = cp.ny == 2 ? (j >> 1) : j;
+      const int zs = cp.nd2 == 2 ? static_cast<int>(j & 1) : 0;
+      const long zu = cp.nd2 == 2 ? (j >> 1) : j;
+      mbar_wait(&y_full[ys], static_cast<uint32_t>(yu & 1));
+      mbar_wait(&z_empty[zs], static_cast<uint32_t>((zu & 1) ^ 1));
+      tcgen05_after_sync();
+      if (elect_one()) {
+        const uint32_t d = tmem_base + z_col + static_cast<uint32_t>(zs * cp.NT2);
+        for (int kc = 0; kc < cp.KCy; ++kc) {
+          const uint32_t a_addr = smem_u32(sY + ys * y_slot_bytes + kc * kStageBytes);
+          const uint32_t b_addr = smem_u32(sW2 + kc * cp.NT2 * 128);
+          const int nk = kc == cp.KCy - 1 ? cp.k16_y : 4;
+          for (int k = 0; k < nk; ++k)
+            umma_bf16(d, make_desc_sw128(a_addr + k * 32), make_desc_sw128(b_addr + k * 32), idesc2,
+                      (kc | k) != 0 ? 1u : 0u);
+        }
+        umma_commit(&z_full[zs]);
+        umma_commit(&y_free[ys]);
+      }
+      __syncwarp();
+    };
+    int s = 0;
+    uint32_t ph = 0;
+    long it = 0;
+    for (long tile = tr.lo; tile < tr.hi; tile += tr.stride, ++it) {
+      const int as = static_cast<int>(it & 1);
+      mbar_wait(&t_empty[as], static_cast<uint32_t>(((it >> 1) & 1) ^ 1));
+      tcgen05_after_sync();
+      mma_tile(p, sA, sW, kPro ? xform : full, empty, &t_full[as], tmem_base + static_cast<uint32_t>(as * p.NT),
+               idesc, s, ph);
+      if (it > 0) expand_mma(it - 1);
+    }
+    if (it > 0) expand_mma(it - 1);
+  } else if (warp < 2 + kEpiWarps) {
     pdl_wait();
     pdl_trigger();
-    const int tt = threadIdx.x - kThreadsPlain;
-    constexpr int kGT = 32 * kProWarps / kProGroups;
-    const int grp = tt / kGT;
-    const int pchunk = tt & 7;
-    const int rbase = (tt % kGT) >> 3;
-    const int kin = (pchunk ^ (rbase & 7)) << 3;
-    const uint32_t rpc = static_cast<uint32_t>(p.rows_per_clip > 0 ? p.rows_per_clip : 0x7fffffff);
-    const uint32_t step = static_cast<uint32_t>(t_stride) * kBlockM;
-    struct Pos { long tile; int kc; uint32_t clip, rem; };
-    auto advance = [&](Pos& q) {
-      if (++q.kc == p.KC) {
-        q.kc = 0;
-        q.tile += t_stride;
-        q.rem += step;
-        while (q.rem >= rpc) { q.rem -= rpc; ++q.clip; }
+    const int q = warp & 3;
+    const int grp = (warp - 2) >> 2;
+    const bool leader = q == 2 && lane == 0;
+    const int r_loc = q * 32 + lane;
+    const uint32_t sw_row = static_cast<uint32_t>(r_loc) * 128, sw_x = static_cast<uint32_t>(r_loc & 7);
+    const int n_sub = (p.NT + 63) >> 6;
+    const uint32_t bias_s = smem_u32(sBias);
+    const uint32_t taddr = tmem_base + (static_cast<uint32_t>(q * 32) << 16) + static_cast<uint32_t>(grp * p.NT);
+    const uint32_t pair_chunks = static_cast<uint32_t>(p.Nc >> 3);
+    const uint32_t pair_sh = (r_loc & 1) * pair_chunks, pair_zero = (1 - (r_loc & 1)) * pair_chunks;
+    const uint4 z4 = make_uint4(0, 0, 0, 0);
+    uint32_t aph = 0;
+    long it = grp;
+    for (long tile = tr.lo + grp * tr.stride; tile < tr.hi; tile += 2 * tr.stride, it += 2, aph ^= 1) {
+      const long row = tile * kBlockM + r_loc;
+      const bool row_ok = row < p.M;
+      const bf16* rrow = (p.R && row_ok) ? p.R + row * p.ldr : nullptr;
+      uint4 rr[8];
+#pragma unroll
+      for (int c = 0; c < 8; ++c)
+        rr[c] = (rrow && c * 8 < p.Nc) ? __ldg(reinterpret_cast<const uint4*>(rrow + c * 8)) : z4;
+      if (p.R) {
+        const long nrow = row + 2L * tr.stride * kBlockM;
+        if (nrow < p.M && tile + 2 * tr.stride < tr.hi) {
+          const char* np_ = reinterpret_cast<const char*>(p.R + nrow * p.ldr);
+          for (int off = 0; off < p.Nc * 2; off += 128)
+            asm volatile("prefetch.global.L2 [%0];" ::"l"(np_ + off));
+        }
       }
-    };
-    auto se_request = [&](const Pos& q, float4& s0, float4& s1) {
-      s0 = make_float4(1.f, 1.f, 1.f, 1.f);
-      s1 = s0;
-      const int k = q.kc * kBlockK + kin;
-      if (p.se != nullptr && q.tile < tile_hi && k < p.Kc && q.kc < p.KC1 && q.rem + kBlockM <= rpc) {
-        const float4* sp = reinterpret_cast<const float4*>(p.se + static_cast<long>(q.clip) * p.Kc + k);
-        s0 = __ldg(sp);
-        s1 = __ldg(sp + 1);
+      const int ys = cp.ny == 2 ? grp : 0;
+      const long yu = cp.ny == 2 ? (it >> 1) : it;
+      const uint32_t yslot = smem_u32(sY + ys * y_slot_bytes) + sw_row;
+      const uint32_t sslot = cp.pair ? smem_u32(sS + ys * kStageBytes) : smem_u32(sY + ys * y_slot_bytes);
+      mbar_wait(&t_full[grp], aph);
+      tcgen05_after_sync();
+      mbar_wait(&y_free[ys], static_cast<uint32_t>((yu & 1) ^ 1));
+      for (int sb = 0; sb < n_sub; ++sb) {
+        if (sb > 0) {
+#pragma unroll
+          for (int c = 0; c < 8; ++c) {
+            const int cc = sb * 64 + c * 8;
+            rr[c] = (rrow && cc < p.Nc) ? __ldg(reinterpret_cast<const uint4*>(rrow + cc)) : z4;
+          }
+        }
+#pragma unroll
+        for (int g = 0; g < 4; ++g) {
+          const int c0 = sb * 64 + g * 16;
+          if (c0 >= p.NT) continue;
+          uint32_t v[16];
+          tmem_ld16(taddr + c0, v);
+          tmem_ld_wait();
+#pragma unroll
+          for (int h = 0; h < 2; ++h) {
+            const int cc = c0 + h * 8;
+            const uint4 o = cc < p.Nc ? epi_pack8(v + h * 8, bias_s + cc * 4, p.R != nullptr, rr[g * 2 + h], p.relu) : z4;
+            const uint32_t chunk = static_cast<uint32_t>(g * 2 + h);
+            if (cp.pair) {
+              st_shared16(sslot + sw_row + ((chunk ^ sw_x) << 4), o);
+              st_shared16(yslot + (((chunk + pair_sh) ^ sw_x) << 4), o);
+              if (chunk < pair_chunks) st_shared16(yslot + (((chunk + pair_zero) ^ sw_x) << 4), z4);
+            } else {
+              st_shared16(yslot + sb * kStageBytes + ((chunk ^ sw_x) << 4), o);
+            }
+          }
+        }
       }
-    };
-    Pos cur;
-    cur.tile = tile_lo; cur.kc = 0;
-    cur.clip = static_cast<uint32_t>(tile_lo * static_cast<long>(kBlockM) / rpc);
-    cur.rem = static_cast<uint32_t>(tile_lo * static_cast<long>(kBlockM) - static_cast<long>(cur.clip) * rpc);
-    int s = 0;
-    uint32_t ph = 0;
-    for (int g = 0; g < grp; ++g) {
-      advance(cur);
-      if (++s == p.stages) { s = 0; ph ^= 1; }
-    }
-    float4 nx0, nx1;
-    se_request(cur, nx0, nx1);
-    while (cur.tile < tile_hi) {
-      const uint32_t clip0 = cur.clip, rem0 = cur.rem;
-      const bool one_clip = rem0 + kBlockM <= rpc;
-      const int k = cur.kc * kBlockK + kin;
-      const bool k_ok = k < p.Kc && cur.kc < p.KC1;
-      float2 sc[4];
-      sc[0] = make_float2(nx0.x, nx0.y); sc[1] = make_float2(nx0.z, nx0.w);
-      sc[2] = make_float2(nx1.x, nx1.y); sc[3] = make_float2(nx1.z, nx1.w);
-#pragma unroll
-      for (int g = 0; g < kProGroups; ++g) advance(cur);
-      se_request(cur, nx0, nx1);
-      mbar_wait(&full[s], ph);
-      if (k_ok) {
-        const uint32_t addr0 = smem_u32(sA + s * kStageBytes) + rbase * 128 + pchunk * 16;
-        float2 hs[4];
-#pragma unroll
-        for (int j = 0; j < 4; ++j) hs[j] = __fmul2_rn(sc[j], make_float2(0.5f, 0.5f));
-#pragma unroll
-        for (int half = 0; half < kBlockM / (kGT / 8) / 4; ++half) {
-          uint32_t w[4][4];
-#pragma unroll
-          for (int i = 0; i < 4; ++i)
-            asm volatile("ld.shared.v4.b32 {%0, %1, %2, %3}, [%4];"
-                         : "=r"(w[i][0]), "=r"(w[i][1]), "=r"(w[i][2]), "=r"(w[i][3])
-                         : "r"(addr0 + (half * 4 + i) * (kGT / 8 * 128)));
-#pragma unroll
-          for (int i = 0; i < 4; ++i) {
-            if (p.se && !one_clip) {
-              uint32_t x = rem0 + rbase + (kGT / 8) * (half * 4 + i), clip = clip0;
-              while (x >= rpc) { x -= rpc; ++clip; }
-              if (static_cast<long>(clip) * rpc + x < p.M) {
-                const float4* sp = reinterpret_cast<const float4*>(p.se + static_cast<long>(clip) * p.Kc + k);
-                const float4 s0 = __ldg(sp), s1 = __ldg(sp + 1);
-                sc[0] = make_float2(s0.x, s0.y); sc[1] = make_float2(s0.z, s0.w);
-                sc[2] = make_float2(s1.x, s1.y); sc[3] = make_float2(s1.z, s1.w);
-#pragma unroll
-                for (int j = 0; j < 4; ++j) hs[j] = __fmul2_rn(sc[j], make_float2(0.5f, 0.5f));
-              }
-            }
-            if (p.swish) {
-#pragma unroll
-              for (int j = 0; j < 4; ++j) {
-                const float2 h = __fmul2_rn(make_float2(__uint_as_float(w[i][j] << 16), __uint_as_float(w[i][j] & 0xffff0000u)), hs[j]);
-                float2 t;
-                asm("tanh.approx.f32 %0, %1;" : "=f"(t.x) : "f"(h.x));
-                asm("tanh.approx.f32 %0, %1;" : "=f"(t.y) : "f"(h.y));
-                __nv_bfloat162 t2 = __float22bfloat162_rn(__ffma2_rn(h, t, h));
-                w[i][j] = *reinterpret_cast<uint32_t*>(&t2);
-              }
-            } else {
-#pragma unroll
-              for (int j = 0; j < 4; ++j) {
-                const float2 scj = make_float2(2.f * hs[j].x, 2.f * hs[j].y);
-                __nv_bfloat162 t2 = __float22bfloat162_rn(__fmul2_rn(
-                    make_float2(__uint_as_float(w[i][j] << 16), __uint_as_float(w[i][j] & 0xffff0000u)), scj));
-                w[i][j] = *reinterpret_cast<uint32_t*>(&t2);
-              }
-            }
-            asm volatile("st.shared.v4.b32 [%0], {%1, %2, %3, %4};" ::"r"(addr0 + (half * 4 + i) * (kGT / 8 * 128)), "r"(w[i][0]), "r"(w[i][1]), "r"(w[i][2]), "r"(w[i][3]) : "memory");
+      tcgen05_before_sync();
+      mbar_arrive(&t_empty[grp]);
+      fence_proxy_async();
+      mbar_arrive(&y_full[ys]);
+      if (grp == 0) asm volatile("bar.sync 1, 128;" ::: "memory");
+      else asm volatile("bar.sync 2, 128;" ::: "memory");
+      if (leader) {
+        for (int sb = 0; sb < n_sub; ++sb)
+          tma_store_2d(&tmD, sslot + sb * kStageBytes, sb * 64, static_cast<int>(tile * kBlockM));
+        tma_store_commit();
+        tma_store_wait_read<0>();
+        mbar_arrive(&y_free[ys]);
+      }
+    }
+  } else if (warp < 2 + kEpiWarps + kChainEpi2Warps) {
+    pdl_wait();
+    pdl_trigger();
+    const int q = warp & 3;
+    const bool leader = warp == 2 + kEpiWarps && lane == 0;
+    const int r_loc = q * 32 + lane;
+    const uint32_t sw_row = static_cast<uint32_t>(r_loc) * 128, sw_x = static_cast<uint32_t>(r_loc & 7);
+    const int n_sub = (cp.NT2 + 63) >> 6;
+    const uint32_t bias_s = smem_u32(sBias2);
+    const uint32_t stage0 = smem_u32(sO);
+    const uint4 z4 = make_uint4(0, 0, 0, 0);
+    uint32_t sub_ctr = 0;
+    long j = 0;
+    for (long tile = tr.lo; tile < tr.hi; tile += tr.stride, ++j) {
+      const int zs = cp.nd2 == 2 ? static_cast<int>(j & 1) : 0;
+      const long zu = cp.nd2 == 2 ? (j >> 1) : j;
+      const uint32_t taddr = tmem_base + (static_cast<uint32_t>(q * 32) << 16) + z_col +
+                             static_cast<uint32_t>(zs * cp.NT2);
+      mbar_wait(&z_full[zs], static_cast<uint32_t>(zu & 1));
+      tcgen05_after_sync();
+      for (int sb = 0; sb < n_sub; ++sb, ++sub_ctr) {
+        const uint32_t buf = stage0 + (sub_ctr & 1) * kStageBytes + sw_row;
+#pragma unroll
+        for (int g = 0; g < 4; ++g) {
+          const int c0 = sb * 64 + g * 16;
+          if (c0 >= cp.NT2) continue;
+          uint32_t v[16];
+          tmem_ld16(taddr + c0, v);
+          tmem_ld_wait();
+#pragma unroll
+          for (int h = 0; h < 2; ++h) {
+            const uint4 o = epi_pack8(v + h * 8, bias_s + (c0 + h * 8) * 4, false, z4, cp.relu2);
+            st_shared16(buf + (((g * 2 + h) ^ sw_x) << 4), o);
           }
         }
+        if (sb == n_sub - 1) {
+          tcgen05_before_sync();
+          mbar_arrive(&z_empty[zs]);
+        }
+        fence_proxy_async();
+        if (leader) tma_store_wait_read<0>();
+        asm volatile("bar.sync 3, 128;" ::: "memory");
+        if (leader) {
+          tma_store_2d(&tmZ, stage0 + (sub_ctr & 1) * kStageBytes, sb * 64, static_cast<int>(tile * kBlockM));
+          tma_store_commit();
+        }
       }
-      fence_proxy_async();
-      mbar_arrive(&xform[s]);
-      s += kProGroups;
-      while (s >= p.stages) { s -= p.stages; ph ^= 1; }
-    }
+    }
+    if (leader) tma_store_wait_read<0>();
+  } else if (kPro) {
+    prologue_transform(p, tr, threadIdx.x - kChainThreadsPlain, sA, full, xform);
   }
 
   tcgen05_before_sync();
@@ -505,10 +813,139 @@
   return true;
 }
 
+struct ChainPlan {
+  int NT, KC, KC1, k16_last, k16_last1, NT2, KCy, k16_y, stages, ny, nd2, tmem_cols;
+  size_t smem;
+};
+constexpr int kSmemSm100 = 227 * 1024;
+static bool chain_plan(int K, int K2, int Nc, int Nc2, int pair, ChainPlan* pl) {
+  if (K <= 0 || Nc <= 0 || Nc2 <= 0 || K2 < 0 || K % 8 || K2 % 8 || Nc % 8 || Nc2 % 8) return false;
+  pl->NT = (Nc + 15) / 16 * 16;
+  pl->NT2 = (Nc2 + 15) / 16 * 16;
+  if (pl->NT > 256 || pl->NT2 > 256 || (pair && 2 * Nc > kBlockK)) return false;
+  const int k16 = (K + 15) / 16;
+  pl->KC1 = pl->KC = (k16 + 3) / 4;
+  pl->k16_last1 = pl->k16_last = k16 - (pl->KC1 - 1) * 4;
+  if (K2 > 0) {
+    const int k16_2 = (K2 + 15) / 16, KC2 = (k16_2 + 3) / 4;
+    pl->KC += KC2;
+    pl->k16_last = k16_2 - (KC2 - 1) * 4;
+  }
+  const int k16y = ((pair ? 2 * Nc : Nc) + 15) / 16;
+  pl->KCy = (k16y + 3) / 4;
+  pl->k16_y = k16y - (pl->KCy - 1) * 4;
+  if (2 * pl->NT + pl->NT2 > 512) return false;
+  pl->nd2 = 2 * pl->NT + 2 * pl->NT2 <= 512 ? 2 : 1;
+  pl->tmem_cols = 32;
+  while (pl->tmem_cols < 2 * pl->NT + pl->nd2 * pl->NT2) pl->tmem_cols *= 2;
+  const size_t fixed = 1024  + 2048  + 512  + (size_t)pl->KC * pl->NT * 128 +
+                       (size_t)pl->KCy * pl->NT2 * 128 + 2 * kStageBytes ;
+  const size_t slot = (size_t)pl->KCy * kStageBytes + (pair ? kStageBytes : 0);
+  for (pl->ny = 2; pl->ny >= 1; --pl->ny) {
+    const size_t used = fixed + pl->ny * slot;
+    pl->stages = used < (size_t)kSmemSm100 ? static_cast<int>((kSmemSm100 - used) / kStageBytes) : 0;
+    if (pl->stages >= (pl->ny == 2 ? 3 : 2)) break;
+  }
+  if (pl->ny < 1) return false;
+  if (pl->stages > 8) pl->stages = 8;
+  pl->smem = fixed + pl->ny * slot + (size_t)pl->stages * kStageBytes;
+  return true;
+}
+
 }
 }
 
 using namespace x3d;
+
+extern "C" int x3d_pw_tc_chain_supported(int K, int K2, int Nc, int Nc2, int pair2) {
+  tc::ChainPlan pl;
+  return tc::chain_plan(K, K2, Nc, Nc2, pair2, &pl) ? 1 : 0;
+}
+
+extern "C" int x3d_pw_tc_chain_fwd(const x3d_pw_tc_chain_args* a, void* stream) {
+  X3D_REQUIRE(a && a->A && a->Wp && a->D && a->Wp2 && a->D2, X3D_ERR_INVALID_ARG, "x3d_pw_tc_chain_fwd: null pointer");
+  X3D_REQUIRE(a->M > 0 && a->M < (1L << 31), X3D_ERR_INVALID_ARG, "x3d_pw_tc_chain_fwd: M out of range");
+  X3D_REQUIRE(a->K > 0 && a->K % 8 == 0 && a->lda % 8 == 0 && a->lda >= a->K, X3D_ERR_INVALID_ARG,
+              "x3d_pw_tc_chain_fwd: K=%d / lda=%d must be multiples of 8", a->K, a->lda);
+  X3D_REQUIRE(a->Nc > 0 && a->Nc % 8 == 0 && a->ldd % 8 == 0 && a->ldd >= a->Nc && (!a->R || a->ldr % 8 == 0) &&
+              a->Nc2 > 0 && a->Nc2 % 8 == 0 && a->ldd2 % 8 == 0 && a->ldd2 >= a->Nc2,
+              X3D_ERR_INVALID_ARG, "x3d_pw_tc_chain_fwd: Nc/Nc2/ldd/ldd2/ldr must be multiples of 8");
+  X3D_REQUIRE(!a->se || a->rows_per_clip > 0, X3D_ERR_INVALID_ARG, "x3d_pw_tc_chain_fwd: rows_per_clip missing");
+  X3D_REQUIRE(!a->pair2 || a->M % 2 == 0, X3D_ERR_INVALID_ARG, "x3d_pw_tc_chain_fwd: pixel-pair form needs an even M");
+  X3D_REQUIRE((reinterpret_cast<uintptr_t>(a->A) & 15) == 0 && (reinterpret_cast<uintptr_t>(a->Wp) & 15) == 0 &&
+              (reinterpret_cast<uintptr_t>(a->D) & 15) == 0 && (reinterpret_cast<uintptr_t>(a->Wp2) & 15) == 0 &&
+              (reinterpret_cast<uintptr_t>(a->D2) & 15) == 0 && (reinterpret_cast<uintptr_t>(a->R) & 15) == 0,
+              X3D_ERR_INVALID_ARG, "x3d_pw_tc_chain_fwd: pointers must be 16-byte aligned");
+  X3D_REQUIRE(device_sm_count() > 0 && device_is_sm100(), X3D_ERR_NO_DEVICE, "x3d_pw_tc_chain_fwd: needs an sm_100 device");
+  const int K2 = a->A2 ? a->K2 : 0;
+  tc::ChainPlan pl;
+  X3D_REQUIRE(tc::chain_plan(a->K, K2, a->Nc, a->Nc2, a->pair2, &pl) && (size_t)device_max_smem() >= pl.smem,
+              X3D_ERR_UNSUPPORTED, "x3d_pw_tc_chain_fwd: K=%d K2=%d Nc=%d Nc2=%d pair=%d does not fit (x3d_pw_tc_chain_supported)",
+              a->K, K2, a->Nc, a->Nc2, a->pair2);
+  X3D_REQUIRE(a->Kpad % 64 == 0 && a->Kpad >= pl.KC * 64 && a->Npad % 16 == 0 && a->Npad >= pl.NT,
+              X3D_ERR_INVALID_ARG, "x3d_pw_tc_chain_fwd: bad packed projection weight extents Kpad=%d Npad=%d", a->Kpad, a->Npad);
+  X3D_REQUIRE(a->Kpad2 % 64 == 0 && a->Kpad2 >= pl.KCy * 64 && a->Npad2 % 16 == 0 && a->Npad2 >= pl.NT2,
+              X3D_ERR_INVALID_ARG, "x3d_pw_tc_chain_fwd: bad packed expand weight extents Kpad2=%d Npad2=%d", a->Kpad2, a->Npad2);
+  int a2_bh = 0, a2_bf = 0, a2_ho = 0, a2_wo = 0;
+  if (a->A2) {
+    X3D_REQUIRE(!a->R, X3D_ERR_INVALID_ARG, "x3d_pw_tc_chain_fwd: A2 (shortcut as extra K) and R (residual) exclude each other");
+    X3D_REQUIRE(a->K2 > 0 && a->K2 % 8 == 0 && a->a2_stride >= 0, X3D_ERR_INVALID_ARG, "x3d_pw_tc_chain_fwd: bad second source K2=%d stride=%d", a->K2, a->a2_stride);
+    X3D_REQUIRE((reinterpret_cast<uintptr_t>(a->A2) & 15) == 0, X3D_ERR_INVALID_ARG, "x3d_pw_tc_chain_fwd: A2 must be 16-byte aligned");
+    if (a->a2_stride > 0) {
+      X3D_REQUIRE(a->a2_hi > 0 && a->a2_wi > 0 && a->a2_nt > 0, X3D_ERR_INVALID_ARG, "x3d_pw_tc_chain_fwd: bad second source %dx%d", a->a2_hi, a->a2_wi);
+      a2_ho = (a->a2_hi - 1) / a->a2_stride + 1; a2_wo = (a->a2_wi - 1) / a->a2_stride + 1;
+      X3D_REQUIRE(a->M == a->a2_nt * a2_ho * a2_wo, X3D_ERR_INVALID_ARG, "x3d_pw_tc_chain_fwd: M=%ld is not nt*Ho*Wo = %ld*%d*%d",
+                  (long)a->M, (long)a->a2_nt, a2_ho, a2_wo);
+      X3D_REQUIRE(tc::sampler_box(a2_ho, a2_wo, &a2_bh, &a2_bf), X3D_ERR_UNSUPPORTED,
+                  "x3d_pw_tc_chain_fwd: 128-pixel tiles do not align with %dx%d frames", a2_ho, a2_wo);
+    }
+  }
+  X3D_REQUIRE(tensor_map_encoder() != nullptr, X3D_ERR_NO_DEVICE, "x3d_pw_tc_chain_fwd: cuTensorMapEncodeTiled unavailable");
+  CUtensorMap tmA, tmW, tmD, tmW2, tmZ;
+  X3D_REQUIRE(tc::make_map_2d(&tmA, a->A, (uint64_t)a->K, (uint64_t)a->M, (uint64_t)a->lda * 2, 64, 128) &&
+              tc::make_map_2d(&tmW, a->Wp, (uint64_t)a->Kpad, (uint64_t)a->Npad, (uint64_t)a->Kpad * 2, 64, (uint32_t)pl.NT) &&
+              tc::make_map_2d(&tmD, a->D, (uint64_t)a->Nc, (uint64_t)a->M, (uint64_t)a->ldd * 2, 64, 128) &&
+              tc::make_map_2d(&tmW2, a->Wp2, (uint64_t)a->Kpad2, (uint64_t)a->Npad2, (uint64_t)a->Kpad2 * 2, 64, (uint32_t)pl.NT2) &&
+              tc::make_map_2d(&tmZ, a->D2, (uint64_t)a->Nc2, (uint64_t)a->M, (uint64_t)a->ldd2 * 2, 64, 128),
+              X3D_ERR_LAUNCH, "x3d_pw_tc_chain_fwd: tensor map encoding failed (K=%d Nc=%d Nc2=%d M=%ld)", a->K, a->Nc, a->Nc2, (long)a->M);
+  CUtensorMap tmA2 = tmA;
+  if (a->A2 && a->a2_stride > 0)
+    X3D_REQUIRE(tc::make_map_sampler(&tmA2, a->A2, a->K2, a->a2_hi, a->a2_wi, (long)a->a2_nt, a->a2_stride, a2_wo, a2_bh, a2_bf),
+                X3D_ERR_LAUNCH, "x3d_pw_tc_chain_fwd: tensor map for A2 failed (K2=%d %dx%d stride %d)", a->K2, a->a2_hi, a->a2_wi, a->a2_stride);
+  else if (a->A2)
+    X3D_REQUIRE(tc::make_map_2d(&tmA2, a->A2, (uint64_t)a->K2, (uint64_t)a->M, (uint64_t)a->K2 * 2, 64, 128),
+                X3D_ERR_LAUNCH, "x3d_pw_tc_chain_fwd: tensor map for dense A2 failed (K2=%d M=%ld)", a->K2, (long)a->M);
+
+  tc::ChainParams cp;
+  tc::Params& p = cp.c;
+  p.bias = a->bias; p.R = static_cast<const bf16*>(a->R); p.se = a->se; p.D = static_cast<bf16*>(a->D);
+  p.M = a->M; p.rows_per_clip = a->rows_per_clip; p.Kc = a->K; p.Nc = a->Nc; p.ldr = a->ldr; p.ldd = a->ldd;
+  p.colmean = nullptr; p.ldc = 0; p.store_d = 1;
+  p.KC1 = pl.KC1; p.k16_last1 = pl.k16_last1; p.a2_ppf = (a->A2 && a->a2_stride > 0) ? a2_ho * a2_wo : 0; p.a2_wo = a2_wo;
+  p.NT = pl.NT; p.KC = pl.KC; p.k16_last = pl.k16_last; p.stages = pl.stages; p.tmem_cols = pl.tmem_cols;
+  p.relu = a->relu; p.swish = a->swish;
+  p.contiguous = a->se != nullptr ? 1 : 0;
+  cp.bias2 = a->bias2; cp.Nc2 = a->Nc2; cp.NT2 = pl.NT2; cp.KCy = pl.KCy; cp.k16_y = pl.k16_y;
+  cp.pair = a->pair2 ? 1 : 0; cp.ny = pl.ny; cp.nd2 = pl.nd2; cp.relu2 = a->relu2;
+
+  const long num_tiles = (a->M + tc::kBlockM - 1) / tc::kBlockM;
+  const int gx = (int)(num_tiles < device_sm_count() ? num_tiles : device_sm_count());
+  cudaStream_t st = static_cast<cudaStream_t>(stream);
+  const bool pro = (a->se != nullptr) || a->swish;
+  cudaError_t e;
+  static SmemOptIn optin_pro, optin_plain;
+  if (pro) {
+    e = ensure_dynamic_smem(tc::pw_tc_chain_kernel<true>, optin_pro, pl.smem, false);
+    X3D_REQUIRE(e == cudaSuccess, X3D_ERR_LAUNCH, "x3d_pw_tc_chain_fwd: smem attribute: %s", cudaGetErrorString(e));
+    e = launch_pdl(tc::pw_tc_chain_kernel<true>, dim3(gx), dim3(tc::kChainThreadsPro), pl.smem, st, tmA, tmW, tmD, tmA2, tmW2, tmZ, cp);
+  } else {
+    e = ensure_dynamic_smem(tc::pw_tc_chain_kernel<false>, optin_plain, pl.smem, false);
+    X3D_REQUIRE(e == cudaSuccess, X3D_ERR_LAUNCH, "x3d_pw_tc_chain_fwd: smem attribute: %s", cudaGetErrorString(e));
+    e = launch_pdl(tc::pw_tc_chain_kernel<false>, dim3(gx), dim3(tc::kChainThreadsPlain), pl.smem, st, tmA, tmW, tmD, tmA2, tmW2, tmZ, cp);
+  }
+  X3D_REQUIRE(e == cudaSuccess, X3D_ERR_LAUNCH, "x3d_pw_tc_chain_fwd: launch: %s", cudaGetErrorString(e));
+  return check_launch("x3d_pw_tc_chain_fwd");
+}
 
 extern "C" int x3d_pw_tc_sampler_supported(int Hi, int Wi, int stride) {
   if (Hi <= 0 || Wi <= 0 || stride < 1) return 0;
diff --git a/x3d_tf_b200/model.py b/x3d_tf_b200/model.py
--- a/x3d_tf_b200/model.py
+++ b/x3d_tf_b200/model.py
@@ -195,6 +195,7 @@
         self._k2t = _pad_to(_pad_to(k2.T, 0, self.Ns), 1, self.Ks)
         self._paired: Dict[int, Tuple[torch.Tensor, torch.Tensor]] = {}
         self._stacked: Dict[int, tuple] = {}
+        self._doubled: Optional[torch.Tensor] = None
 
     def _pair_factor(self, M: int, rows_per_clip: int = 0) -> int:
         for P in (4, 2):
@@ -232,6 +233,28 @@
                 torch.bfloat16).contiguous()
             self._stacked[key] = (wp, (self.bias + other.bias).contiguous(), other)
         return self._stacked[key][:2]
+
+    def _doubled_weights(self, device) -> torch.Tensor:
+        if self._doubled is None:
+            w = np.zeros(((self.Ns + 15) // 16 * 16, (2 * self.Ks + 63) // 64 * 64), np.float64)
+            w[:self.Ns, :self.Ks] = self._k2t
+            w[:self.Ns, self.Ks:2 * self.Ks] = self._k2t
+            self._doubled = torch.from_numpy(np.ascontiguousarray(w, dtype=np.float32)).to(device).to(
+                torch.bfloat16).contiguous()
+        return self._doubled
+
+    def chain_pair(self, M: int, rows_per_clip: int) -> Optional[bool]:
+        P = self._pair_factor(M, rows_per_clip)
+        return None if P > 2 else P == 2
+
+    def run_chained(self, a: torch.Tensor, M: int, nxt: "PointwiseConv", pair2: bool, *, residual=None, se=None,
+                    rows_per_clip=0, swish=False, relu=False, shortcut: Optional["PointwiseConv"] = None,
+                    x: Optional[torch.Tensor] = None, stride: int = 1) -> Tuple[torch.Tensor, torch.Tensor]:
+        wp, bias = (self.wp, self.bias) if shortcut is None else self._stacked_weights(shortcut, a.device)
+        wp2 = nxt._doubled_weights(a.device) if pair2 else nxt.wp
+        return ops.pw_tc_chain_fwd(a, wp, bias, wp2, nxt.bias, M=M, K=self.Ks, Nc=self.Ns, Nc2=nxt.Ns,
+                                   residual=residual, se=se, rows_per_clip=rows_per_clip, swish=swish, relu=relu,
+                                   a2=x, a2_stride=stride, pair2=pair2)
 
     def run_with_shortcut(self, a: torch.Tensor, M: int, shortcut: "PointwiseConv", x: torch.Tensor,
                           stride: int, *, se=None, rows_per_clip=0, swish=False, relu=False) -> torch.Tensor:
@@ -269,6 +292,7 @@
     pair_max_k = int(os.environ.get("X3D_PAIR_MAX_K", "256"))
     pair_max_n = int(os.environ.get("X3D_PAIR_MAX_N", "256"))
     pair_aligned = os.environ.get("X3D_PAIR_ALIGNED", "0") == "1"
+    chain_expand = os.environ.get("X3D_CHAIN_EXPAND", "auto")
 
 
 def _use_tc() -> bool:
@@ -411,6 +435,27 @@
     def _forward(self, x: torch.Tensor, residual: Optional[torch.Tensor] = None,
                  relu: bool = False, shortcut: Optional[PointwiseConv] = None,
                  shortcut_rows: Optional[torch.Tensor] = None) -> torch.Tensor:
+        return self._forward_chain(x, residual, relu, shortcut, shortcut_rows)[0]
+
+    def _chain_target(self, nxt: Optional["Bottleneck"], b: torch.Tensor, M: int, rows_per_clip: int,
+                      se, swish: bool, shortcut: Optional[PointwiseConv], device) -> Optional[Tuple[PointwiseConv, bool]]:
+        if nxt is None or Options.chain_expand != "auto" or not _use_tc() or b.dtype != torch.bfloat16 or \
+                Options.fuse_expand != "off" or nxt.in_channels != self.out_channels or se is not None or swish:
+            return None
+        c = self._prep(device)["c"]
+        if shortcut is None and c._pair_factor(M, rows_per_clip) > 1:
+            return None
+        a = nxt._prep(device)["a"]
+        pair2 = a.chain_pair(M, rows_per_clip)
+        if pair2 is None or not ops.pw_tc_chain_supported(c.Ks, 0 if shortcut is None else shortcut.Ks,
+                                                          c.Ns, a.Ns, pair2):
+            return None
+        return a, pair2
+
+    def _forward_chain(self, x: torch.Tensor, residual: Optional[torch.Tensor] = None,
+                       relu: bool = False, shortcut: Optional[PointwiseConv] = None,
+                       shortcut_rows: Optional[torch.Tensor] = None, expanded: Optional[torch.Tensor] = None,
+                       nxt: Optional["Bottleneck"] = None) -> Tuple[torch.Tensor, Optional[torch.Tensor]]:
         if self.in_channels is None:
             raise RuntimeError("Bottleneck used before its input width is known")
         d = self._prep(x.device)
@@ -420,14 +465,15 @@
         _, ph, _ = A.same_pad(H, 3, self.stride)
         _, pw, _ = A.same_pad(W, 3, self.stride)
         mode = Options.fuse_expand
-        fuse2 = tc and x.dtype == torch.bfloat16 and (mode == "all" or (mode == "auto" and ci <= 72)) and \
+        fuse2 = expanded is None and tc and x.dtype == torch.bfloat16 and \
+            (mode == "all" or (mode == "auto" and ci <= 72)) and \
             ops.expand_dw2_supported(T, H, W, x.shape[-1], ci, self.stride) > 0
         if fuse2:
             ops.Profiler.tag = "ab"
             swish_in_b = Options.swish_in_dw and not self.has_se
             b, partial = ops.expand_dw2_fwd(x, d["a"].wp, d["a"].bias, d["wb"], d["bb"],
                                             self.stride, ph, pw, self.has_se, swish=swish_in_b)
-        elif tc and mode == "v1" and x.dtype == torch.bfloat16 and \
+        elif expanded is None and tc and mode == "v1" and x.dtype == torch.bfloat16 and \
                 ops.expand_dw_supported(T, H, W, x.shape[-1], ci, self.stride) > 0:
             ops.Profiler.tag = "ab"
             b, partial = ops.expand_dw_fwd(x, d["a"].wp, d["a"].bias, d["wb"], d["bb"],
@@ -435,7 +481,9 @@
             swish_in_b = False
         else:
             ops.Profiler.tag = "a"
-            a = d["a"].run(x, N * T * H * W, use_tc=tc, relu=True, pair_rows=T * H * W).view(N, T, H, W, ci)
+            if expanded is None:
+                expanded = d["a"].run(x, N * T * H * W, use_tc=tc, relu=True, pair_rows=T * H * W)
+            a = expanded.view(N, T, H, W, ci)
             ops.Profiler.tag = "b"
             swish_in_b = Options.swish_in_dw and not self.has_se
             cw = Options.channelwise
@@ -447,21 +495,29 @@
                 b, partial = ops.dw_planar_fwd(a, d["wbp"], self.stride, ph, pw, self.has_se, swish=swish_in_b)
             else:
                 b, partial = ops.dw_fwd(a, d["wb"], d["bb"], self.stride, ph, pw, self.has_se, swish=swish_in_b)
-            del a
+            del a, expanded
         _, _, Ho, Wo, _ = b.shape
         se = None
         if self.has_se:
             ops.Profiler.tag = "se"
             se = ops.se_mlp_fwd(partial, T * Ho * Wo, d["w1"], d["b1"], d["w2"], d["b2"])
         ops.Profiler.tag = "c"
-        if shortcut is not None:
-            out = d["c"].run_with_shortcut(b, N * T * Ho * Wo, shortcut, x if shortcut_rows is None else shortcut_rows,
+        M = N * T * Ho * Wo
+        target = self._chain_target(nxt, b, M, T * Ho * Wo, se, not swish_in_b, shortcut, x.device)
+        z = None
+        if target is not None:
+            out, z = d["c"].run_chained(b, M, target[0], target[1], residual=residual, se=se, rows_per_clip=T * Ho * Wo,
+                                        swish=not swish_in_b, relu=relu, shortcut=shortcut,
+                                        x=None if shortcut is None else (x if shortcut_rows is None else shortcut_rows),
+                                        stride=self.stride)
+        elif shortcut is not None:
+            out = d["c"].run_with_shortcut(b, M, shortcut, x if shortcut_rows is None else shortcut_rows,
                                            self.stride, se=se,
                                            rows_per_clip=T * Ho * Wo, swish=not swish_in_b, relu=relu)
         else:
-            out = d["c"].run(b, N * T * Ho * Wo, use_tc=tc, se=se, rows_per_clip=T * Ho * Wo,
+            out = d["c"].run(b, M, use_tc=tc, se=se, rows_per_clip=T * Ho * Wo,
                              swish=not swish_in_b, residual=residual, relu=relu)
-        return out.view(N, T, Ho, Wo, _pad8(self.out_channels))
+        return out.view(N, T, Ho, Wo, _pad8(self.out_channels)), z
 
     def call(self, input, training: bool = False):
         self._no_training(training)
@@ -504,6 +560,10 @@
         return self._dev[key]
 
     def _forward(self, x: torch.Tensor) -> torch.Tensor:
+        return self._forward_chain(x)[0]
+
+    def _forward_chain(self, x: torch.Tensor, expanded: Optional[torch.Tensor] = None,
+                       nxt: Optional[Bottleneck] = None) -> Tuple[torch.Tensor, Optional[torch.Tensor]]:
         d = self._prep(x.device)
         N, T, H, W, _ = x.shape
         if self.has_shortcut:
@@ -513,7 +573,8 @@
             if _use_tc() and x.dtype == torch.bfloat16 and Options.fold_shortcut:
                 rows = None if ops.pw_tc_sampler_supported(H, W, s) else \
                     (x.view(-1, x.shape[-1]) if s == 1 else ops.gather_rows_fwd(x, s))
-                return self.bottleneck._forward(x, relu=True, shortcut=d["r"], shortcut_rows=rows)
+                return self.bottleneck._forward_chain(x, relu=True, shortcut=d["r"], shortcut_rows=rows,
+                                                      expanded=expanded, nxt=nxt)
             if _use_tc() and x.dtype == torch.bfloat16:
                 rows = x.view(-1, x.shape[-1]) if s == 1 else ops.gather_rows_fwd(x, s)
                 res = d["r"].run(rows, N * T * Ho * Wo, use_tc=True, pair_rows=T * Ho * Wo)
@@ -521,7 +582,7 @@
                 res = d["r"].run(x, N * T * Ho * Wo, use_tc=False, gather=(T, Ho, Wo, H, W, s))
         else:
             res = x
-        return self.bottleneck._forward(x, residual=res, relu=True)
+        return self.bottleneck._forward_chain(x, residual=res, relu=True, expanded=expanded, nxt=nxt)
 
     def call(self, input, training: bool = False):
         self._no_training(training)
@@ -551,9 +612,12 @@
             self.blocks.append(self._child(f"stage/layer_with_weights-{i}", blk))
 
     def _forward(self, x):
-        for b in self.blocks:
-            x = b._forward(x)
-        return x
+        return self._forward_chain(x)[0]
+
+    def _forward_chain(self, x, expanded: Optional[torch.Tensor] = None, nxt: Optional[Bottleneck] = None):
+        for i, b in enumerate(self.blocks):
+            x, expanded = b._forward_chain(x, expanded, self.blocks[i + 1].bottleneck if i + 1 < len(self.blocks) else nxt)
+        return x, expanded
 
     def call(self, input, training: bool = False):
         self._no_training(training)
@@ -689,8 +753,10 @@
     def _forward(self, x: torch.Tensor, training: bool) -> Tuple[torch.Tensor, torch.Tensor]:
         act_dtype = self._dtype or (torch.float32 if x.dtype == torch.uint8 else x.dtype)
         out = self.conv1._forward(x, act_dtype)
-        for st in self.stages:
-            out = st._forward(out)
+        expanded = None
+        for i, st in enumerate(self.stages):
+            nxt = self.stages[i + 1].blocks[0].bottleneck if i + 1 < len(self.stages) else None
+            out, expanded = st._forward_chain(out, expanded, nxt)
         pooled = self.conv5._forward_pooled(out)
         if pooled is None:
             out = self.conv5._forward(out)
@@ -718,7 +784,8 @@
 
     def _graph(self, shape, dtype, device, slot: int = 0, training: bool = False):
         key = (tuple(shape), dtype, str(device), Options.pointwise, Options.stem, Options.stem_u8, Options.swish_in_dw,
-               Options.fuse_expand, Options.channelwise, Options.fold_shortcut, Options.pool_in_conv5, slot)
+               Options.fuse_expand, Options.channelwise, Options.fold_shortcut, Options.pool_in_conv5,
+               Options.chain_expand, slot)
         if key not in self._graphs:
             static_in = torch.zeros(tuple(shape), dtype=dtype, device=device)
             self._forward(static_in, training)
diff --git a/x3d_tf_b200/ops.py b/x3d_tf_b200/ops.py
--- a/x3d_tf_b200/ops.py
+++ b/x3d_tf_b200/ops.py
@@ -213,6 +213,48 @@
     return out
 
 
+def pw_tc_chain_fwd(a: torch.Tensor, wp: torch.Tensor, bias: Optional[torch.Tensor], wp2: torch.Tensor,
+                    bias2: Optional[torch.Tensor], *, M: int, K: int, Nc: int, Nc2: int,
+                    residual: Optional[torch.Tensor] = None, se: Optional[torch.Tensor] = None,
+                    rows_per_clip: int = 0, swish: bool = False, relu: bool = False,
+                    a2: Optional[torch.Tensor] = None, a2_stride: int = 1, pair2: bool = False,
+                    relu2: bool = True) -> Tuple[torch.Tensor, torch.Tensor]:
+    _req(a, "a")
+    if a.dtype != torch.bfloat16:
+        raise TypeError("pw_tc_chain_fwd needs bf16 activations")
+    y = torch.empty((M, Nc), dtype=torch.bfloat16, device=a.device)
+    z = torch.empty((M, Nc2), dtype=torch.bfloat16, device=a.device)
+    args = _lib.PwTcChainArgs()
+    args.A, args.Wp, args.bias = a.data_ptr(), wp.data_ptr(), _ptr(bias)
+    args.R, args.se, args.D = _ptr(residual), _ptr(se), y.data_ptr()
+    args.M, args.K, args.Nc = M, K, Nc
+    args.lda, args.ldr, args.ldd = K, Nc, Nc
+    args.Npad, args.Kpad = wp.shape
+    args.rows_per_clip = rows_per_clip
+    args.swish, args.relu = int(swish), int(relu)
+    if a2 is not None:
+        _req(a2, "a2")
+        if a2.dtype != torch.bfloat16 or a2.dim() not in (2, 5):
+            raise TypeError("pw_tc_chain_fwd: a2 must be a bf16 [N,T,H,W,C] tensor or a dense [M,C] matrix")
+        if a2.dim() == 5:
+            args.A2, args.a2_nt, args.K2 = a2.data_ptr(), a2.shape[0] * a2.shape[1], a2.shape[4]
+            args.a2_stride, args.a2_hi, args.a2_wi = a2_stride, a2.shape[2], a2.shape[3]
+        else:
+            if a2.shape[0] != M:
+                raise ValueError("pw_tc_chain_fwd: dense a2 needs M rows")
+            args.A2, args.K2, args.a2_stride = a2.data_ptr(), a2.shape[1], 0
+    args.Wp2, args.bias2, args.D2 = wp2.data_ptr(), _ptr(bias2), z.data_ptr()
+    args.Nc2, args.ldd2 = Nc2, Nc2
+    args.Npad2, args.Kpad2 = wp2.shape
+    args.pair2, args.relu2 = int(pair2), int(relu2)
+    _launch("x3d_pw_tc_chain_fwd", lambda: lib().x3d_pw_tc_chain_fwd(args, _stream()))
+    return y, z
+
+
+def pw_tc_chain_supported(K: int, K2: int, Nc: int, Nc2: int, pair2: bool) -> bool:
+    return bool(lib().x3d_pw_tc_chain_supported(K, K2, Nc, Nc2, int(pair2)))
+
+
 def pw_tc_sampler_supported(Hi: int, Wi: int, stride: int) -> bool:
     return bool(lib().x3d_pw_tc_sampler_supported(Hi, Wi, stride))
 
```
